# jgeisler0303/DDP-Generator

Hardware: AMD Instinct MI355X
Metric: iLQG iterations/sec, 65k-batch CarParking (n=4,m=2,N=500) (higher is better)
Workload: dtype f64

## Files before the change

### ddp-generator_amd/csrc/ilqg_host.c

```c
#include <math.h>
#include <stddef.h>
#include <stdio.h>
#include <stdlib.h>
#include <string.h>
#include <sys/time.h>

#include "mex.h"
#include "iLQG.h"
#include "back_pass.h"
#include "line_search.h"
#include "boxQP.h"
#include "matMult.h"
#include "printMat.h"

#include "ilqg_batch.h"
#include "ilqg_shim.h"
#include "ilqg_rules.h"

#define REC_HOST_SIZE_BASE (N_X + sizeofQxx + N_U + sizeofQuu + sizeofQxu + N_X * N_X + N_X * N_U + 2 * N_U)
#if FULL_DDP
#define REC_HOST_SIZE (REC_HOST_SIZE_BASE + N_X * sizeofQxx + N_X * sizeofQuu + N_X * sizeofQxu + 2 * N_U + 2 * N_X * N_U)
#else
#define REC_HOST_SIZE (REC_HOST_SIZE_BASE + 2 * N_U + 2 * N_X * N_U)
#endif
#define FIN_SIZE (N_X + sizeofQxx)

#ifndef DEBUG_ILQG
#define DEBUG_ILQG 1
#endif
#ifndef DEBUG_FORWARDPASS
#define DEBUG_FORWARDPASS 1
#endif
#define SAY_LOOP(level, args) do { if((DEBUG_ILQG) && o->debug_level >= (level)) PRNT args; } while(0)
#define SAY_SEARCH(level, args) do { if((DEBUG_FORWARDPASS) && o->debug_level >= (level)) PRNT args; } while(0)

#define ILQG_MAX_GROUPS 4
#define ILQG_TRACE_MAX 4096
struct ilqg_batch {
    ilqg_dev_t *dev[ILQG_MAX_GROUPS];
    int first[ILQG_MAX_GROUPS], count[ILQG_MAX_GROUPS];
    int groups;
    int device, B, N;
    tOptSet opt;
    double alpha_store[ILQG_MAX_ALPHA];
    int resweep, fuse_derivs, ls_split, ls_keep, bw_split;
    double **p;
    char *p_given;
    int params_pushed;
    int pb_n, pb_W, pb_named[64];
    char ps_on[64];
    int hist_cap;
    int compact;
    int trace_n;
    int trace_it[ILQG_TRACE_MAX], trace_active[ILQG_TRACE_MAX], trace_slots[ILQG_TRACE_MAX];
    int compactions;
    long long stream_counts[4];
    double *scratch;
    size_t scratch_doubles;
    char err[512];
};

static char g_create_err[512];

static void fatal_no_device(const char *what, const char *msg) {
    fprintf(stderr,
            "ilqg: %s needs the HIP backend, which is unavailable: %s\n"
            "ilqg: this library has no CPU fallback for the hot path.\n",
            what, msg ? msg : "");
    abort();
}

static double ilqg_default_alpha[8] = {1.0, 0.3727594, 0.1389495, 0.0517947,
                                       0.0193070, 0.0071969, 0.0026827, 0.0010000};

void standard_parameters(tOptSet *o) {
    o->alpha = ilqg_default_alpha;
    o->n_alpha = 8;
    o->tolFun = 1e-7;
    o->tolConstraint = 1e-7;
    o->tolGrad = 1e-5;
    o->max_iter = 20;
    o->lambdaInit = 1;
    o->dlambdaInit = 1;
    o->lambdaFactor = 1.6;
    o->lambdaMax = 1e10;
    o->lambdaMin = 1e-6;
    o->regType = 1;
    o->zMin = 0.0;
    o->debug_level = 2;
    o->w_pen_init_l = 1.0;
    o->w_pen_init_f = 1.0;
    o->w_pen_max_l = INF;
    o->w_pen_max_f = INF;
    o->w_pen_fact1 = 4.0;
    o->w_pen_fact2 = 1.0;
}

static char err_scalar[] = "parameter must be scalar";
static char err_alpha_range[] = "all alpha must be in the range [1.0..0.0)";
static char err_alpha_mono[] = "all alpha must be monotonically decreasing";
static char err_pos[] = "parameter must be positive";
static char err_gt_one[] = "parameter must be > 1";
static char err_one_two[] = "parameter must be in range [1..2]";
static char err_zero_one[] = "parameter must be in range [0..1)";
static char err_debug[] = "parameter must be in range [0..6]";
static char err_unknown[] = "no such parameter";

enum { CHK_GT0, CHK_GE0, CHK_GE1, CHK_1_2, CHK_0_1, CHK_0_6 };
typedef struct {
    const char *name;
    size_t offset;
    int is_int;
    int check;
} opt_row_t;

#define ROW_D(field, chk) {#field, offsetof(tOptSet, field), 0, chk}
#define ROW_I(field, chk) {#field, offsetof(tOptSet, field), 1, chk}
static const opt_row_t opt_rows[] = {
    ROW_D(tolFun, CHK_GT0),       ROW_D(tolConstraint, CHK_GT0), ROW_D(tolGrad, CHK_GT0),
    ROW_I(max_iter, CHK_GE0),     ROW_D(lambdaInit, CHK_GE0),    ROW_D(dlambdaInit, CHK_GE0),
    ROW_D(lambdaFactor, CHK_GE1), ROW_D(lambdaMax, CHK_GE0),     ROW_D(lambdaMin, CHK_GE0),
    ROW_I(regType, CHK_1_2),      ROW_D(zMin, CHK_0_1),          ROW_I(debug_level, CHK_0_6),
    ROW_D(w_pen_init_l, CHK_GE0), ROW_D(w_pen_init_f, CHK_GE0),  ROW_D(w_pen_max_l, CHK_GE0),
    ROW_D(w_pen_max_f, CHK_GE0),  ROW_D(w_pen_fact1, CHK_GE1),   ROW_D(w_pen_fact2, CHK_GE1),
};

char *setOptParam(tOptSet *o, const char *name, const double *value, const int n) {
    size_t r;
// ... 46 lines not shown
void printTri(const double *A, const int n, const char *nm) {
    int r, c;
    PRNT("%s= [\n", nm);
    for(r = 0; r < n; r++) {
        for(c = 0; c < n; c++) PRNT(c ? ", %g" : "  %g", A[SYMTRI_MAT_IDX(r, c)]);
        PRNT("\n");
    }
    PRNT("]\n");
}

void printMat(const double *A, const int n, const int m, const char *nm) {
    int r, c;
    PRNT("%s= [\n", nm);
    for(r = 0; r < n; r++) {
        for(c = 0; c < m; c++) PRNT(c ? ", %g" : "  %g", A[r + n * c]);
        PRNT("\n");
    }
    PRNT("]\n");
}

void printParams(double **p, int k) {
    int i;
    for(i = 0; i < n_params; i++) {
        if(paramdesc[i]->size == -1)
            PRNT("%s[k]= %g\n", paramdesc[i]->name, p[i][k]);
        else if(paramdesc[i]->size == 1)
            PRNT("%s= %g\n", paramdesc[i]->name, p[i][0]);
        else
            printVec(p[i], paramdesc[i]->size, paramdesc[i]->name);
    }
}

static int fail(ilqg_batch_t *c, const char *what) {
    snprintf(c->err, sizeof(c->err), "%s: %s", what, ilqg_dev_error());
    return 1;
}

static int fail_msg(ilqg_batch_t *c, const char *msg) {
    snprintf(c->err, sizeof(c->err), "%s", msg);
    return 1;
}

void ilqg_problem_dims(int *out) {
    ilqg_dev_dims(out);
    out[6] = n_params;
}

const char *ilqg_problem_param_name(int i) { return (i >= 0 && i < n_params) ? paramdesc[i]->name : NULL; }
int ilqg_problem_param_size(int i) { return (i >= 0 && i < n_params) ? paramdesc[i]->size : 0; }
int ilqg_device_count(void) { return ilqg_dev_count(); }

int ilqg_reference_success(int status, int iterations) {
    switch(status) {
    case ILQG_ST_CONVERGED_GRAD:
    case ILQG_ST_CONVERGED_FUN:
    case ILQG_ST_LAMBDA_MAX: return 1;
    case ILQG_ST_DERIVS_FAILED: return iterations > 0;
    default: return 0;
    }
}

const char *ilqg_batch_error(const ilqg_batch_t *c) { return c ? c->err : g_create_err; }

static int param_len(const ilqg_batch_t *c, int i) { return paramdesc[i]->size == -1 ? c->N + 1 : paramdesc[i]->size; }

static int find_param(const char *name) {
    int i;
    for(i = 0; i < n_params; i++)
        if(strcmp(paramdesc[i]->name, name) == 0) return i;
    return -1;
}

ilqg_batch_t *ilqg_batch_create_groups(int device, int batch, int n_hor, int groups) {
    int i, g, per, dims[8];
    ilqg_batch_t *c = (ilqg_batch_t *)calloc(1, sizeof(*c));
    if(!c) return NULL;
    c->device = device;
    c->B = batch;
    c->N = n_hor;
    c->resweep = (sizeof(multipliersEl_t) > 0 || sizeof(multipliersFin_t) > 0) ? 1 : 0;
    c->fuse_derivs = c->resweep ? 0 : 1;
    c->ls_keep = 1;
    c->bw_split = 0;
    standard_parameters(&c->opt);
    ilqg_dev_dims(dims);
    c->ls_split = dims[7] ? 1 : 4;
    c->ls_keep = 2;
    if(groups <= 0) {
        const char *e = getenv("ILQG_GROUPS");
        groups = e ? atoi(e) : ((batch >= 8192 && !dims[7]) ? 4 : 1);
    }

    if(groups < 1) groups = 1;
    if(groups > ILQG_MAX_GROUPS) groups = ILQG_MAX_GROUPS;
    per = ((batch + groups - 1) / groups + 63) / 64 * 64;
    c->groups = 0;
    for(g = 0; g < groups && (g == 0 || g * per < batch); g++) {
        c->first[g] = g * per;
        c->count[g] = (batch - g * per < per) ? batch - g * per : per;
        if(ilqg_dev_create(&c->dev[g], device, c->count[g], n_hor)) {
            snprintf(g_create_err, sizeof(g_create_err), "ilqg_batch_create: %s", ilqg_dev_error());
            for(i = 0; i < g; i++) ilqg_dev_destroy(c->dev[i]);
            free(c);
            return NULL;
        }
        c->groups = g + 1;
    }
    c->p = (double **)calloc(n_params > 0 ? n_params : 1, sizeof(double *));
    c->p_given = (char *)calloc(n_params > 0 ? n_params : 1, 1);
    for(i = 0; i < n_params; i++) c->p[i] = (double *)calloc(param_len(c, i), sizeof(double));
    return c;
}

ilqg_batch_t *ilqg_batch_create(int device, int batch, int n_hor) {
    return ilqg_batch_create_groups(device, batch, n_hor, 0);
}

int ilqg_batch_groups(const ilqg_batch_t *c) { return c->groups; }

void ilqg_batch_destroy(ilqg_batch_t *c) {
    int i;
    if(!c) return;
    for(i = 0; i < c->groups; i++) ilqg_dev_destroy(c->dev[i]);
    for(i = 0; i < n_params; i++) free(c->p[i]);
    free(c->p);
    free(c->p_given);
    free(c->scratch);
    free(c);
}

#define EACH_GROUP(g) for(g = 0; g < c->groups; g++)
static int each_write(ilqg_batch_t *c, int field, const double *host, const char *what) {
    int g;
    EACH_GROUP(g) {
        const size_t per = (size_t)ilqg_dev_field_steps(c->dev[g], field) * ilqg_dev_field_width(field);
        if(ilqg_dev_write(c->dev[g], field, host + per * c->first[g])) return fail(c, what);
    }
    return 0;
}
static int each_write_steps(ilqg_batch_t *c, int field, const double *host, int steps, const char *what) {
    int g;
    EACH_GROUP(g) {
        const size_t per = (size_t)steps * ilqg_dev_field_width(field);
        if(ilqg_dev_write_steps(c->dev[g], field, host + per * c->first[g], steps)) return fail(c, what);
    }
    return 0;
}
static int each_read(ilqg_batch_t *c, int field, double *host, const char *what) {
    int g;
    EACH_GROUP(g) {
        const size_t per = (size_t)ilqg_dev_field_steps(c->dev[g], field) * ilqg_dev_field_width(field);
        if(ilqg_dev_read(c->dev[g], field, host + per * c->first[g])) return fail(c, what);
    }
    return 0;
}
static int int_width(int field) { return field == ILQG_I_ALPHA_OK ? ILQG_MAX_ALPHA : 1; }
static int each_read_int(ilqg_batch_t *c, int field, int *host, const char *what) {
    int g;
    EACH_GROUP(g) if(ilqg_dev_read_int(c->dev[g], field, host + (size_t)int_width(field) * c->first[g])) return fail(c, what);
    return 0;
}
static int each_write_int(ilqg_batch_t *c, int field, const int *host, const char *what) {
    int g;
    EACH_GROUP(g) if(ilqg_dev_write_int(c->dev[g], field, host + (size_t)int_width(field) * c->first[g])) return fail(c, what);
    return 0;
}

int ilqg_batch_set_option(ilqg_batch_t *c, const char *name, const double *value, int n) {
    char *e;
    if(strcmp(name, "resweep") == 0) {
        if(n != 1) return fail_msg(c, err_scalar);
        c->resweep = value[0] != 0.0;
        return 0;
    }
    if(strcmp(name, "ls_split") == 0) {
        if(n != 1) return fail_msg(c, err_scalar);
        if(value[0] < 0.0) return fail_msg(c, err_pos);
        c->ls_split = (int)value[0];
        return 0;
    }
    if(strcmp(name, "bw_split") == 0) {
        if(n != 1) return fail_msg(c, err_scalar);
        c->bw_split = value[0] != 0.0;
        return 0;
    }
    if(strcmp(name, "ls_keep") == 0) {
        if(n != 1) return fail_msg(c, err_scalar);
        if(value[0] != 0.0 && value[0] != 1.0 && value[0] != 2.0) return fail_msg(c, "ls_keep must be 0, 1 or 2");
        c->ls_keep = (int)value[0];
        return 0;
    }
    if(strcmp(name, "fuse_derivs") == 0) {
        if(n != 1) return fail_msg(c, err_scalar);
        c->fuse_derivs = value[0] != 0.0;
        return 0;
    }
    if(strcmp(name, "compact") == 0) {
        if(n != 1) return fail_msg(c, err_scalar);
        if(value[0] < 0.0) return fail_msg(c, err_pos);
        c->compact = (int)value[0];
        return 0;
    }
    if(strcmp(name, "alpha") == 0) {
        tOptSet probe = c->opt;
        if(n > ILQG_MAX_ALPHA) return fail_msg(c, "at most 16 alpha values");
        e = setOptParam(&probe, name, value, n);
        if(e) return fail_msg(c, e);
        memcpy(c->alpha_store, value, sizeof(double) * n);
        value = c->alpha_store;
    }
    e = setOptParam(&c->opt, name, value, n);
    if(e) return fail_msg(c, e);
    return 0;
}

int ilqg_batch_set_param(ilqg_batch_t *c, const char *name, const double *value, int n) {
    const int i = find_param(name);
    int j;
    if(i < 0) {
        snprintf(c->err, sizeof(c->err), "Parameter name '%s' is not a parameter of this problem.", name);
        return 1;
    }
    if(param_len(c, i) != n) {
        snprintf(c->err, sizeof(c->err), "Parameter name '%s' must be a vector length %d.", name, param_len(c, i));
        return 1;
    }
    for(j = 0; j < c->pb_n; j++)
        if(c->pb_named[j] == i) {
            snprintf(c->err, sizeof(c->err), "ilqg_batch_set_param: name: parameter '%s' currently has a value per trajectory "
                     "(ilqg_batch_set_params_batch); a shared value would be read by no trajectory.  Clear the per-trajectory set "
                     "first: ilqg_batch_set_params_batch(c, 0, NULL, NULL)", name);
            return 1;
        }
    if(i < 64 && c->ps_on[i]) {
        snprintf(c->err, sizeof(c->err), "ilqg_batch_set_param: name: parameter '%s' currently has a window per trajectory "
                 "(ilqg_batch_set_param_steps_batch); a shared window would be read by no trajectory.  Use "
                 "ilqg_batch_set_param_steps_batch / ilqg_batch_shift_param_batch, or make the name shared again first: "
                 "ilqg_batch_set_param_steps_batch(c, name, values = NULL)", name);
        return 1;
    }
    memcpy(c->p[i], value, sizeof(double) * n);
    c->p_given[i] = 1;
    c->params_pushed = 0;
    return 0;
}

static int push_config(ilqg_batch_t *c) {
    ilqg_dev_opts_t d;
    int i;
    const tOptSet *o = &c->opt;
    memset(&d, 0, sizeof(d));
    if(o->n_alpha < 1 || o->n_alpha > ILQG_MAX_ALPHA) return fail_msg(c, "n_alpha must be in 1..16");
    d.n_alpha = o->n_alpha;
    for(i = 0; i < o->n_alpha; i++) d.alpha[i] = o->alpha[i];
    d.tolFun = o->tolFun; d.tolGrad = o->tolGrad; d.tolConstraint = o->tolConstraint;
    d.lambdaInit = o->lambdaInit; d.dlambdaInit = o->dlambdaInit; d.lambdaFactor = o->lambdaFactor;
    d.lambdaMax = o->lambdaMax; d.lambdaMin = o->lambdaMin;
    d.zMin = o->zMin; d.regType = o->regType; d.max_iter = o->max_iter;
    d.w_pen_init_l = o->w_pen_init_l; d.w_pen_init_f = o->w_pen_init_f;
    d.w_pen_max_l = o->w_pen_max_l; d.w_pen_max_f = o->w_pen_max_f;
    d.w_pen_fact1 = o->w_pen_fact1; d.w_pen_fact2 = o->w_pen_fact2;
    d.resweep = c->resweep;
    d.fuse_derivs = c->fuse_derivs;
    d.ls_split = c->ls_split;
    d.ls_keep = c->ls_keep;
    d.bw_split = c->bw_split;
    { int g; EACH_GROUP(g) if(ilqg_dev_set_opts(c->dev[g], &d)) return fail(c, "options"); }
    if(!c->params_pushed) {
        int sizes[64];
        for(i = 0; i < n_params; i++)
            if(!c->p_given[i]) {
                snprintf(c->err, sizeof(c->err), "Parameter name '%s' was not set.", paramdesc[i]->name);
                return 1;
            }
        if(n_params > 64) return fail_msg(c, "more than 64 problem parameters");
        for(i = 0; i < n_params; i++) sizes[i] = paramdesc[i]->size;
        { int g; EACH_GROUP(g) if(ilqg_dev_set_params(c->dev[g], n_params, sizes, (const double *const *)c->p)) return fail(c, "parameters"); }
        c->params_pushed = 1;
    }
    return 0;
}

int ilqg_batch_set_x0(ilqg_batch_t *c, const double *x0) { return each_write_steps(c, ILQG_F_X, x0, 1, "set_x0"); }
int ilqg_batch_set_u(ilqg_batch_t *c, const double *u) { return each_write(c, ILQG_F_U, u, "set_u"); }
int ilqg_batch_set_x(ilqg_batch_t *c, const double *x) { return each_write(c, ILQG_F_X, x, "set_x"); }

static int restart(ilqg_batch_t *c) {
    int g;
    EACH_GROUP(g) {
        if(ilqg_dev_rollout_init(c->dev[g])) return fail(c, "initial roll-out");
        if(ilqg_dev_reset(c->dev[g])) return fail(c, "reset");
    }
    return 0;
}

static int clear_history(ilqg_batch_t *c, const char *who) {
    int g;
    if(c->hist_cap > 0) EACH_GROUP(g) if(ilqg_dev_set_history(c->dev[g], c->hist_cap)) return fail(c, who);
    return 0;
}

int ilqg_batch_init(ilqg_batch_t *c) { return push_config(c) || clear_history(c, "ilqg_batch_init") || restart(c); }

typedef struct { const void *ptr; const char *name; } named_ptr_t;
static int device_ptrs(ilqg_batch_t *c, const char *who, const named_ptr_t *ptrs, int n) {
    int i;
    for(i = 0; i < n; i++)
        if(ptrs[i].ptr && ilqg_dev_check_device_ptr(c->dev[0], ptrs[i].ptr, ptrs[i].name)) return fail(c, who);
    return 0;
}
static int stream_in(ilqg_batch_t *c, void *stream, const char *what) {
    int g;
    EACH_GROUP(g) if(ilqg_dev_stream_in(c->dev[g], stream)) return fail(c, what);
    return 0;
}

static int shift_groups(ilqg_batch_t *c, int round, int on_device, int steps, const double *x0_new, const double *u_tail, void *stream) {
    int g;
    EACH_GROUP(g) if(round >= 0 ? ilqg_dev_loop_shift(c->dev[g], round) : ilqg_dev_shift(c->dev[g], steps, x0_new == NULL)) return fail(c, "shift");
    EACH_GROUP(g) {
        const double *const x0_g = x0_new ? x0_new + (size_t)c->first[g] * N_X : NULL;
        const double *const tail_g = (u_tail && steps > 0) ? u_tail + (size_t)c->first[g] * steps * N_U : NULL;
        if(x0_g && (on_device ? ilqg_dev_put_x0_device(c->dev[g], x0_g) : ilqg_dev_write_steps(c->dev[g], ILQG_F_X, x0_g, 1)))
            return fail(c, "shift: x0_new");
        if(tail_g && (on_device ? ilqg_dev_put_u_tail_device : ilqg_dev_write_u_tail)(c->dev[g], tail_g, steps)) return fail(c, "shift: u_tail");
        if(on_device && ilqg_dev_stream_out(c->dev[g], stream)) return fail(c, "shift: stream");
    }
    return restart(c);
}
static int shift(ilqg_batch_t *c, const char *who, int on_device, int steps, const double *x0_new, const double *u_tail, void *stream) {
    const named_ptr_t ptrs[] = {{x0_new, "x0_new"}, {u_tail, "u_tail"}};
    if(steps < 0 || steps >= c->N) {
        snprintf(c->err, sizeof(c->err), "%s: steps = %d, must be in 0 .. n_hor - 1 = %d", who, steps, c->N - 1);
        return 1;
    }
    if(on_device && device_ptrs(c, who, ptrs, 2)) return 1;
    if(push_config(c)) return 1;
    if(on_device && stream_in(c, stream, "shift: stream")) return 1;
    return shift_groups(c, -1, on_device, steps, x0_new, u_tail, stream);
}

int ilqg_batch_shift(ilqg_batch_t *c, int steps, const double *x0_new, const double *u_tail) {
    return shift(c, "ilqg_batch_shift", 0, steps, x0_new, u_tail, NULL);
}

int ilqg_batch_shift_device(ilqg_batch_t *c, int steps, const double *x0_new, const double *u_tail, void *stream) {
    return shift(c, "ilqg_batch_shift_device", 1, steps, x0_new, u_tail, stream);
}

// ... 633 lines not shown
    }
    if(steps < 0 || steps > c->N) {
        snprintf(c->err, sizeof(c->err), "ilqg_batch_shift_param: steps = %d, must be in 0 .. n_hor = %d", steps, c->N);
        return 1;
    }
    if(i < 64 && c->ps_on[i]) {
        snprintf(c->err, sizeof(c->err), "ilqg_batch_shift_param: name: parameter '%s' currently has a window per trajectory "
                 "(ilqg_batch_set_param_steps_batch); moving the shared window would move what no trajectory reads.  Use "
                 "ilqg_batch_shift_param_batch, or make the name shared again first: ilqg_batch_set_param_steps_batch(c, name, "
                 "values = NULL)", name);
        return 1;
    }
    if(steps == 0) return 0;
    n = c->N + 1;
    if(c->params_pushed) EACH_GROUP(g) if(ilqg_dev_shift_param(c->dev[g], i, steps, tail)) return fail(c, "shift_param");
    for(k = 0; k < n; k++) c->p[i][k] = k + steps < n ? c->p[i][k + steps] : (tail ? tail[k + steps - n] : c->p[i][n - 1]);
    return 0;
}

static int iterate_groups(ilqg_batch_t *c, int n) {
    int it, g;
    for(it = 0; it < n; it++) EACH_GROUP(g) if(ilqg_dev_iterate(c->dev[g], 1)) return fail(c, "iterate");
    return 0;
}

int ilqg_batch_iterate(ilqg_batch_t *c, int n) {
    if(push_config(c)) return 1;
    return iterate_groups(c, n);
}

int ilqg_batch_active(ilqg_batch_t *c, int *n) {
    int g, a;
    *n = 0;
    EACH_GROUP(g) {
        if(ilqg_dev_count_active(c->dev[g], &a)) return fail(c, "active count");
        *n += a;
    }
    return 0;
}

static double now_s(void) {
    struct timeval tv;
    gettimeofday(&tv, NULL);
    return (double)tv.tv_sec + 1e-6 * (double)tv.tv_usec;
}
static int group_of(const ilqg_batch_t *c, int b) {
    int g;
    for(g = c->groups - 1; g > 0; g--)
        if(b >= c->first[g]) break;
    return g;
}
static int move_between(ilqg_batch_t *dst, ilqg_batch_t *src, int n, const int *dst_idx, const int *src_idx) {
    int gd, gs, j, rc = 0;
    int *to = (int *)malloc(sizeof(int) * (n > 0 ? n : 1)), *from = (int *)malloc(sizeof(int) * (n > 0 ? n : 1));
    for(gd = 0; gd < dst->groups && !rc; gd++)
        for(gs = 0; gs < src->groups && !rc; gs++) {
            int m = 0;
            for(j = 0; j < n; j++)
                if(group_of(dst, dst_idx[j]) == gd && group_of(src, src_idx[j]) == gs) {
                    to[m] = dst_idx[j] - dst->first[gd];
                    from[m] = src_idx[j] - src->first[gs];
                    m++;
                }
            if(m && ilqg_dev_move(dst->dev[gd], src->dev[gs], m, to, from, !src->fuse_derivs)) rc = fail(dst, "moving trajectories");
        }
    free(to);
    free(from);
    return rc;
}
static ilqg_batch_t *working_copy(ilqg_batch_t *c, int n) {
    int i;
    int dims[8], groups;
    ilqg_batch_t *w;
    ilqg_dev_dims(dims);
    (void)dims;
    groups = 0;
    if(getenv("ILQG_COMPACT_GROUPS")) groups = atoi(getenv("ILQG_COMPACT_GROUPS"));
    w = ilqg_batch_create_groups(c->device, n, c->N, groups);
    if(!w) return NULL;
    c->stream_counts[3] += 1;
    w->opt = c->opt;
    memcpy(w->alpha_store, c->opt.alpha, sizeof(double) * c->opt.n_alpha);
    w->opt.alpha = w->alpha_store;
    w->resweep = c->resweep; w->fuse_derivs = c->fuse_derivs; w->ls_split = c->ls_split; w->ls_keep = c->ls_keep; w->bw_split = c->bw_split;
    for(i = 0; i < n_params; i++) {
        memcpy(w->p[i], c->p[i], sizeof(double) * param_len(c, i));
        w->p_given[i] = c->p_given[i];
    }
    if(push_config(w)) {
        snprintf(c->err, sizeof(c->err), "%s", w->err);
        ilqg_batch_destroy(w);
        return NULL;
    }
    return w;
}

int ilqg_batch_solve(ilqg_batch_t *c) {
    int it, active = 1, rc = 0, j;
    ilqg_batch_t *cur = c;
    int *map = NULL, *status = NULL, *ident = NULL;
    const int dbg = getenv("ILQG_SOLVE_DEBUG") != NULL;
    double t_dbg = 0.0, t_poll = 0.0;
    if(push_config(c)) return 1;
    c->err[0] = 0;
    c->trace_n = 0;
    t_poll = dbg ? now_s() : 0.0;
    c->compactions = 0;
    for(it = 0; it < c->opt.max_iter && active; ) {
        int n = c->opt.max_iter - it < 4 ? c->opt.max_iter - it : 4;
        if(iterate_groups(cur, n)) { rc = 1; break; }
        it += n;
        if(ilqg_batch_active(cur, &active)) { rc = 1; break; }
        if(dbg && it % 40 == 0) {
            fprintf(stderr, "ilqg solve: iteration %d, %d live of %d slots, %.2f ms per iteration\n", it, active, cur->B, 1e3 * (now_s() - t_poll) / n);
        }
        t_poll = dbg ? now_s() : 0.0;
        if(c->trace_n < ILQG_TRACE_MAX) {
            c->trace_it[c->trace_n] = it;
            c->trace_active[c->trace_n] = active;
            c->trace_slots[c->trace_n] = cur->B;
            c->trace_n++;
        }
        if(c->compact > 0 && active > 0 && it < c->opt.max_iter && 2 * active <= cur->B && active >= c->compact) {
            ilqg_batch_t *w;
            int *nmap, m = 0;
            status = (int *)realloc(status, sizeof(int) * cur->B);
            if(each_read_int(cur, ILQG_I_STATUS, status, "status")) { rc = 1; break; }
            if(cur != c) {
                ident = (int *)realloc(ident, sizeof(int) * cur->B);
                for(j = 0; j < cur->B; j++) ident[j] = j;
                if(move_between(c, cur, cur->B, map, ident)) { rc = 1; break; }
            }
            nmap = (int *)malloc(sizeof(int) * active);
            for(j = 0; j < cur->B && m < active; j++)
                if(status[j] == ILQG_ST_ACTIVE) nmap[m++] = (cur == c) ? j : map[j];
            t_dbg = dbg ? now_s() : 0.0;
            w = working_copy(c, m);
            if(!w) { free(nmap); rc = 1; break; }
            if(dbg) fprintf(stderr, "ilqg solve: iteration %d, %d live of %d slots: new context %.1f ms", it, m, cur->B, 1e3 * (now_s() - t_dbg));
            t_dbg = dbg ? now_s() : 0.0;
            ident = (int *)realloc(ident, sizeof(int) * (m > cur->B ? m : cur->B));
            for(j = 0; j < m; j++) ident[j] = j;
            if(move_between(w, c, m, ident, nmap)) { snprintf(c->err, sizeof(c->err), "%s", w->err); ilqg_batch_destroy(w); free(nmap); rc = 1; break; }
            if(dbg) fprintf(stderr, ", gather %.1f ms", 1e3 * (now_s() - t_dbg));
            t_dbg = dbg ? now_s() : 0.0;
            if(cur != c) ilqg_batch_destroy(cur);
            if(dbg) fprintf(stderr, ", release %.1f ms\n", 1e3 * (now_s() - t_dbg));
            free(map);
            cur = w;
            map = nmap;
            c->compactions++;
        }
    }
    if(cur != c) {
        if(!rc) {
            ident = (int *)realloc(ident, sizeof(int) * cur->B);
            for(j = 0; j < cur->B; j++) ident[j] = j;
            if(move_between(c, cur, cur->B, map, ident)) rc = 1;
        } else if(!c->err[0]) {
            snprintf(c->err, sizeof(c->err), "%s", cur->err);
        }
        ilqg_batch_destroy(cur);
    }
    free(map);
    free(status);
    free(ident);
    return rc;
// ... 1384 lines not shown
```

### ddp-generator_amd/csrc/ilqg_shim.h

```cpp
#ifndef ILQG_SHIM_H
#define ILQG_SHIM_H

#ifdef __cplusplus
extern "C" {
#endif

#define ILQG_MAX_ALPHA 16

typedef struct ilqg_dev ilqg_dev_t;

typedef struct {
    int n_alpha;
    double alpha[ILQG_MAX_ALPHA];
    double tolFun, tolGrad, tolConstraint;
    double lambdaInit, dlambdaInit, lambdaFactor, lambdaMax, lambdaMin;
    double zMin;
    int regType;
    int max_iter;
    double w_pen_init_l, w_pen_init_f, w_pen_max_l, w_pen_max_f, w_pen_fact1, w_pen_fact2;
    int resweep;
    int ls_split;
    int ls_keep;
    int bw_split;
    int fuse_derivs;
} ilqg_dev_opts_t;

enum {
    ILQG_ST_ACTIVE = 0,
    ILQG_ST_CONVERGED_GRAD = 1,
    ILQG_ST_CONVERGED_FUN = 2,
    ILQG_ST_MAX_ITER = 3,
    ILQG_ST_NO_DESCENT = 4,
    ILQG_ST_LAMBDA_MAX = 5,
    ILQG_ST_DERIVS_FAILED = 6,
    ILQG_ST_INIT_FAILED = 7
};

enum {
    ILQG_F_X = 0,
    ILQG_F_U,
    ILQG_F_LG,
    ILQG_F_KG,
    ILQG_F_DER,
    ILQG_F_FIN,
    ILQG_F_MUL,
    ILQG_F_MULF,
    ILQG_F_COST,
    ILQG_F_NEW_COST,
    ILQG_F_DCOST,
    ILQG_F_EXPECTED,
    ILQG_F_LAMBDA,
    ILQG_F_DLAMBDA,
    ILQG_F_GNORM,
    ILQG_F_DV0,
    ILQG_F_DV1,
    ILQG_F_WPEN_L,
    ILQG_F_WPEN_F,
    ILQG_F_WPEN_L_DER,
    ILQG_F_WPEN_F_DER,
    ILQG_F_ALPHA_COST,
    ILQG_F_COUNT
};

enum {
    ILQG_I_STATUS = 0,
    ILQG_I_ITER,
    ILQG_I_NEED_DERIVS,
    ILQG_I_ALPHA_IDX,
    ILQG_I_ACCEPTED,
    ILQG_I_BP_CALLS,
    ILQG_I_BP_RC,
    ILQG_I_RESWEEP,
    ILQG_I_LOC,
    ILQG_I_ALPHA_OK,
    ILQG_I_COUNT
};

enum {
    ILQG_K_DERIVS = 0,
    ILQG_K_BACKWARD,
    ILQG_K_ROLLOUT_SEARCH,
    ILQG_K_SELECT,
    ILQG_K_ROLLOUT_WINNER,
    ILQG_K_UPDATE,
    ILQG_K_ROLLOUT_COST,
    ILQG_K_ROLLOUT_INIT,
    ILQG_K_TRANSPOSE,
    ILQG_K_BACKWARD_FUSED,
    ILQG_K_ROLLOUT_SEARCH2,
    ILQG_K_MULTIPLIERS,
    ILQG_K_SEARCH,
    ILQG_K_SEARCH2,
    ILQG_K_ADOPT,
    ILQG_K_SHIFT,
    ILQG_K_LOG,
    ILQG_K_HEAD,
    ILQG_K_SHIFT_PARAM,
    ILQG_K_POLICY,
    ILQG_K_POLICY_PARAMS,
    ILQG_K_PLANT,
    ILQG_K_SHIFT_PARAM_ROWS,
    ILQG_K_SHIFT_WINDOWS,
    ILQG_K_HISTORY,
    ILQG_K_COUNT
};
enum {
    ILQG_K_BEST_OF = ILQG_K_COUNT,
// ... 146 lines not shown
```

### ddp-generator_amd/csrc/ilqg_shim_impl.inc

```

#if ILQG_WAVE_MAP
struct SharedWork {
    trajEl_t *buf;
    size_t bytes;
    hipEvent_t free_ev;
    int refs;
    bool whole, half[2], factored, pv_set;
    int N, B, part, half_cap;
    ParamValues pv;
};
static SharedWork g_work[64];
#else
struct SharedWork;
#endif

constexpr int QUEUE_CELL = 32;

namespace {

struct DeviceMem {
    static hipError_t take(void **p, size_t bytes) { return hipMalloc(p, bytes); }
    static hipError_t give(void *p) { return hipFree(p); }
};
struct PinnedMem {
    static hipError_t take(void **p, size_t bytes) { return hipHostMalloc(p, bytes, hipHostMallocDefault); }
    static hipError_t give(void *p) { return hipHostFree(p); }
};
template <class T, class Mem = DeviceMem>
class Buffer {
    T *p_ = nullptr;
    size_t bytes_ = 0;

  public:
    Buffer() = default;
    Buffer(const Buffer &) = delete;
    Buffer &operator=(const Buffer &) = delete;
    Buffer(Buffer &&o) noexcept : p_(o.p_), bytes_(o.bytes_) { o.p_ = nullptr, o.bytes_ = 0; }
    Buffer &operator=(Buffer &&o) noexcept {
        if(this != &o) {
            (void)release();
            p_ = o.p_, bytes_ = o.bytes_;
            o.p_ = nullptr, o.bytes_ = 0;
        }
        return *this;
    }
    ~Buffer() {
        if(p_) (void)Mem::give(p_);
    }
    T *get() const { return p_; }
    size_t bytes() const { return bytes_; }
    int release() {
        T *old = p_;
        p_ = nullptr, bytes_ = 0;
        if(old) HIP_TRY(Mem::give(old));
        return 0;
    }
    int renew(size_t bytes) {
        if(release()) return 1;
        const hipError_t allocation = Mem::take((void **)&p_, bytes);
        if(allocation != hipSuccess) p_ = nullptr;
        HIP_TRY(allocation);
        bytes_ = bytes;
        return 0;
    }
    int reserve(size_t bytes, hipStream_t drain = nullptr) {
        if(bytes <= bytes_) return 0;
        if(drain) HIP_TRY(hipStreamSynchronize(drain));
        return renew(bytes);
    }
    int try_reserve(size_t bytes, hipStream_t drain) {
        if(bytes <= bytes_) return 0;
        HIP_TRY(hipStreamSynchronize(drain));
        if(release()) return 1;
        if(getenv("ILQG_TEST_NO_PLANES") || Mem::take((void **)&p_, bytes) != hipSuccess) {
            (void)hipGetLastError();
            p_ = nullptr;
            return 2;
        }
        bytes_ = bytes;
        return 0;
    }
};
template <class T>
static int repoint(T *&view, const Buffer<T> &owner, int rc) {
    view = owner.get();
    return rc;
}

struct DevBuffers {
    Buffer<double> f[ILQG_F_COUNT], nom;
    Buffer<int> i[ILQG_I_COUNT], derivs_failed, pending_list, n_pending;
    Buffer<trajEl_t> work;
    Buffer<double *> param_table;
    std::vector<Buffer<double>> param_bufs;
    Buffer<int> counter;
    Buffer<int> queues;
    Buffer<double> cand, cand1;
    Buffer<double> xpl, upl;
    Buffer<unsigned> spec_ints;
    Buffer<double> spec_doubles;
    Buffer<double> log_x, log_u, log_c;
    Buffer<double> plant_xp, plant_cost, plant_values, plant_dist;
    Buffer<int> plant_failed;
    Buffer<double> pb_values;
    static constexpr int SR = N_STEP_PARAMS > 0 ? N_STEP_PARAMS : 1;
    Buffer<double> sr_rows[SR];
    Buffer<double> win_future[SR];
    Buffer<double> hist_d;
    Buffer<int> hist_i;
    Buffer<double> hist_next_d;
    Buffer<int> hist_next_i;
    Buffer<unsigned long long> harvest;
    Buffer<char, PinnedMem> harvest_host;
    Buffer<double> staging;
    Buffer<char, PinnedMem> pinned;
};

template <class Fn>
struct WaveKernel {
    Fn fn;
    int block;
    size_t lds;
    int per_wg;
    int cap;
    size_t lds_limit;
    bool scratch;
    dim3 grid(size_t n, int cus) const {
        const size_t wgs = (n + per_wg - 1) / per_wg, most = (size_t)cap * cus;
        return dim3((unsigned)(cap && most < wgs ? most : wgs));
    }
};
struct WaveKernels {
    WaveKernel<void (*)(DevPtrs, ilqg_dev_opts_t, ParamValues, int, int, int, int, int)> derivs[2];
    WaveKernel<void (*)(DevPtrs, ilqg_dev_opts_t, int, int, int)> sweep[6];
};

}

struct ilqg_dev : DevBuffers {
    int device, B, Bp, N;
    hipStream_t stream;
    DevPtrs P;
    ilqg_dev_opts_t O;
    ParamValues pv;
    bool io_deferred;
    size_t io_off;
    struct PendingRead { void *dst; const void *src; size_t bytes; int transpose_w; };
    std::vector<PendingRead> pending;
    bool keep_first;
    size_t roll_pad;
    bool roll_dma;
    int loc_set;
    bool defer_commit, commit_pending, pending_zero;
    int commit_s1, commit_set;
    bool winner_done;
    int cus;
    bool work_consts;
    bool half_consts[2];
    hipStream_t stream2;
    hipEvent_t fork, join;
    hipStream_t roll;
    hipEvent_t roll_in, roll_out;
    struct SharedWork *shared;
    bool per_step_params;
    struct Loop {
        int rounds, steps;
        bool plant, windows;
        bool named;
        PolicyParamMap map;
        bool given[SR];
    } loop;
    bool pb_on;
    PolicyParamMap pb_map;
    bool sr_on[SR];
    bool rows_on;
    PolicyParamMap rows_map;
    int hist_next_cap;
    History hist;
    hipEvent_t ext_in, ext_out;
    struct EnvSwitches { bool no_quad, quad_stored, two_pieces, deriv_parts, no_dma, no_rollout_parts, quad_spec, second_stream; size_t roll_lds; } env;
    WaveKernels wave_kernels;
    bool timing;
    struct Span { int kernel; hipEvent_t a, b; };
    std::vector<Span> spans;
    std::vector<hipEvent_t> event_pool;
    double t_ms[ILQG_K_TOTAL];
    int t_n[ILQG_K_TOTAL];
    hipEvent_t epoch;
    double t_busy[ILQG_K_TOTAL];
};

namespace {

static ilqg_dev *g_spec_last;
struct FieldInfo { int steps_plus; int wd, wh; };

FieldInfo field_info(int f) {
    switch(f) {
        case ILQG_F_X: return {1, NX, NX};
        case ILQG_F_U: return {0, NU, NU};
        case ILQG_F_LG: return {0, NU, NU};
        case ILQG_F_KG: return {0, NXU, NXU};
        case ILQG_F_DER: return {0, WAVE_MAP ? REC_HOST : REC, REC_HOST};
        case ILQG_F_FIN: return {-1, FIN, FIN};
        case ILQG_F_MUL: return {0, MEW, MEW};
        case ILQG_F_MULF: return {-1, MFW, MFW};
        case ILQG_F_ALPHA_COST: return {-1, ILQG_MAX_ALPHA, ILQG_MAX_ALPHA};
        default: return {-1, 1, 1};
    }
}

int nom_column(int field) {
    switch(field) {
        case ILQG_F_X: return NOM_X;
        case ILQG_F_U: return NOM_U;
        case ILQG_F_LG: return NOM_L;
        case ILQG_F_KG: return NOM_K;
        default: return -1;
    }
}
bool has_tiled_copy(int field) { return !WAVE_MAP && (field == ILQG_F_X || field == ILQG_F_U); }
bool has_tiled_scratch(int field) { return !WAVE_MAP && (field == ILQG_F_LG || field == ILQG_F_KG); }
int field_steps(const ilqg_dev *d, int f) {
    const FieldInfo fi = field_info(f);
    return fi.steps_plus < 0 ? 1 : d->N + fi.steps_plus;
}

int int_field_width(int f) { return f == ILQG_I_ALPHA_OK ? ILQG_MAX_ALPHA : 1; }

int io_flush(ilqg_dev *d) {
    HIP_TRY(hipStreamSynchronize(d->stream));
    for(const auto &r : d->pending) {
        if(r.transpose_w) {
            const int *src = (const int *)r.src;
            int *dst = (int *)r.dst;
            for(int b = 0; b < d->B; b++)
                for(int j = 0; j < r.transpose_w; j++) dst[(size_t)b * r.transpose_w + j] = src[(size_t)j * d->Bp + b];
        } else {
            memcpy(r.dst, r.src, r.bytes);
        }
    }
    d->pending.clear();
    d->io_off = 0;
    return 0;
}

int stage(ilqg_dev *d, size_t bytes, void **dev, void **pin) {
    if(!d->io_deferred) {
        if(d->staging.reserve(bytes)) return 1;
        *dev = d->staging.get();
        *pin = nullptr;
        return 0;
    }
    bytes = (bytes + 255) & ~(size_t)255;
    if(d->io_off + bytes > d->staging.bytes() || d->io_off + bytes > d->pinned.bytes()) {
        if(io_flush(d)) return 1;
        const size_t want = (bytes > (1u << 20) ? bytes : (1u << 20)) + 2 * d->pinned.bytes();
        if(d->staging.reserve(want) || d->pinned.reserve(want)) return 1;
    }
    *dev = (char *)d->staging.get() + d->io_off;
    *pin = d->pinned.get() + d->io_off;
    d->io_off += bytes;
    return 0;
}
int stage_in(ilqg_dev *d, void *dev, void *pin, const void *host, size_t bytes) {
    if(pin) {
        memcpy(pin, host, bytes);
        host = pin;
    }
    HIP_TRY(hipMemcpyAsync(dev, host, bytes, hipMemcpyHostToDevice, d->stream));
    return 0;
}
int stage_out(ilqg_dev *d, const void *dev, void *pin, void *host, size_t bytes) {
    HIP_TRY(hipMemcpyAsync(pin ? pin : host, dev, bytes, hipMemcpyDeviceToHost, d->stream));
    if(pin) d->pending.push_back({host, pin, bytes, 0});
    else HIP_TRY(hipStreamSynchronize(d->stream));
    return 0;
}
// ... 298 lines not shown
                    }
                    bytes = bytes / 2 + sizeof(trajEl_t);
                }
                W.bytes = bytes;
                HIP_TRY(hipMemsetAsync(W.buf, 0, W.bytes, d->stream));
                HIP_TRY(hipStreamSynchronize(d->stream));
                HIP_TRY(hipEventCreateWithFlags(&W.free_ev, hipEventDisableTiming));
            }
            W.refs++;
            d->shared = &W;
            if((W.bytes - sizeof(trajEl_t)) / per_traj < 1) {
                g_err = "ilqg_dev_create: the device's derivative work buffer (made for a shorter horizon) does not hold one trajectory";
                return 1;
            }
#endif
            continue;
        }
        if(nom_column(f) >= 0 && !has_tiled_copy(f) && !has_tiled_scratch(f)) continue;
        const FieldInfo fi = field_info(f);
        const size_t bytes = (size_t)field_steps(d, f) * fi.wd * d->Bp * sizeof(double);
        if(repoint(d->P.f[f], d->f[f], d->f[f].reserve(bytes))) return 1;
        HIP_TRY(hipMemsetAsync(d->P.f[f], 0, bytes, d->stream));
    }
    {
        const size_t bytes = (size_t)d->Bp * (d->N + 1) * RN * sizeof(double);
        if(repoint(d->P.nom, d->nom, d->nom.reserve(bytes))) return 1;
        HIP_TRY(hipMemsetAsync(d->P.nom, 0, bytes, d->stream));
    }
    for(int f = 0; f < ILQG_I_COUNT; f++) {
        const size_t bytes = (size_t)int_field_width(f) * d->Bp * sizeof(int);
        if(repoint(d->P.i[f], d->i[f], d->i[f].reserve(bytes))) return 1;
        HIP_TRY(hipMemsetAsync(d->P.i[f], 0, bytes, d->stream));
    }
    if(repoint(d->P.derivs_failed, d->derivs_failed, d->derivs_failed.reserve(d->Bp * sizeof(int)))) return 1;
    HIP_TRY(hipMemsetAsync(d->P.derivs_failed, 0, d->Bp * sizeof(int), d->stream));
    if(d->counter.reserve(sizeof(int))) return 1;
    if(d->queues.reserve(2 * QUEUE_CELL * sizeof(int))) return 1;
    {
        int cus = 0;
        HIP_TRY(hipDeviceGetAttribute(&cus, hipDeviceAttributeMultiprocessorCount, device));
        d->cus = cus > 0 ? cus : 256;
    }
    if(repoint(d->P.pending, d->pending_list, d->pending_list.reserve(d->Bp * sizeof(int)))) return 1;
    if(repoint(d->P.n_pending, d->n_pending, d->n_pending.reserve(sizeof(int)))) return 1;
    HIP_TRY(hipMemsetAsync(d->P.n_pending, 0, sizeof(int), d->stream));
    d->P.n_pending_next = d->P.n_pending;
    HIP_TRY(hipStreamSynchronize(d->stream));
    return 0;
}

void ilqg_dev_destroy(ilqg_dev_t *d) {
    if(!d) return;
    hipSetDevice(d->device);
    if(d->stream) hipStreamSynchronize(d->stream);
    if(d->stream2) hipStreamSynchronize(d->stream2);
    for(auto &s : d->spans) {
        hipEventDestroy(s.a);
        hipEventDestroy(s.b);
    }
    for(hipEvent_t e : d->event_pool) hipEventDestroy(e);
    static_cast<DevBuffers &>(*d) = DevBuffers();
#if ILQG_WAVE_MAP
    if(d->shared && --d->shared->refs == 0) {
        hipFree(d->shared->buf);
        hipEventDestroy(d->shared->free_ev);
        memset(d->shared, 0, sizeof(SharedWork));
    }
#endif
    if(g_spec_last == d) g_spec_last = nullptr;
    if(d->stream) hipStreamDestroy(d->stream);
    if(d->stream2) hipStreamDestroy(d->stream2);
    if(d->fork) hipEventDestroy(d->fork);
    if(d->join) hipEventDestroy(d->join);
    if(d->roll) hipStreamSynchronize(d->roll);
    if(d->roll_in) hipEventDestroy(d->roll_in);
    if(d->roll_out) hipEventDestroy(d->roll_out);
    if(d->epoch) hipEventDestroy(d->epoch);
    if(d->ext_in) hipEventDestroy(d->ext_in);
    if(d->ext_out) hipEventDestroy(d->ext_out);
    delete d;
}

int ilqg_dev_set_params(ilqg_dev_t *d, int n_params, const int *sizes, const double *const *values) {
    HIP_TRY(hipSetDevice(d->device));
    HIP_TRY(hipStreamSynchronize(d->stream));
    d->param_bufs.clear();
    if(repoint(d->P.p, d->param_table, d->param_table.release())) return 1;
    std::vector<double *> ptrs(n_params > 0 ? n_params : 1, nullptr);
    {
        constexpr int want[ILQG_NP > 0 ? ILQG_NP : 1] = ILQG_PSIZES;
        constexpr int offs[ILQG_NP > 0 ? ILQG_NP : 1] = ILQG_POFFSETS;
        if(n_params != ILQG_NP) {
            g_err = "ilqg_dev_set_params: parameter count differs from the problem this library was built for";
            return 1;
        }
        for(int i = 0; i < n_params; i++) {
            if(sizes[i] != want[i]) {
                g_err = "ilqg_dev_set_params: parameter size differs from the problem's paramdesc[]";
                return 1;
            }
            for(int j = 0; j < sizes[i]; j++) d->pv.v[offs[i] + j] = values[i][j];
        }
        d->per_step_params = false;
        for(int i = 0; i < n_params; i++) d->per_step_params |= (sizes[i] == -1);
    }
    for(int i = 0; i < n_params; i++) {
        const int sz = sizes[i] == -1 ? d->N + 1 : sizes[i];
        Buffer<double> buf;
        if(buf.reserve(sz * sizeof(double))) return 1;
        HIP_TRY(hipMemcpy(buf.get(), values[i], sz * sizeof(double), hipMemcpyHostToDevice));
        ptrs[i] = buf.get();
        d->param_bufs.push_back(std::move(buf));
    }
    if(repoint(d->P.p, d->param_table, d->param_table.reserve(ptrs.size() * sizeof(double *)))) return 1;
    HIP_TRY(hipMemcpy(d->P.p, ptrs.data(), ptrs.size() * sizeof(double *), hipMemcpyHostToDevice));
    d->work_consts = d->half_consts[0] = d->half_consts[1] = false;
    return 0;
}

static const PolicyParamMap *policy_param_map(int n_named, const int *named, const double *values, PolicyParamMap &map);
static void rows_refresh(ilqg_dev_t *d) {
    PolicyParamMap m;
    if(d->pb_on) {
        m = d->pb_map;
    } else {
        for(int j = 0; j < ILQG_PTOTAL; j++) m.src[j] = -1;
        m.W = 0;
    }
    const bool steps = step_rows_into(m, d);
    d->rows_map = m;
    d->rows_on = d->pb_on || steps;
}
static int table_buffer(ilqg_dev_t *d, size_t bytes) {
    if(bytes <= d->pb_values.bytes()) return 0;
    d->pb_on = false;
    rows_refresh(d);
    return d->pb_values.reserve(bytes, d->stream);
}
int ilqg_dev_set_params_batch(ilqg_dev_t *d, int n_named, const int *named, const double *values, int on_device) {
    HIP_TRY(hipSetDevice(d->device));
    if(WAVE_MAP) {
        g_err = "set_params_batch: this library maps one wavefront to a trajectory (wave mapping); its kernels do not carry "
                "parameters per lane, per-trajectory parameters need a lane-mapped library";
        return 1;
    }
    if(n_named < 0) {
        g_err = "set_params_batch: n_names must not be negative";
        return 1;
    }
    if(n_named == 0) {
        d->pb_on = false;
        rows_refresh(d);
        return 0;
    }
    PolicyParamMap map;
    if(!policy_param_map(n_named, named, values, map)) return 1;
    const size_t bytes = (size_t)d->B * (size_t)map.W * sizeof(double);
    if(table_buffer(d, bytes)) return 1;
    HIP_TRY(hipMemcpyAsync(d->pb_values.get(), values, bytes, on_device ? hipMemcpyDeviceToDevice : hipMemcpyHostToDevice, d->stream));
    if(!on_device) HIP_TRY(hipStreamSynchronize(d->stream));
    d->pb_map = map;
    d->pb_on = true;
    rows_refresh(d);
    return 0;
}

static int step_slot(int index) {
    constexpr int sizes[ILQG_NP > 0 ? ILQG_NP : 1] = ILQG_PSIZES;
    if(index < 0 || index >= ILQG_NP || sizes[index] != -1) return -1;
    int s = 0;
    for(int i = 0; i < index; i++) s += sizes[i] == -1 ? 1 : 0;
    return s;
}
static int step_rows_buffer(ilqg_dev_t *d, int s) {
    const size_t n = (size_t)d->N + 1, bytes = (size_t)d->Bp * n * sizeof(double);
    if(bytes > d->sr_rows[s].bytes()) {
        d->sr_on[s] = false;
        rows_refresh(d);
        if(d->sr_rows[s].reserve(bytes, d->stream)) return 1;
    }
    if(!d->sr_on[s] && d->Bp > d->B)
        HIP_TRY(hipMemsetAsync(d->sr_rows[s].get() + (size_t)d->B * n, 0, (size_t)(d->Bp - d->B) * n * sizeof(double), d->stream));
    return 0;
}
int ilqg_dev_set_param_steps_batch(ilqg_dev_t *d, int index, const double *values, int on_device) {
    HIP_TRY(hipSetDevice(d->device));
    if(WAVE_MAP) {
        g_err = "set_param_steps_batch: this library maps one wavefront to a trajectory (wave mapping); its kernels do not carry "
                "parameters per lane, per-trajectory parameters need a lane-mapped library";
        return 1;
    }
    const int s = step_slot(index);
    if(s < 0) {
        g_err = "set_param_steps_batch: not a parameter with one value per time step";
        return 1;
    }
    if(!values) {
        d->sr_on[s] = false;
        rows_refresh(d);
        return 0;
    }
    if(step_rows_buffer(d, s)) return 1;
    const size_t bytes = (size_t)d->B * ((size_t)d->N + 1) * sizeof(double);
    HIP_TRY(hipMemcpyAsync(d->sr_rows[s].get(), values, bytes, on_device ? hipMemcpyDeviceToDevice : hipMemcpyHostToDevice, d->stream));
    if(!on_device) HIP_TRY(hipStreamSynchronize(d->stream));
    d->sr_on[s] = true;
    rows_refresh(d);
    return 0;
}

int ilqg_dev_get_param_steps_batch(ilqg_dev_t *d, int index, double *rows) {
    HIP_TRY(hipSetDevice(d->device));
    const int s = step_slot(index);
    if(s < 0 || !d->sr_on[s]) {
        g_err = "get_param_steps_batch: the parameter has no rows per trajectory in this context";
        return 1;
    }
    HIP_TRY(hipMemcpyAsync(rows, d->sr_rows[s].get(), (size_t)d->B * ((size_t)d->N + 1) * sizeof(double), hipMemcpyDeviceToHost, d->stream));
    HIP_TRY(hipStreamSynchronize(d->stream));
    return 0;
}

int ilqg_dev_get_params_batch(ilqg_dev_t *d, double *rows) {
    HIP_TRY(hipSetDevice(d->device));
    if(!d->pb_on) {
        g_err = "get_params_batch: the context has no per-trajectory parameters";
        return 1;
    }
    HIP_TRY(hipMemcpyAsync(rows, d->pb_values.get(), (size_t)d->B * (size_t)d->pb_map.W * sizeof(double), hipMemcpyDeviceToHost, d->stream));
    HIP_TRY(hipStreamSynchronize(d->stream));
    return 0;
}

int ilqg_dev_set_opts(ilqg_dev_t *d, const ilqg_dev_opts_t *o) {
#if !ILQG_EXPERIMENTS
    if(o->bw_split) {
        g_err = "option bw_split: the two-wavefront backward pass (a measured negative result) is compiled into the -DILQG_EXPERIMENTS libraries only (lib*_exp.so)";
        return 1;
    }
#endif
    if(o->n_alpha < 1 || o->n_alpha > ILQG_MAX_ALPHA) {
        g_err = "ilqg_dev_set_opts: n_alpha must be in 1..16";
        return 1;
    }
    d->O = *o;
    return 0;
}

int ilqg_dev_field_width(int field) { return field_info(field).wh; }
int ilqg_dev_field_steps(ilqg_dev_t *d, int field) { return field_steps(d, field); }
void *ilqg_dev_field_ptr(ilqg_dev_t *d, int field) { return d->P.f[field]; }
void *ilqg_dev_stream(ilqg_dev_t *d) { return (void *)d->stream; }

int ilqg_dev_copy_scalar_to(ilqg_dev_t *d, int field, void *dst_device) {
    HIP_TRY(hipSetDevice(d->device));
    if(field < ILQG_F_COST || field >= ILQG_F_ALPHA_COST) {
        g_err = "ilqg_dev_copy_scalar_to: not a per-trajectory scalar field";
        return 1;
    }
    HIP_TRY(hipMemcpyAsync(dst_device, d->P.f[field], (size_t)d->B * sizeof(double), hipMemcpyDeviceToDevice, d->stream));
    return 0;
}

int ilqg_dev_write(ilqg_dev_t *d, int field, const double *host) {
    return ilqg_dev_write_steps(d, field, host, field_steps(d, field));
}

static bool is_traj_major(int field) { return WAVE_MAP && field == ILQG_F_FIN; }

static int nom_io(ilqg_dev *d, int field, double *host_rw, const double *host_ro, int steps) {
    const FieldInfo fi = field_info(field);
    const size_t n = (size_t)d->B * steps * fi.wh;
    void *dev, *pin;
    if(stage(d, n * sizeof(double), &dev, &pin)) return 1;
    if(host_ro && stage_in(d, dev, pin, host_ro, n * sizeof(double))) return 1;
    {
        Timed t(d, ILQG_K_TRANSPOSE);
        hipLaunchKernelGGL(k_nom_io, grid1(n, 256), dim3(256), 0, d->stream, d->P.nom, (double *)dev, d->B, d->N, steps,
                           fi.wh, nom_column(field), host_ro ? 1 : 0);
    }
    HIP_TRY(hipGetLastError());
    if(host_rw) return stage_out(d, dev, pin, host_rw, n * sizeof(double));
    return io_done(d);
}

#if ILQG_WAVE_MAP
#define REC_FIELDS(OP)                                                                            \
    OP(cx, NX) OP(cxx, SXX) OP(cu, NU) OP(cuu, SUU) OP(cxu, NXU) OP(fx, NX * NX) OP(fu, NXU)     \
    OP(lower, NU) OP(upper, NU) REC_FIELDS_FULL(OP)                                               \
    OP(lower_sign, NU) OP(upper_sign, NU) OP(lower_hx, NXU) OP(upper_hx, NXU)
#if FULL_DDP
#define REC_FIELDS_FULL(OP) OP(fxx, NX * SXX) OP(fuu, NX * SUU) OP(fxu, NX * NXU)
#else
#define REC_FIELDS_FULL(OP)
#endif

static int own_work(ilqg_dev *d) {
    if(d->P.work) return 0;
    size_t free_b = 0, total_b = 0;
    HIP_TRY(hipMemGetInfo(&free_b, &total_b));
    const size_t per_traj = (size_t)d->N * sizeof(trajEl_t);
    if((double)d->B * (double)per_traj > 0.5 * (double)free_b) {
        g_err = "derivative records of the whole batch do not fit the device (wave mapping): stage-by-stage calls and "
                "record transfers need a smaller batch; ilqg_dev_iterate / ilqg_dev_backward(mode 2) work in chunks";
        return 1;
    }
    if(repoint(d->P.work, d->work, d->work.reserve((size_t)d->B * per_traj))) return 1;
    HIP_TRY(hipMemsetAsync(d->P.work, 0, (size_t)d->B * per_traj, d->stream));
    d->work_consts = false;
    return 0;
}

static int der_io(ilqg_dev *d, double *host_rw, const double *host_ro) {
    if(own_work(d)) return 1;
    const size_t n = (size_t)d->B * d->N;
    std::vector<trajEl_t> tmp(n);
    HIP_TRY(hipMemcpy(tmp.data(), d->P.work, n * sizeof(trajEl_t), hipMemcpyDeviceToHost));
    for(size_t e = 0; e < n; e++) {
        trajEl_t &t = tmp[e];
        if(host_ro) {
            const double *r = host_ro + e * REC_HOST;
#define OP(field, cnt) memcpy(t.field, r, sizeof(double) * (cnt)); r += (cnt);
            REC_FIELDS(OP)
#undef OP
        } else {
            double *r = host_rw + e * REC_HOST;
#define OP(field, cnt) memcpy(r, t.field, sizeof(double) * (cnt)); r += (cnt);
            REC_FIELDS(OP)
#undef OP
        }
    }
    if(host_ro) HIP_TRY(hipMemcpy(d->P.work, tmp.data(), n * sizeof(trajEl_t), hipMemcpyHostToDevice));
    return 0;
}
#endif

static int all_home(ilqg_dev_t *d);

int ilqg_dev_write_steps(ilqg_dev_t *d, int field, const double *host, int steps) {
    HIP_TRY(hipSetDevice(d->device));
    if(has_tiled_copy(field) && all_home(d)) return 1;
    const FieldInfo fi = field_info(field);
    if(steps < 1 || steps > field_steps(d, field)) {
        g_err = "ilqg_dev_write_steps: bad step count";
        return 1;
    }
#if ILQG_WAVE_MAP
    if(field == ILQG_F_DER) {
        if(io_flush(d)) return 1;
        return der_io(d, nullptr, host);
    }
#endif
    if(nom_column(field) >= 0) {
        if(nom_io(d, field, nullptr, host, steps)) return 1;
        if(!has_tiled_copy(field)) return 0;
    }
    if(is_traj_major(field)) {
        const size_t row = (size_t)steps * fi.wd * sizeof(double);
        const size_t dpitch = (size_t)field_steps(d, field) * fi.wd * sizeof(double);
        const void *src = host;
        if(d->io_deferred) {
            void *dev, *pin;
            if(stage(d, row * d->B, &dev, &pin)) return 1;
            memcpy(pin, host, row * d->B);
            src = pin;
        }
        HIP_TRY(hipMemcpy2DAsync(d->P.f[field], dpitch, src, row, row, d->B, hipMemcpyHostToDevice, d->stream));
        return io_done(d);
    }
    const size_t n = (size_t)d->B * steps * fi.wh;
    void *dev, *pin;
    if(stage(d, n * sizeof(double), &dev, &pin)) return 1;
    if(stage_in(d, dev, pin, host, n * sizeof(double))) return 1;
    {
        Timed t(d, ILQG_K_TRANSPOSE);
        const size_t total = (size_t)d->B * steps * fi.wd;
        hipLaunchKernelGGL(k_to_dev, grid1(total, 256), dim3(256), 0, d->stream, (const double *)dev, d->P.f[field], d->B, d->Bp,
                           steps, fi.wh, fi.wd);
    }
    HIP_TRY(hipGetLastError());
    return io_done(d);
}

int ilqg_dev_read(ilqg_dev_t *d, int field, double *host) {
    HIP_TRY(hipSetDevice(d->device));
    if(has_tiled_copy(field) && all_home(d)) return 1;
    const FieldInfo fi = field_info(field);
    const int steps = field_steps(d, field);
    const size_t n = (size_t)d->B * steps * fi.wh;
#if ILQG_WAVE_MAP
    if(field == ILQG_F_DER) {
        if(io_flush(d)) return 1;
        return der_io(d, host, nullptr);
    }
#endif
    if(nom_column(field) >= 0 && !has_tiled_copy(field)) return nom_io(d, field, host, nullptr, steps);
    if(is_traj_major(field)) {
        void *dev = nullptr, *pin = nullptr;
        if(d->io_deferred && stage(d, n * sizeof(double), &dev, &pin)) return 1;
        return stage_out(d, d->P.f[field], pin, host, n * sizeof(double));
    }
    void *dev, *pin;
    if(stage(d, n * sizeof(double), &dev, &pin)) return 1;
    {
        Timed t(d, ILQG_K_TRANSPOSE);
        hipLaunchKernelGGL(k_from_dev, grid1(n, 256), dim3(256), 0, d->stream, d->P.f[field], (double *)dev, d->B, d->Bp,
                           steps, fi.wh, fi.wd);
    }
    HIP_TRY(hipGetLastError());
    return stage_out(d, dev, pin, host, n * sizeof(double));
}

int ilqg_dev_write_int(ilqg_dev_t *d, int field, const int *host) {
    HIP_TRY(hipSetDevice(d->device));
    const int w = int_field_width(field);
    const size_t bytes = (size_t)w * d->Bp * sizeof(int);
    std::vector<int> tmp;
    int *src;
    if(d->io_deferred) {
        void *dev, *pin;
        if(stage(d, bytes, &dev, &pin)) return 1;
        src = (int *)pin;
    } else {
        tmp.resize((size_t)w * d->Bp);
        src = tmp.data();
    }
    memset(src, 0, bytes);
    for(int b = 0; b < d->B; b++)
        for(int j = 0; j < w; j++) src[(size_t)j * d->Bp + b] = host[(size_t)b * w + j];
    HIP_TRY(hipMemcpyAsync(d->P.i[field], src, bytes, hipMemcpyHostToDevice, d->stream));
    return io_done(d);
}

int ilqg_dev_read_int(ilqg_dev_t *d, int field, int *host) {
    HIP_TRY(hipSetDevice(d->device));
    const int w = int_field_width(field);
    const size_t bytes = (size_t)w * d->Bp * sizeof(int);
    if(d->io_deferred) {
        void *dev, *pin;
        if(stage(d, bytes, &dev, &pin)) return 1;
        HIP_TRY(hipMemcpyAsync(pin, d->P.i[field], bytes, hipMemcpyDeviceToHost, d->stream));
        d->pending.push_back({host, pin, bytes, w});
        return 0;
    }
    std::vector<int> tmp((size_t)w * d->Bp, 0);
    HIP_TRY(hipMemcpyAsync(tmp.data(), d->P.i[field], tmp.size() * sizeof(int), hipMemcpyDeviceToHost, d->stream));
    HIP_TRY(hipStreamSynchronize(d->stream));
    for(int b = 0; b < d->B; b++)
        for(int j = 0; j < w; j++) host[(size_t)b * w + j] = tmp[(size_t)j * d->Bp + b];
    return 0;
}

int ilqg_dev_io_begin(ilqg_dev_t *d) {
    d->io_deferred = true;
    d->io_off = 0;
    return 0;
}

int ilqg_dev_io_end(ilqg_dev_t *d) {
    HIP_TRY(hipSetDevice(d->device));
    d->io_deferred = false;
    return io_flush(d);
}

#define NEED_PARAMS(d)                                                   \
    if(!(d)->P.p) {                                                      \
        g_err = "problem parameters not set (ilqg_dev_set_params)";      \
        return 1;                                                        \
    }

static int all_home(ilqg_dev_t *d) {
#if !ILQG_WAVE_MAP
    if(d->loc_set < 0) return 0;
    hipLaunchKernelGGL(k_all_home, dim3(8 * d->cus), dim3(256), 0, d->stream, d->P);
    HIP_TRY(hipGetLastError());
    HIP_TRY(hipMemsetAsync(d->P.i[ILQG_I_LOC], 0, d->Bp * sizeof(int), d->stream));
    d->loc_set = -1;
#endif
    return 0;
}

int ilqg_dev_reset(ilqg_dev_t *d) {
    HIP_TRY(hipSetDevice(d->device));
    hipLaunchKernelGGL(k_reset, grid1(d->Bp, 256), dim3(256), 0, d->stream, d->P, d->O);
    if(HAS_MUL) {
        NEED_PARAMS(d);
        Timed t(d, ILQG_K_MULTIPLIERS);
        LAUNCH_TWIN(d, k_multipliers, dim3(d->Bp / WAVE), dim3(WAVE), 0, d->stream, d->P, d->O, d->pv, 1);
    }
    HIP_TRY(hipGetLastError());
    return 0;
}

static hipStream_t roll_stream(ilqg_dev_t *d) { return d->roll ? d->roll : d->stream; }
static int roll_enter(ilqg_dev_t *d) {
    if(!d->roll) return 0;
    HIP_TRY(hipEventRecord(d->roll_in, d->stream));
    HIP_TRY(hipStreamWaitEvent(d->roll, d->roll_in, 0));
    return 0;
}
static int roll_leave(ilqg_dev_t *d) {
    if(!d->roll) return 0;
    HIP_TRY(hipEventRecord(d->roll_out, d->roll));
    HIP_TRY(hipStreamWaitEvent(d->stream, d->roll_out, 0));
    return 0;
}

static void launch_rollout(ilqg_dev_t *d, int mode, int kernel_id, int a0, int n_alpha, hipStream_t stream = nullptr) {
    if(!stream) stream = d->stream;
    Timed t(d, kernel_id, stream);
    const dim3 grid((d->Bp + ROLL_BLOCK - 1) / ROLL_BLOCK, n_alpha), block(ROLL_BLOCK);
    if(mode == ROLL_INIT)
        with_rows(d, [&](auto... tr) { hipLaunchKernelGGL((k_rollout<RK_INIT, decltype(tr)...>), grid, block, 0, stream, d->P, d->O, d->pv, mode, a0, tr...); });
    else if(mode == ROLL_COST)
        with_rows(d, [&](auto... tr) { hipLaunchKernelGGL((k_rollout<RK_COST, decltype(tr)...>), grid, block, 0, stream, d->P, d->O, d->pv, mode, a0, tr...); });
#if ILQG_WAVE_MAP && defined(ILQG_ROLLOUT_PARTS)
    else if(!HAS_MUL && !d->env.no_rollout_parts) {
        DevPtrs Q = d->P;
        if(!d->keep_first) Q.cand1 = nullptr;
        if(d->roll_dma) {
            hipLaunchKernelGGL(k_rollout_parts<true>, dim3(d->Bp / WAVE, n_alpha), dim3(WAVE * RW), (size_t)WAVE * RNP * sizeof(double) + d->roll_pad,
                               stream, Q, d->O, d->pv, mode, a0);
        } else {
            const size_t lds = (n_alpha > 1) ? d->env.roll_lds : 0;
            hipLaunchKernelGGL(k_rollout_parts<false>, dim3(d->Bp / WAVE, n_alpha), dim3(WAVE * RW), lds, stream, Q, d->O, d->pv, mode, a0);
        }
    }
#endif
    else
        with_rows(d, [&](auto... tr) { hipLaunchKernelGGL((k_rollout<RK_GENERAL, decltype(tr)...>), grid, block, 0, stream, d->P, d->O, d->pv, mode, a0, tr...); });
}

int ilqg_dev_rollout_init(ilqg_dev_t *d) {
    NEED_PARAMS(d);
    HIP_TRY(hipSetDevice(d->device));
    if(all_home(d)) return 1;
    if(roll_enter(d)) return 1;
    HIP_TRY(hipMemsetAsync(d->P.i[ILQG_I_STATUS], 0, d->Bp * sizeof(int), roll_stream(d)));
    launch_rollout(d, ROLL_INIT, ILQG_K_ROLLOUT_INIT, 0, 1, roll_stream(d));
    HIP_TRY(hipGetLastError());
    return roll_leave(d);
}

int ilqg_dev_shift(ilqg_dev_t *d, int steps, int use_plan_x0) {
    HIP_TRY(hipSetDevice(d->device));
    if(steps < 0 || steps >= d->N) {
        g_err = "ilqg_dev_shift: steps must be in 0 .. n_hor - 1";
        return 1;
    }
    {
        Timed t(d, ILQG_K_SHIFT);
#if ILQG_WAVE_MAP
        hipLaunchKernelGGL(k_shift_wave, dim3(d->B), dim3(SHIFT_BLOCK), 0, d->stream, d->P, steps, use_plan_x0);
#else
        hipLaunchKernelGGL(k_shift_lane, dim3((unsigned)((size_t)(NX > NU ? NX : NU) * d->Bp / WAVE)), dim3(WAVE * SHIFT_WAVES), 0, d->stream, d->P, steps, use_plan_x0);
#endif
    }
    HIP_TRY(hipGetLastError());
#if !ILQG_WAVE_MAP
    if(d->loc_set >= 0) HIP_TRY(hipMemsetAsync(d->P.i[ILQG_I_LOC], 0, d->Bp * sizeof(int), d->stream));
    d->loc_set = -1;
#endif
    return 0;
}

int ilqg_dev_write_u_tail(ilqg_dev_t *d, const double *host, int steps) {
    HIP_TRY(hipSetDevice(d->device));
    if(steps < 1 || steps > d->N) {
        g_err = "ilqg_dev_write_u_tail: bad step count";
        return 1;
    }
    if(all_home(d)) return 1;
    const size_t n = (size_t)d->B * steps * NU;
    void *dev, *pin;
    if(stage(d, n * sizeof(double), &dev, &pin)) return 1;
    if(stage_in(d, dev, pin, host, n * sizeof(double))) return 1;
    {
        Timed t(d, ILQG_K_TRANSPOSE);
        hipLaunchKernelGGL(k_put_u_steps, grid1(n, 256), dim3(256), 0, d->stream, d->P, (const double *)dev, d->N - steps, steps);
    }
    HIP_TRY(hipGetLastError());
    return io_done(d);
}

static int segments_ok(ilqg_dev_t *d, int K, int first) {
    if(K < 1 || K > WAVE || (K & (K - 1)) != 0) {
        g_err = "K must be one of 1, 2, 4, 8, 16, 32, 64";
        return 0;
    }
    if(d->B % K != 0 || first < 0 || first % K != 0) {
        g_err = "K must divide the group's size and its first trajectory";
        return 0;
    }
    return 1;
}
static size_t slice(size_t &total, size_t bytes) {
    const size_t at = total;
    total += (bytes + 255) & ~(size_t)255;
    return at;
}

static int launch_best_of(ilqg_dev_t *d, int K, int first, const double *score, int *winner, double *best, int *n_eligible) {
    {
        Timed t(d, ILQG_K_BEST_OF);
        hipLaunchKernelGGL(k_best_of, dim3(d->Bp / WAVE), dim3(WAVE), 0, d->stream, d->P, K, first, score, winner, best, n_eligible);
    }
    HIP_TRY(hipGetLastError());
    return 0;
}

int ilqg_dev_best_of(ilqg_dev_t *d, int K, int first, const double *score, int *winner, double *best, int *n_eligible, int on_device) {
    HIP_TRY(hipSetDevice(d->device));
    if(!segments_ok(d, K, first)) return 1;
    if(!winner) {
        g_err = "best_of: winner is NULL";
        return 1;
    }
    if(on_device) return launch_best_of(d, K, first, score, winner, best, n_eligible);
    const size_t G = (size_t)(d->B / K);
    size_t total = 0;
    const size_t o_score = slice(total, score ? d->B * sizeof(double) : 0), o_win = slice(total, G * sizeof(int));
    const size_t o_best = slice(total, best ? G * sizeof(double) : 0), o_n = slice(total, n_eligible ? G * sizeof(int) : 0);
    void *dev, *pin;
    if(stage(d, total, &dev, &pin)) return 1;
    char *const dv = (char *)dev, *const pv = (char *)pin;
    if(score && stage_in(d, dv + o_score, pin ? pv + o_score : nullptr, score, d->B * sizeof(double))) return 1;
    if(launch_best_of(d, K, first, score ? (const double *)(dv + o_score) : nullptr, (int *)(dv + o_win), best ? (double *)(dv + o_best) : nullptr,
                      n_eligible ? (int *)(dv + o_n) : nullptr))
        return 1;
    void *const host[3] = {winner, best, n_eligible};
    const size_t off[3] = {o_win, o_best, o_n}, bytes[3] = {G * sizeof(int), G * sizeof(double), G * sizeof(int)};
    for(int i = 0; i < 3; i++) {
        if(!host[i]) continue;
        void *to = pin ? (void *)(pv + off[i]) : host[i];
        HIP_TRY(hipMemcpyAsync(to, dv + off[i], bytes[i], hipMemcpyDeviceToHost, d->stream));
        if(pin) d->pending.push_back({host[i], to, bytes[i], 0});
    }
    if(!pin) HIP_TRY(hipStreamSynchronize(d->stream));
    return 0;
}

int ilqg_dev_shift_winners(ilqg_dev_t *d, int K, int first, const int *winner, int steps, const double *x0_new, const double *u_tail, const double *du,
                           int on_device) {
    HIP_TRY(hipSetDevice(d->device));
    if(!segments_ok(d, K, first)) return 1;
    if(steps < 0 || steps >= d->N) {
        g_err = "ilqg_dev_shift_winners: steps must be in 0 .. n_hor - 1";
        return 1;
    }
    if(!winner) {
        g_err = "ilqg_dev_shift_winners: winner is NULL";
        return 1;
    }
    if(steps == 0) u_tail = nullptr;
    if(!on_device) {
        const size_t G = (size_t)(d->B / K);
        size_t total = 0;
        const size_t b_win = G * sizeof(int), b_x0 = x0_new ? G * NX * sizeof(double) : 0, b_tail = u_tail ? G * steps * NU * sizeof(double) : 0;
        const size_t b_du = du ? (size_t)d->B * d->N * NU * sizeof(double) : 0;
        const size_t o_win = slice(total, b_win), o_x0 = slice(total, b_x0), o_tail = slice(total, b_tail), o_du = slice(total, b_du);
        void *dev, *pin;
        if(stage(d, total, &dev, &pin)) return 1;
        char *const dv = (char *)dev, *const pv = (char *)pin;
        if(stage_in(d, dv + o_win, pin ? pv + o_win : nullptr, winner, b_win)) return 1;
        if(x0_new && stage_in(d, dv + o_x0, pin ? pv + o_x0 : nullptr, x0_new, b_x0)) return 1;
        if(u_tail && stage_in(d, dv + o_tail, pin ? pv + o_tail : nullptr, u_tail, b_tail)) return 1;
        if(du && stage_in(d, dv + o_du, pin ? pv + o_du : nullptr, du, b_du)) return 1;
        winner = (const int *)(dv + o_win);
        if(x0_new) x0_new = (const double *)(dv + o_x0);
        if(u_tail) u_tail = (const double *)(dv + o_tail);
        if(du) du = (const double *)(dv + o_du);
    }
    {
        Timed t(d, ILQG_K_SHIFT_WINNERS);
#if ILQG_WAVE_MAP
        hipLaunchKernelGGL(k_shift_winners_wave, dim3(d->B / K), dim3(SHIFT_BLOCK), 0, d->stream, d->P, K, first, winner, steps, x0_new, u_tail, du);
#else
        hipLaunchKernelGGL(k_shift_winners_lane, dim3((unsigned)((size_t)(NX > NU ? NX : NU) * d->Bp / WAVE)), dim3(WAVE * SHIFT_WAVES), 0, d->stream, d->P, K,
                           first, winner, steps, x0_new, u_tail, du);
#endif
    }
    HIP_TRY(hipGetLastError());
#if !ILQG_WAVE_MAP
    if(d->loc_set >= 0) HIP_TRY(hipMemsetAsync(d->P.i[ILQG_I_LOC], 0, d->Bp * sizeof(int), d->stream));
    d->loc_set = -1;
#endif
    return on_device ? 0 : io_done(d);
}

static int launch_head(ilqg_dev_t *d, int steps, double *x, double *u, double *l, double *L, double *cost) {
    const int tiles = (x ? (steps * NX + 7) / 8 : 0) + ((u ? 1 : 0) + (l ? 1 : 0)) * ((steps * NU + 7) / 8) + (L ? (steps * NXU + 7) / 8 : 0);
    const int gy = tiles > 0 ? (tiles + HEAD_WAVES - 1) / HEAD_WAVES : 1;
    {
        Timed t(d, ILQG_K_HEAD);
        hipLaunchKernelGGL(k_head, dim3((unsigned)((d->B + 7) / 8), (unsigned)gy), dim3(WAVE * HEAD_WAVES), 0, d->stream, d->P, steps, x, u, l, L, cost);
    }
    HIP_TRY(hipGetLastError());
    return 0;
}
static int head_steps_ok(ilqg_dev_t *d, int steps) {
    if(steps >= 1 && steps <= d->N) return 1;
    g_err = "head: steps must be in 1 .. n_hor";
    return 0;
}

int ilqg_dev_head_device(ilqg_dev_t *d, int steps, double *x, double *u, double *l, double *L, double *cost) {
    HIP_TRY(hipSetDevice(d->device));
    if(!head_steps_ok(d, steps)) return 1;
    if(!x && !u && !l && !L && !cost) return 0;
    return launch_head(d, steps, x, u, l, L, cost);
}

int ilqg_dev_head(ilqg_dev_t *d, int steps, double *x, double *u, double *l, double *L, double *cost) {
    HIP_TRY(hipSetDevice(d->device));
    if(!head_steps_ok(d, steps)) return 1;
    double *const host[5] = {x, u, l, L, cost};
    const size_t per[5] = {(size_t)steps * NX, (size_t)steps * NU, (size_t)steps * NU, (size_t)steps * NXU, 1};
    size_t off[5], total = 0;
    for(int i = 0; i < 5; i++) {
        off[i] = total;
        if(host[i]) total += ((size_t)d->B * per[i] + 31) & ~(size_t)31;
    }
    if(total == 0) return 0;
    void *dev, *pin;
    if(stage(d, total * sizeof(double), &dev, &pin)) return 1;
    double *dv[5];
// ... 53 lines not shown
    }
    return &map;
}
static int launch_policy(ilqg_dev_t *d, int R, const double *x0, const PolicyParamMap *map, const double *values, int shared, const double *dist,
                         int dist_shared, double alpha, int feedback, double *cost, int *ok, double *x_end, double *x, double *u) {
    if(roll_enter(d)) return 1;
    const dim3 grid = grid1((size_t)d->B * (size_t)R, ROLL_BLOCK);
    {
        Timed t(d, map ? ILQG_K_POLICY_PARAMS : ILQG_K_POLICY, roll_stream(d));
        with_rows(d, [&](auto... tr) {
            with_own_rows(map != nullptr, [&](auto... own) {
                hipLaunchKernelGGL((k_policy<sizeof...(own) != 0, decltype(tr)..., decltype(own)...>), grid, dim3(ROLL_BLOCK), 0, roll_stream(d), d->P, d->O,
                                   d->pv, R, x0, alpha, feedback ? 1 : 0, cost, ok, x_end, x, u, dist, dist_shared ? 1 : 0, tr..., own...);
            }, values, shared ? 1 : 0, map ? *map : PolicyParamMap{});
        });
    }
    HIP_TRY(hipGetLastError());
    return roll_leave(d);
}

static int policy_rollout_staged(ilqg_dev_t *d, int R, const double *x0, const PolicyParamMap *map, const double *values, int shared,
                                 const double *dist, int dist_shared, double alpha, int feedback, double *cost, int *ok, double *x_end, double *x,
                                 double *u) {
    const size_t n = (size_t)d->B * (size_t)R;
    void *const host[5] = {cost, ok, x_end, x, u};
    const size_t bytes[5] = {n * sizeof(double), n * sizeof(int), n * NX * sizeof(double), n * (size_t)(d->N + 1) * NX * sizeof(double),
                             n * (size_t)d->N * NU * sizeof(double)};
    const size_t in_bytes = n * NX * sizeof(double);
    const size_t val_bytes = map ? (shared ? (size_t)R : n) * (size_t)map->W * sizeof(double) : 0;
    const size_t val_off = (in_bytes + 255) & ~(size_t)255;
    const size_t dist_bytes = dist ? (dist_shared ? (size_t)R : n) * (size_t)d->N * NX * sizeof(double) : 0;
    const size_t dist_off = val_off + ((val_bytes + 255) & ~(size_t)255);
    size_t off[5], total = dist_off + ((dist_bytes + 255) & ~(size_t)255);
    for(int i = 0; i < 5; i++) {
        off[i] = total;
        if(host[i]) total += (bytes[i] + 255) & ~(size_t)255;
    }
    void *dev, *pin;
    if(stage(d, total, &dev, &pin)) return 1;
    if(stage_in(d, dev, pin, x0, in_bytes)) return 1;
    if(map && stage_in(d, (char *)dev + val_off, pin ? (char *)pin + val_off : nullptr, values, val_bytes)) return 1;
    if(dist && stage_in(d, (char *)dev + dist_off, pin ? (char *)pin + dist_off : nullptr, dist, dist_bytes)) return 1;
    void *dv[5];
    for(int i = 0; i < 5; i++) dv[i] = host[i] ? (void *)((char *)dev + off[i]) : nullptr;
    if(launch_policy(d, R, (const double *)dev, map, (const double *)((char *)dev + val_off), shared,
                     dist ? (const double *)((char *)dev + dist_off) : nullptr, dist_shared, alpha, feedback, (double *)dv[0], (int *)dv[1],
                     (double *)dv[2], (double *)dv[3], (double *)dv[4]))
        return 1;
    for(int i = 0; i < 5; i++) {
        if(!host[i]) continue;
        void *to = pin ? (void *)((char *)pin + off[i]) : host[i];
        HIP_TRY(hipMemcpyAsync(to, dv[i], bytes[i], hipMemcpyDeviceToHost, d->stream));
        if(pin) d->pending.push_back({host[i], to, bytes[i], 0});
    }
    if(!pin) HIP_TRY(hipStreamSynchronize(d->stream));
    return 0;
}

static int policy_rollout(ilqg_dev_t *d, bool on_host, int R, const double *x0, int n_named, const int *named, const double *values, int shared,
                          const double *dist, int dist_shared, double alpha, int feedback, double *cost, int *ok, double *x_end, double *x,
                          double *u) {
    HIP_TRY(hipSetDevice(d->device));
    NEED_PARAMS(d);
    PolicyParamMap table;
    const PolicyParamMap *map = nullptr;
    if(!policy_args_ok(d, R, x0) || (n_named != 0 && !(map = policy_param_map(n_named, named, values, table)))) return 1;
    if(!cost && !ok && !x_end && !x && !u) return 0;
    return on_host ? policy_rollout_staged(d, R, x0, map, values, shared, dist, dist_shared, alpha, feedback, cost, ok, x_end, x, u)
                   : launch_policy(d, R, x0, map, values, shared, dist, dist_shared, alpha, feedback, cost, ok, x_end, x, u);
}

int ilqg_dev_policy_rollout(ilqg_dev_t *d, int R, const double *x0, int n_named, const int *named, const double *values, int shared,
                            const double *dist, int dist_shared, double alpha, int feedback, double *cost, int *ok, double *x_end, double *x, double *u) {
    return policy_rollout(d, false, R, x0, n_named, named, values, shared, dist, dist_shared, alpha, feedback, cost, ok, x_end, x, u);
}

int ilqg_dev_policy_rollout_host(ilqg_dev_t *d, int R, const double *x0, int n_named, const int *named, const double *values, int shared,
                                 const double *dist, int dist_shared, double alpha, int feedback, double *cost, int *ok, double *x_end, double *x,
                                 double *u) {
    return policy_rollout(d, true, R, x0, n_named, named, values, shared, dist, dist_shared, alpha, feedback, cost, ok, x_end, x, u);
}

int ilqg_dev_put_x0_device(ilqg_dev_t *d, const double *x0) {
    HIP_TRY(hipSetDevice(d->device));
    if(all_home(d)) return 1;
    const size_t n = (size_t)d->B * NX;
    {
        Timed t(d, ILQG_K_TRANSPOSE);
        hipLaunchKernelGGL(k_nom_io, grid1(n, 256), dim3(256), 0, d->stream, d->P.nom, const_cast<double *>(x0), d->B, d->N, 1, NX, NOM_X, 1);
        if(!WAVE_MAP) hipLaunchKernelGGL(k_to_dev, grid1(n, 256), dim3(256), 0, d->stream, x0, d->P.f[ILQG_F_X], d->B, d->Bp, 1, NX, NX);
    }
    HIP_TRY(hipGetLastError());
    return 0;
}

int ilqg_dev_put_u_tail_device(ilqg_dev_t *d, const double *tail, int steps) {
    HIP_TRY(hipSetDevice(d->device));
    if(steps < 1 || steps > d->N) {
        g_err = "ilqg_dev_put_u_tail_device: bad step count";
        return 1;
    }
    if(all_home(d)) return 1;
    {
        Timed t(d, ILQG_K_TRANSPOSE);
        hipLaunchKernelGGL(k_put_u_steps, grid1((size_t)d->B * steps * NU, 256), dim3(256), 0, d->stream, d->P, tail, d->N - steps, steps);
    }
    HIP_TRY(hipGetLastError());
    return 0;
}

int ilqg_dev_stream_in(ilqg_dev_t *d, void *stream) {
    HIP_TRY(hipSetDevice(d->device));
    HIP_TRY(hipEventRecord(d->ext_in, (hipStream_t)stream));
    HIP_TRY(hipStreamWaitEvent(d->stream, d->ext_in, 0));
    return 0;
}
int ilqg_dev_stream_out(ilqg_dev_t *d, void *stream) {
    HIP_TRY(hipSetDevice(d->device));
    HIP_TRY(hipEventRecord(d->ext_out, d->stream));
    HIP_TRY(hipStreamWaitEvent((hipStream_t)stream, d->ext_out, 0));
    return 0;
}

int ilqg_dev_check_device_ptr(ilqg_dev_t *d, const void *ptr, const char *what) {
    HIP_TRY(hipSetDevice(d->device));
    hipPointerAttribute_t a;
    memset(&a, 0, sizeof(a));
    const hipError_t e = hipPointerGetAttributes(&a, ptr);
    if(e != hipSuccess) (void)hipGetLastError();
    if(e != hipSuccess || a.type != hipMemoryTypeDevice || a.device != d->device) {
        g_err = std::string(what) + " must point to device memory on the context's device";
        return 1;
    }
    return 0;
}

int ilqg_dev_shift_param(ilqg_dev_t *d, int index, int steps, const double *tail) {
    HIP_TRY(hipSetDevice(d->device));
    NEED_PARAMS(d);
    constexpr int want[ILQG_NP > 0 ? ILQG_NP : 1] = ILQG_PSIZES;
    if(index < 0 || index >= ILQG_NP || index >= (int)d->param_bufs.size() || want[index] != -1) {
        g_err = "ilqg_dev_shift_param: not a parameter with one value per time step";
        return 1;
    }
    if(steps < 0 || steps > d->N) {
        g_err = "ilqg_dev_shift_param: steps must be in 0 .. n_hor";
        return 1;
    }
    if(steps == 0) return 0;
    const double *tail_dev = nullptr;
    if(tail) {
        void *dev, *pin;
        if(stage(d, (size_t)steps * sizeof(double), &dev, &pin)) return 1;
        if(stage_in(d, dev, pin, tail, (size_t)steps * sizeof(double))) return 1;
        tail_dev = (const double *)dev;
    }
    {
        Timed t(d, ILQG_K_SHIFT_PARAM);
        hipLaunchKernelGGL(k_shift_param, dim3(1), dim3(PARAM_BLOCK), 0, d->stream, d->param_bufs[index].get(), d->N + 1, steps, tail_dev);
    }
    HIP_TRY(hipGetLastError());
    d->work_consts = d->half_consts[0] = d->half_consts[1] = false;
    return tail ? io_done(d) : 0;
}

int ilqg_dev_shift_param_batch(ilqg_dev_t *d, int index, int steps, const double *tail, int on_device) {
    HIP_TRY(hipSetDevice(d->device));
    const int s = step_slot(index);
    if(s < 0 || !d->sr_on[s]) {
        g_err = "ilqg_dev_shift_param_batch: the parameter has no rows per trajectory in this context";
        return 1;
    }
    if(steps < 0 || steps > d->N) {
        g_err = "ilqg_dev_shift_param_batch: steps must be in 0 .. n_hor";
        return 1;
    }
    if(steps == 0) return 0;
    const double *tail_dev = tail;
    if(tail && !on_device) {
        void *dev, *pin;
        const size_t bytes = (size_t)d->B * (size_t)steps * sizeof(double);
        if(stage(d, bytes, &dev, &pin)) return 1;
        if(stage_in(d, dev, pin, tail, bytes)) return 1;
        tail_dev = (const double *)dev;
    }
    {
        Timed t(d, ILQG_K_SHIFT_PARAM_ROWS);
        hipLaunchKernelGGL(k_shift_param_rows, dim3(d->B), dim3(PARAM_BLOCK), 0, d->stream, d->sr_rows[s].get(), d->N + 1, steps, tail_dev);
    }
    HIP_TRY(hipGetLastError());
    return (tail && !on_device) ? io_done(d) : 0;
}

static int slot_index(int s) {
    constexpr int sizes[ILQG_NP > 0 ? ILQG_NP : 1] = ILQG_PSIZES;
    for(int i = 0; i < ILQG_NP; i++)
        if(sizes[i] == -1 && s-- == 0) return i;
    return -1;
}
}
template <int n_slots, class Each>
static int each_future(ilqg_dev_t *d, const double *const *future, Each &&each) {
    if constexpr(n_slots > 0) {
        const size_t per = (size_t)d->loop.rounds * (size_t)d->loop.steps;
        for(int s = 0; s < n_slots; s++) {
            const double *f = future ? future[slot_index(s)] : nullptr;
            if(f && each(s, f, (d->sr_on[s] ? (size_t)d->B : (size_t)1) * per * sizeof(double))) return 1;
        }
    }
    return 0;
}
template <int n_slots>
static int windows_move(ilqg_dev_t *d, int round) {
    if constexpr(n_slots > 0) {
        NEED_PARAMS(d);
        WindowSet<n_slots> S;
        int most = 1;
        for(int s = 0; s < n_slots; s++) {
            const bool rows = d->sr_on[s];
            S.w[s].base = rows ? d->sr_rows[s].get() : d->param_bufs[slot_index(s)].get();
            S.w[s].rows = rows ? d->B : 1;
            S.w[s].future = d->loop.given[s] ? d->win_future[s].get() : nullptr;
            S.w[s].stride = rows ? (size_t)d->loop.rounds * (size_t)d->loop.steps : 0;
            if(S.w[s].rows > most) most = S.w[s].rows;
        }
        {
            Timed t(d, ILQG_K_SHIFT_WINDOWS);
            hipLaunchKernelGGL(k_shift_windows<n_slots>, dim3(most, n_slots), dim3(PARAM_BLOCK), 0, d->stream, S, d->N + 1, d->loop.steps,
                               round * d->loop.steps);
        }
        HIP_TRY(hipGetLastError());
        d->work_consts = d->half_consts[0] = d->half_consts[1] = false;
    }
    return 0;
}
static int loop_close(ilqg_dev_t *d) {
    d->loop.rounds = 0;
    return d->log_x.release() | d->log_u.release() | d->log_c.release() | plant_release(d);
}
static int loop_round_ok(const ilqg_dev_t *d, int round, const char *who) {
    if(round >= 0 && round < d->loop.rounds) return 1;
    g_err = std::string(who) + ": no such round of an open loop (ilqg_dev_loop_begin)";
    return 0;
}
extern "C" {
int ilqg_dev_loop_begin(ilqg_dev_t *d, const ilqg_dev_loop_t *loop) {
    HIP_TRY(hipSetDevice(d->device));
    const ilqg_dev_loop_t &L = *loop;
    const bool windows = L.windows && N_STEP_PARAMS > 0, named = L.plant && L.n_named > 0;
    if(L.rounds < 1 || L.steps < 1 || L.steps >= d->N) {
        g_err = "ilqg_dev_loop_begin: need rounds >= 1 and 1 <= steps < n_hor";
        return 1;
    }
    if(L.plant || windows) NEED_PARAMS(d);
    PolicyParamMap map;
    if(L.plant && L.n_named < 0) {
        g_err = "ilqg_dev_loop_begin: n_names must not be negative";
        return 1;
    }
    if(named && !policy_param_map(L.n_named, L.named, L.values, map)) return 1;
    HIP_TRY(hipStreamSynchronize(d->stream));
    if(L.plant && d->roll) HIP_TRY(hipStreamSynchronize(d->roll));
    d->loop.rounds = L.rounds, d->loop.steps = L.steps, d->loop.plant = L.plant != 0, d->loop.windows = L.windows != 0;
    for(bool &given : d->loop.given) given = false;
    const size_t B = (size_t)d->B, rounds = (size_t)L.rounds, per = B * rounds * (size_t)L.steps;
    if(d->log_x.renew(per * NX * sizeof(double)) || d->log_u.renew(per * NU * sizeof(double)) || d->log_c.renew(B * rounds * sizeof(double)) ||
       (L.plant && (plant_release(d) || d->plant_xp.renew(B * NX * sizeof(double)) || d->plant_failed.renew(B * sizeof(int)) ||
                    d->plant_cost.renew(B * rounds * sizeof(double)) || (named && d->plant_values.renew(B * (size_t)map.W * sizeof(double))) ||
                    (L.disturbance && d->plant_dist.renew(per * NX * sizeof(double))))) ||
       (windows && each_future<N_STEP_PARAMS>(d, L.future, [&](int s, const double *, size_t bytes) {
            d->loop.given[s] = true;
            return d->win_future[s].reserve(bytes);
        }))) {
        (void)loop_close(d);
        return 1;
    }
    bool sent = L.plant != 0;
    if(L.plant) {
        HIP_TRY(hipMemsetAsync(d->plant_failed.get(), 0, B * sizeof(int), d->stream));
        HIP_TRY(hipMemsetAsync(d->log_x.get(), 0, per * NX * sizeof(double), d->stream));
        HIP_TRY(hipMemsetAsync(d->log_u.get(), 0, per * NU * sizeof(double), d->stream));
        HIP_TRY(hipMemsetAsync(d->plant_cost.get(), 0, B * rounds * sizeof(double), d->stream));
        if(named) {
            d->loop.map = map;
            d->loop.named = true;
            HIP_TRY(hipMemcpyAsync(d->plant_values.get(), L.values, B * (size_t)map.W * sizeof(double), hipMemcpyHostToDevice, d->stream));
        }
        if(L.disturbance) HIP_TRY(hipMemcpyAsync(d->plant_dist.get(), L.disturbance, per * NX * sizeof(double), hipMemcpyHostToDevice, d->stream));
        if(L.x_plant) HIP_TRY(hipMemcpyAsync(d->plant_xp.get(), L.x_plant, B * NX * sizeof(double), hipMemcpyHostToDevice, d->stream));
        else if(launch_head(d, 1, d->plant_xp.get(), nullptr, nullptr, nullptr, nullptr)) return 1;
    }
    if(windows && each_future<N_STEP_PARAMS>(d, L.future, [&](int s, const double *f, size_t bytes) {
           HIP_TRY(hipMemcpyAsync(d->win_future[s].get(), f, bytes, hipMemcpyHostToDevice, d->stream));
           sent = true;
           return 0;
       }))
        return 1;
    if(sent) HIP_TRY(hipStreamSynchronize(d->stream));
    return 0;
}

int ilqg_dev_loop_apply(ilqg_dev_t *d, int round, int feedback) {
    HIP_TRY(hipSetDevice(d->device));
    if(!loop_round_ok(d, round, "ilqg_dev_loop_apply")) return 1;
    const int steps = d->loop.steps, rounds = d->loop.rounds;
    if(!d->loop.plant) {
        {
            Timed t(d, ILQG_K_LOG);
            hipLaunchKernelGGL(k_log_steps, grid1((size_t)d->B * steps * (NX + NU), 256), dim3(256), 0, d->stream, d->P, d->log_x.get(), d->log_u.get(),
                               d->log_c.get(), round, rounds, steps);
        }
        HIP_TRY(hipGetLastError());
        return 0;
    }
    NEED_PARAMS(d);
    if(roll_enter(d)) return 1;
    {
        Timed t(d, ILQG_K_PLANT, roll_stream(d));
        with_rows(d, [&](auto... tr) {
            with_own_rows(d->loop.named, [&](auto... own) {
                hipLaunchKernelGGL((k_plant<sizeof...(own) != 0, decltype(tr)..., decltype(own)...>), grid1((size_t)d->B, ROLL_BLOCK), dim3(ROLL_BLOCK), 0,
                                   roll_stream(d), d->P, d->O, d->pv, steps, feedback ? 1 : 0, d->plant_xp.get(), d->plant_failed.get(),
                                   (const double *)d->plant_dist.get(), round * steps, rounds * steps, round, rounds, d->log_x.get(), d->log_u.get(),
                                   d->plant_cost.get(), d->log_c.get(), tr..., own...);
            }, (const double *)d->plant_values.get(), d->loop.map);
        });
    }
    HIP_TRY(hipGetLastError());
    return roll_leave(d);
}

int ilqg_dev_loop_shift(ilqg_dev_t *d, int round) {
    HIP_TRY(hipSetDevice(d->device));
    if(!loop_round_ok(d, round, "ilqg_dev_loop_shift")) return 1;
    if(d->loop.windows && windows_move<N_STEP_PARAMS>(d, round)) return 1;
    if(ilqg_dev_shift(d, d->loop.steps, !d->loop.plant)) return 1;
    return d->loop.plant ? ilqg_dev_put_x0_device(d, d->plant_xp.get()) : 0;
}

int ilqg_dev_loop_read(ilqg_dev_t *d, double *x_plant, double *x, double *u, double *cost_applied, double *plan_cost, int *ok) {
    HIP_TRY(hipSetDevice(d->device));
    if(d->loop.rounds < 1 || ((x_plant || cost_applied || ok) && !d->loop.plant)) {
        g_err = "ilqg_dev_loop_read: no loop, or none with plants (ilqg_dev_loop_begin)";
        return 1;
    }
    const size_t B = (size_t)d->B, rounds = (size_t)d->loop.rounds, per = B * rounds * (size_t)d->loop.steps;
    if(x_plant) HIP_TRY(hipMemcpyAsync(x_plant, d->plant_xp.get(), B * NX * sizeof(double), hipMemcpyDeviceToHost, d->stream));
    if(cost_applied) HIP_TRY(hipMemcpyAsync(cost_applied, d->plant_cost.get(), B * rounds * sizeof(double), hipMemcpyDeviceToHost, d->stream));
    if(ok) HIP_TRY(hipMemcpyAsync(ok, d->plant_failed.get(), B * sizeof(int), hipMemcpyDeviceToHost, d->stream));
    if(x) HIP_TRY(hipMemcpyAsync(x, d->log_x.get(), per * NX * sizeof(double), hipMemcpyDeviceToHost, d->stream));
    if(u) HIP_TRY(hipMemcpyAsync(u, d->log_u.get(), per * NU * sizeof(double), hipMemcpyDeviceToHost, d->stream));
    if(plan_cost) HIP_TRY(hipMemcpyAsync(plan_cost, d->log_c.get(), B * rounds * sizeof(double), hipMemcpyDeviceToHost, d->stream));
    HIP_TRY(hipStreamSynchronize(d->stream));
    if(ok)
        for(size_t b = 0; b < B; b++) ok[b] = ok[b] ? 0 : 1;
    return 0;
}

#if ILQG_WAVE_MAP

static int spec_sweeps_at_most(const ilqg_dev_opts_t &O) {
    double lam = 0.0, dlam = 0.0;
    int sweeps = 1;
    while(sweeps <= 4096) {
        lambda_up(O.lambdaFactor, O.lambdaMin, &lam, &dlam);
        if(lam > O.lambdaMax || !(lam == lam)) break;
        sweeps++;
    }
    return sweeps;
}

struct WorkPlan {
    SharedWork *shared;
    bool fact, quad;
    char *work;
    size_t stride;
    int chunk;
    bool split;
    int half_cap, part, pieces;
    bool *whole, *half;
};

static int work_plan(ilqg_dev_t *d, int do_derivs, int do_backward, WorkPlan &w) {
    w.shared = do_derivs && do_backward ? d->shared : nullptr;
    w.fact = FACTORED && d->O.fuse_derivs && w.shared;
    w.stride = w.fact ? FACT_STRIDE : (w.shared ? STORED_STRIDE : sizeof(trajEl_t));
    if(w.shared) {
        w.work = reinterpret_cast<char *>(w.shared->buf);
        const size_t fit = (w.shared->bytes - sizeof(trajEl_t)) / ((size_t)d->N * w.stride);
        w.chunk = (int)(fit > (size_t)d->B ? (size_t)d->B : fit);
        if(w.chunk < 1) {
            g_err = "the device's derivative work buffer does not hold one trajectory of this horizon";
            return 1;
        }
    } else {
        if(own_work(d)) return 1;
        w.work = reinterpret_cast<char *>(d->P.work);
        w.chunk = d->B;
    }
    w.quad = QUAD_STEP && d->O.regType == 1 && (w.fact || !FULL || d->env.quad_stored) && !d->env.no_quad;
    w.split = w.shared && w.chunk >= 2 && (d->B > w.chunk || (d->B >= 16 * d->cus && (!w.quad || d->env.two_pieces)));
    w.half_cap = w.split ? w.chunk / 2 : w.chunk;
    w.pieces = (d->B + w.half_cap - 1) / w.half_cap;
    w.part = w.chunk;
    if(w.split) {
        w.part = ((d->B + w.pieces - 1) / w.pieces + 7) / 8 * 8;
        if(w.part > w.half_cap) w.part = w.half_cap;
    }
    w.whole = &d->work_consts, w.half = d->half_consts;
    if(w.shared) {
        SharedWork *W = w.shared;
        const bool same = W->pv_set && W->N == d->N && W->B == d->B && W->part == w.part && W->half_cap == w.half_cap &&
                          W->factored == w.fact && !d->per_step_params && memcmp(&W->pv, &d->pv, sizeof(ParamValues)) == 0;
        if(!same) {
            W->whole = W->half[0] = W->half[1] = false;
// ... 23 lines not shown
           Timed t(d, ILQG_K_DERIVS, q);
           hipLaunchKernelGGL(k.fn, k.grid((size_t)cnt * (d->N + 1), d->cus), dim3(k.block), k.lds, q, P, d->O, d->pv, c0, cnt, have_consts ? 0 : 1,
                              limit_gradients, 0);
       }))
        return 1;
    if(cnt == w.part) {
        if(w.split) w.half[h] = true;
        else *w.whole = w.half[0] = w.half[1] = true;
    }
    return 0;
}

static int spec_rows(ilqg_dev_t *d, int cnt, hipStream_t st) {
    const int rows = (int)sweep_kernel(d, false, true, true).grid((size_t)cnt, d->cus).x * 4 * QUAD_WAVES;
    const int ri = d->spec_ints.try_reserve(((size_t)(3 + SPEC_ATTEMPTS) * d->B + rows) * sizeof(unsigned), st);
    const int rd = ri ? ri : d->spec_doubles.try_reserve((size_t)rows * (SPEC_SLOTS + (size_t)d->N * SPEC_GW) * sizeof(double), st);
    return rd == 0 ? rows : (rd == 2 ? 0 : -1);
}
static void spec_point(ilqg_dev_t *d, DevPtrs &P, int rows, hipStream_t q) {
    unsigned *w = d->spec_ints.get();
    const size_t nb = (size_t)d->B;
    P.spec_word = w;
    P.spec_done = w + nb;
    P.spec_out = w + 2 * nb;
    P.spec_best = w + (2 + SPEC_ATTEMPTS) * nb;
    P.spec_row_b = reinterpret_cast<int *>(w + (3 + SPEC_ATTEMPTS) * nb);
    P.spec_res = d->spec_doubles.get();
    P.spec_gains = d->spec_doubles.get() + (size_t)rows * SPEC_SLOTS;
    P.spec_rows = rows;
    g_spec_last = d;
    (void)hipMemsetAsync(w, 0, (2 + SPEC_ATTEMPTS) * nb * sizeof(unsigned), q);
    (void)hipMemsetAsync(P.spec_best, 0xff, (nb + (size_t)rows) * sizeof(unsigned), q);
}

static int launch_sweep(ilqg_dev_t *d, const WorkPlan &w, DevPtrs &P, hipStream_t st, int single_sweep, int c0, int cnt) {
    HIP_TRY(hipMemsetAsync(P.queue, 0, sizeof(int), st));
    bool spec = w.quad && d->env.quad_spec && !single_sweep && !w.split && c0 == 0 && cnt == d->B;
    if(spec && spec_sweeps_at_most(d->O) > SPEC_ATTEMPTS) spec = false;
    const int rows = spec ? spec_rows(d, cnt, st) : 0;
    if(rows < 0) return 1;
    const auto &k = sweep_kernel(d, w.fact, w.quad, rows > 0);
    return on_scratch_stream(d, k.scratch, st, [&](hipStream_t q) {
        Timed t(d, ILQG_K_BACKWARD, q);
        if(rows) spec_point(d, P, rows, q);
        hipLaunchKernelGGL(k.fn, k.grid((size_t)cnt, d->cus), dim3(k.block), k.lds, q, P, d->O, single_sweep, c0, cnt);
    });
}

static int wave_backward(ilqg_dev_t *d, int single_sweep, int do_derivs, int do_backward) {
    WorkPlan w;
    if(work_plan(d, do_derivs, do_backward, w)) return 1;
    if(w.shared) HIP_TRY(hipStreamWaitEvent(d->stream, w.shared->free_ev, 0));
    if(w.split) {
        HIP_TRY(hipEventRecord(d->fork, d->stream));
        HIP_TRY(hipStreamWaitEvent(d->stream2, d->fork, 0));
    }
    int piece = 0;
    for(int c0 = 0; c0 < d->B; c0 += w.part, piece++) {
        const int cnt = (d->B - c0 < w.part) ? d->B - c0 : w.part;
        const int h = w.split ? (piece & 1) : 0;
        hipStream_t st = h ? d->stream2 : d->stream;
        DevPtrs P = d->P;
        P.work = reinterpret_cast<trajEl_t *>(w.work + (size_t)h * w.half_cap * d->N * w.stride);
        P.work_stride = w.stride;
        P.queue = d->queues.get() + h * QUEUE_CELL;
        if(do_derivs && launch_derivs(d, w, P, st, h, c0, cnt)) return 1;
        if(do_backward && launch_sweep(d, w, P, st, single_sweep, c0, cnt)) return 1;
    }
    if(do_derivs) {
        if(w.split) w.half[0] = w.half[1] = true;
        else *w.whole = w.half[0] = w.half[1] = true;
    }
    if(w.split) {
        HIP_TRY(hipEventRecord(d->join, d->stream2));
        HIP_TRY(hipStreamWaitEvent(d->stream, d->join, 0));
    }
    if(w.shared) HIP_TRY(hipEventRecord(w.shared->free_ev, d->stream));
    HIP_TRY(hipGetLastError());
    return 0;
}
#endif

int ilqg_dev_derivs(ilqg_dev_t *d) {
    NEED_PARAMS(d);
    HIP_TRY(hipSetDevice(d->device));
#if ILQG_WAVE_MAP
    return wave_backward(d, 0, 1, 0);
#else
    {
        Timed t(d, ILQG_K_DERIVS);
        const size_t total = (size_t)d->Bp * (d->N + 1);
        LAUNCH_TWIN(d, k_derivs, grid1(total, 256), dim3(256), 0, d->stream, d->P, d->O, d->pv);
    }
    HIP_TRY(hipGetLastError());
    return 0;
#endif
}

int ilqg_dev_backward(ilqg_dev_t *d, int mode) {
    HIP_TRY(hipSetDevice(d->device));
    if(mode < 0 || mode > 2) {
        g_err = "ilqg_dev_backward: mode must be 0, 1 or 2";
        return 1;
    }
    if(mode == 2) NEED_PARAMS(d);

#if ILQG_WAVE_MAP
    return wave_backward(d, mode == 1, mode == 2, 1);
#else
    {
        Timed t(d, mode == 2 ? ILQG_K_BACKWARD_FUSED : ILQG_K_BACKWARD);
        const dim3 grid(d->Bp / WAVE), block(WAVE);
        if(mode == 0)
            with_rows(d, [&](auto... tr) { hipLaunchKernelGGL((k_backward<0, decltype(tr)...>), grid, block, 0, d->stream, d->P, d->O, d->pv, tr...); });
        else if(mode == 1)
            with_rows(d, [&](auto... tr) { hipLaunchKernelGGL((k_backward<1, decltype(tr)...>), grid, block, 0, d->stream, d->P, d->O, d->pv, tr...); });
#if ILQG_HAVE_SPLIT
        else if(d->O.bw_split && !HAS_MUL && !d->rows_on)
            hipLaunchKernelGGL(k_backward_split, grid, dim3(2 * WAVE), 0, d->stream, d->P, d->O, d->pv);
#endif
        else
            with_rows(d, [&](auto... tr) { hipLaunchKernelGGL((k_backward<2, decltype(tr)...>), grid, block, 0, d->stream, d->P, d->O, d->pv, tr...); });
    }
    if(mode != 2) {
        Timed t(d, ILQG_K_TRANSPOSE);
        hipLaunchKernelGGL(k_pack_records, dim3(d->Bp / WAVE, (d->N + 1 + PACK_WAVES - 1) / PACK_WAVES),
                           dim3(WAVE * PACK_WAVES), 0, d->stream, d->P);
    }
    HIP_TRY(hipGetLastError());
    return 0;
#endif
}

static void launch_select(ilqg_dev_t *d, hipStream_t rs, int a0, int a1, int second) {
    Timed t(d, ILQG_K_SELECT, rs);
    hipLaunchKernelGGL(k_select, grid1(d->Bp, 256), dim3(256), 0, rs, d->P, d->O, a0, a1, second);
}
static int reserve_kept(ilqg_dev_t *d, double *&view, Buffer<double> &owner, int n_alpha, hipStream_t rs) {
    return repoint(view, owner, owner.reserve((size_t)d->Bp * n_alpha * (d->N + 1) * CAND_W * sizeof(double), rs));
}

#if !ILQG_WAVE_MAP
}
template <int STAGE>
static void launch_search_stage(ilqg_dev_t *d, hipStream_t rs, int a0, int n, int set) {
    Timed t(d, STAGE ? ILQG_K_SEARCH2 : ILQG_K_SEARCH, rs);
    const int T = WAVE / n;
    const dim3 grid((d->B + T - 1) / T), block(WAVE);
    if(T * (RN / 2) <= WAVE * DMA_LOADS && !d->env.no_dma)
        with_rows(d, [&](auto... tr) { hipLaunchKernelGGL((k_search<STAGE, true, decltype(tr)...>), grid, block, 2 * T * RN * sizeof(double), rs, d->P, d->O, d->pv, a0, n, set, tr...); });
    else
        with_rows(d, [&](auto... tr) { hipLaunchKernelGGL((k_search<STAGE, false, decltype(tr)...>), grid, block, 0, rs, d->P, d->O, d->pv, a0, n, set, tr...); });
}
extern "C" {

static int search_kept_planes(ilqg_dev_t *d, int A, int s1) {
    hipStream_t rs = roll_stream(d);
    const size_t xplane = (size_t)(d->N + 1) * NX * d->Bp, uplane = (size_t)d->N * NU * d->Bp;
    if(d->P.plane_n != s1) {
        if(all_home(d)) return 1;
        d->P.plane_n = s1;
    }
    const int rx = repoint(d->P.xpl, d->xpl, d->xpl.try_reserve(2 * (size_t)s1 * xplane * sizeof(double), rs));
    const int ru = rx ? rx : repoint(d->P.upl, d->upl, d->upl.try_reserve(2 * (size_t)s1 * uplane * sizeof(double), rs));
    if(rx == 1 || ru == 1) return 1;
    if(rx == 2 || ru == 2) {
        if(repoint(d->P.xpl, d->xpl, d->xpl.release())) return 1;
        d->loc_set = -1;
        HIP_TRY(hipMemsetAsync(d->P.i[ILQG_I_LOC], 0, d->Bp * sizeof(int), d->stream));
        return 2;
    }
    const int n2 = A - s1, set = (d->loc_set == 0) ? 1 : 0;
    d->P.xplane = xplane;
    d->P.uplane = uplane;
    if(n2 > 0 && reserve_kept(d, d->P.cand, d->cand, n2, rs)) return 1;
    if(!d->pending_zero) HIP_TRY(hipMemsetAsync(d->P.n_pending, 0, sizeof(int), rs));
    d->pending_zero = false;
    launch_search_stage<0>(d, rs, 0, s1, set);
    if(n2 > 0) {
        launch_search_stage<1>(d, rs, s1, n2, set);
        Timed t(d, ILQG_K_ADOPT, rs);
        hipLaunchKernelGGL(k_adopt_home, dim3(8 * d->cus), dim3(256), 0, rs, d->P, s1);
    } else {
        Timed t(d, ILQG_K_ADOPT, rs);
        hipLaunchKernelGGL(k_rejected_home, dim3(8 * d->cus), dim3(256), 0, rs, d->P);
    }
    if(d->defer_commit) {
        d->commit_pending = true;
        d->commit_s1 = s1;
        d->commit_set = set;
    } else {
        Timed t(d, ILQG_K_ADOPT, rs);
        hipLaunchKernelGGL(k_commit, grid1(d->Bp, 256), dim3(256), 0, rs, d->P, s1, set);
    }
    d->loc_set = set;
    d->winner_done = true;
    HIP_TRY(hipGetLastError());
    return 0;
}
#endif

#if ILQG_WAVE_MAP && defined(ILQG_ROLLOUT_PARTS)
static int search_rollout_parts(ilqg_dev_t *d, int A, int s1) {
    hipStream_t rs = roll_stream(d);
    const int n2 = A - s1;
    if(reserve_kept(d, d->P.cand1, d->cand1, s1, rs)) return 1;
    if(n2 > 0 && reserve_kept(d, d->P.cand, d->cand, n2, rs)) return 1;
    d->keep_first = true;
    launch_rollout(d, ROLL_SEARCH, ILQG_K_ROLLOUT_SEARCH, 0, s1, rs);
    d->keep_first = false;
    launch_select(d, rs, 0, s1, 0);
    if(n2 > 0) {
        launch_rollout(d, ROLL_LIST_KEEP, ILQG_K_ROLLOUT_SEARCH2, s1, n2, rs);
        launch_select(d, rs, s1, A, 1);
        Timed t(d, ILQG_K_ROLLOUT_WINNER, rs);
        hipLaunchKernelGGL(k_adopt, dim3(8 * d->cus), dim3(256), 0, rs, d->P, s1, n2);
    }
    {
        Timed t(d, ILQG_K_ROLLOUT_WINNER, rs);
        hipLaunchKernelGGL(k_adopt_first, dim3(16 * d->cus), dim3(256), 0, rs, d->P, s1);
    }
    d->winner_done = true;
    return 0;
}
#endif

static int search_plain(ilqg_dev_t *d, int A, int s1) {
    hipStream_t rs = roll_stream(d);
    launch_rollout(d, ROLL_SEARCH, ILQG_K_ROLLOUT_SEARCH, 0, s1, rs);
    launch_select(d, rs, 0, s1, 0);
    d->winner_done = false;
    if(s1 < A && !d->O.ls_keep) {
        launch_rollout(d, ROLL_SEARCH_LIST, ILQG_K_ROLLOUT_SEARCH2, s1, A - s1, rs);
        launch_select(d, rs, s1, A, 1);
    } else if(s1 < A) {
        const int n2 = A - s1;
        if(reserve_kept(d, d->P.cand, d->cand, n2, rs)) return 1;
        launch_rollout(d, ROLL_SECOND, ILQG_K_ROLLOUT_SEARCH2, s1, n2 + 1, rs);
        launch_select(d, rs, s1, A, 1);
        Timed t(d, ILQG_K_ROLLOUT_WINNER, rs);
        hipLaunchKernelGGL(k_adopt, dim3(8 * d->cus), dim3(256), 0, rs, d->P, s1, n2);
        d->winner_done = true;
    }
    return 0;
}

int ilqg_dev_search(ilqg_dev_t *d) {
    NEED_PARAMS(d);
    HIP_TRY(hipSetDevice(d->device));
    const int A = d->O.n_alpha;
    const int s1 = (d->O.ls_split > 0 && d->O.ls_split < A) ? d->O.ls_split : A;
#if !ILQG_WAVE_MAP
    if(d->O.ls_keep >= 2 && s1 <= PLANE_A && WAVE / s1 >= 1 && (A == s1 || WAVE / (A - s1) >= 1)) {
        const int rc = search_kept_planes(d, A, s1);
        if(rc != 2) return rc;
    }
    if(all_home(d)) return 1;
#endif
    if(roll_enter(d)) return 1;
    HIP_TRY(hipMemsetAsync(d->P.n_pending, 0, sizeof(int), roll_stream(d)));
    d->pending_zero = false;
    bool parts = false;
#if ILQG_WAVE_MAP && defined(ILQG_ROLLOUT_PARTS)
    parts = d->O.ls_keep >= 2 && !HAS_MUL && !d->env.no_rollout_parts;
    if(parts && search_rollout_parts(d, A, s1)) return 1;
#endif
    if(!parts && search_plain(d, A, s1)) return 1;
    HIP_TRY(hipGetLastError());
    return roll_leave(d);
}

static void launch_history(ilqg_dev_t *d, hipStream_t stream);
static void launch_move_history(ilqg_dev_t *dst, ilqg_dev_t *src, const int *to, const int *from, int count);
static void launch_harvest(ilqg_dev_t *d, const HarvestPlan &plan, const int *from);

int ilqg_dev_winner(ilqg_dev_t *d) {
    NEED_PARAMS(d);
    HIP_TRY(hipSetDevice(d->device));
    if(d->winner_done) {
        d->winner_done = false;
        return 0;
    }
    if(roll_enter(d)) return 1;
    launch_rollout(d, ROLL_WINNER, ILQG_K_ROLLOUT_WINNER, 0, 1, roll_stream(d));
    HIP_TRY(hipGetLastError());
    return roll_leave(d);
}

int ilqg_dev_update(ilqg_dev_t *d) {
    NEED_PARAMS(d);
    HIP_TRY(hipSetDevice(d->device));
    hipStream_t rs = roll_stream(d);
    if(roll_enter(d)) return 1;
    if(d->hist.cap > 0) {
        Timed t(d, ILQG_K_HISTORY, rs);
        launch_history(d, rs);
    }
    {
        Timed t(d, ILQG_K_UPDATE, rs);
        const int reset = (!WAVE_MAP && d->defer_commit) ? 1 : 0;
        hipLaunchKernelGGL(k_update, grid1(d->Bp, 256), dim3(256), 0, rs, d->P, d->O, d->commit_pending ? d->commit_s1 : -1, d->commit_set, reset);
        d->commit_pending = false;
        d->pending_zero = reset != 0;
    }
    if(HAS_MUL) {
        Timed t(d, ILQG_K_MULTIPLIERS, rs);
        LAUNCH_TWIN(d, k_multipliers, dim3(d->Bp / WAVE), dim3(WAVE), 0, rs, d->P, d->O, d->pv, 0);
    }
    if(d->O.resweep || HAS_MUL) launch_rollout(d, ROLL_COST, ILQG_K_ROLLOUT_COST, 0, 1, rs);
    HIP_TRY(hipGetLastError());
    return roll_leave(d);
}

int ilqg_dev_iterate(ilqg_dev_t *d, int n) {
    struct Defer {
        ilqg_dev_t *d;
        explicit Defer(ilqg_dev_t *d_) : d(d_) { d->defer_commit = true; }
        ~Defer() { d->defer_commit = false; }
    } defer(d);
    for(int it = 0; it < n; it++) {
        if(d->O.fuse_derivs || WAVE_MAP) {
            if(ilqg_dev_backward(d, 2)) return 1;
        } else {
            if(ilqg_dev_derivs(d)) return 1;
            if(ilqg_dev_backward(d, 0)) return 1;
        }
        if(ilqg_dev_search(d)) return 1;
        if(ilqg_dev_winner(d)) return 1;
        if(ilqg_dev_update(d)) return 1;
    }
    return 0;
}

int ilqg_dev_move(ilqg_dev_t *dst, ilqg_dev_t *src, int count, const int *to, const int *from, int with_records) {
    if(count < 1) return 0;
    if(dst->device != src->device || dst->N != src->N) {
        g_err = "ilqg_dev_move: the two contexts differ in device or horizon";
        return 1;
    }
    HIP_TRY(hipSetDevice(dst->device));
    for(int j = 0; j < count; j++)
        if(to[j] < 0 || to[j] >= dst->B || from[j] < 0 || from[j] >= src->B) {
            g_err = "ilqg_dev_move: trajectory index out of range";
            return 1;
        }
    HIP_TRY(hipStreamSynchronize(src->stream));
    if(io_flush(dst)) return 1;
    if(dst->staging.reserve(2 * (size_t)count * sizeof(int))) return 1;
    int *idx = reinterpret_cast<int *>(dst->staging.get());
    HIP_TRY(hipMemcpyAsync(idx, to, (size_t)count * sizeof(int), hipMemcpyHostToDevice, dst->stream));
    HIP_TRY(hipMemcpyAsync(idx + count, from, (size_t)count * sizeof(int), hipMemcpyHostToDevice, dst->stream));
    hipLaunchKernelGGL(k_move_traj, grid1((size_t)count * (src->N + 1), 256), dim3(256), 0, dst->stream, dst->P, src->P, idx, idx + count, count,
                       (with_records && !WAVE_MAP) ? 1 : 0);
    HIP_TRY(hipGetLastError());
    if(src->pb_on) {
        const size_t W = (size_t)src->pb_map.W, bytes = (size_t)dst->B * W * sizeof(double);
        bool same = dst->pb_on && dst->pb_map.W == src->pb_map.W;
        for(int j = 0; same && j < ILQG_PTOTAL; j++) same = dst->pb_map.src[j] == src->pb_map.src[j];
        if(!same) {
            if(table_buffer(dst, bytes)) return 1;
            HIP_TRY(hipMemsetAsync(dst->pb_values.get(), 0, bytes, dst->stream));
            dst->pb_map = src->pb_map;
            dst->pb_on = true;
        }
        rows_refresh(dst);
        hipLaunchKernelGGL(k_move_rows, grid1((size_t)count * W, 256), dim3(256), 0, dst->stream, dst->pb_values.get(), (const double *)src->pb_values.get(), idx,
                           idx + count, count, (int)W);
        HIP_TRY(hipGetLastError());
    }
    for(int s = 0; s < N_STEP_PARAMS; s++) {
        if(!src->sr_on[s]) continue;
        const size_t W = (size_t)src->N + 1;
        if(!dst->sr_on[s]) {
            if(step_rows_buffer(dst, s)) return 1;
            HIP_TRY(hipMemsetAsync(dst->sr_rows[s].get(), 0, (size_t)dst->B * W * sizeof(double), dst->stream));
            dst->sr_on[s] = true;
            rows_refresh(dst);
        }
        hipLaunchKernelGGL(k_move_rows, grid1((size_t)count * W, 256), dim3(256), 0, dst->stream, dst->sr_rows[s].get(), (const double *)src->sr_rows[s].get(), idx,
                           idx + count, count, (int)W);
        HIP_TRY(hipGetLastError());
    }
    if(src->hist.cap > 0) {
        if(dst->hist.cap == 0 && ilqg_dev_set_history(dst, src->hist.cap)) return 1;
        launch_move_history(dst, src, idx, idx + count, count);
        HIP_TRY(hipGetLastError());
    }
    HIP_TRY(hipStreamSynchronize(dst->stream));
    return 0;
}

int ilqg_dev_harvest(ilqg_dev_t *d, int count, const int *from, const ilqg_dev_harvest_t *what, int *words, int *offsets) {
    if(count < 1) return 0;
    HIP_TRY(hipSetDevice(d->device));
    if(!from || !what || !words || !offsets) {
        g_err = "ilqg_dev_harvest: from, what, words or offsets is NULL";
        return 1;
    }
    for(int j = 0; j < count; j++)
        if(from[j] < 0 || from[j] >= d->B) {
            g_err = "ilqg_dev_harvest: trajectory index out of range";
            return 1;
        }
    if(what->n_hist < 0 || what->n_hist > HARVEST_FIELDS || (what->n_hist > 0 && (!what->hist_int || !what->hist_field))) {
        g_err = "ilqg_dev_harvest: n_hist = " + std::to_string(what->n_hist) + ", must be 0 .. " + std::to_string(HARVEST_FIELDS) + " fields, each with its kind and index";
        return 1;
    }
    if(what->n_hist > 0 && d->hist.cap == 0) {
        g_err = "ilqg_dev_harvest: the context has no history (ilqg_dev_set_history with cap > 0 switches one on)";
        return 1;
    }
    HarvestPlan plan = {};
    plan.count = count, plan.n_hist = what->n_hist;
    int w = 2;
    plan.ox = what->x ? w : -1;
    w += what->x ? (d->N + 1) * NX : 0;
    plan.ou = what->u ? w : -1;
    w += what->u ? d->N * NU : 0;
    offsets[0] = plan.ox, offsets[1] = plan.ou;
    for(int i = 0; i < what->n_hist; i++) {
        const int f = what->hist_field[i], is_int = what->hist_int[i];
        if(is_int ? (f != ILQG_HI_N && (f < 0 || f >= ILQG_HI_COUNT)) : (f < 0 || f >= HIST_DOUBLES)) {
            g_err = "ilqg_dev_harvest: no such history field (w_pen_l / w_pen_f are recorded in libraries of problems with multipliers only)";
// ... 194 lines not shown
    HIP_TRY(hipSetDevice(d->device));
    if(drain_spans(d)) return 1;
    if(enable)
        while(d->event_pool.size() < 1024) {
            hipEvent_t e = nullptr;
            HIP_TRY(hipEventCreate(&e));
            d->event_pool.push_back(e);
        }
    d->timing = enable != 0;
    memset(d->t_ms, 0, sizeof(d->t_ms));
    memset(d->t_n, 0, sizeof(d->t_n));
    memset(d->t_busy, 0, sizeof(d->t_busy));
    if(enable) {
        if(!d->epoch) HIP_TRY(hipEventCreate(&d->epoch));
        HIP_TRY(hipEventRecord(d->epoch, d->stream));
    }
    return 0;
}

int ilqg_dev_get_busy(ilqg_dev_t *d, int kernel, double *busy_ms) {
    if(kernel < 0 || kernel >= ILQG_K_TOTAL) {
        g_err = "ilqg_dev_get_busy: bad kernel id";
        return 1;
    }
    if(drain_spans(d)) return 1;
    *busy_ms = d->t_busy[kernel];
    return 0;
}

int ilqg_dev_get_timing(ilqg_dev_t *d, int kernel, int *launches, double *total_ms) {
    if(kernel < 0 || kernel >= ILQG_K_TOTAL) {
        g_err = "ilqg_dev_get_timing: bad kernel id";
        return 1;
    }
    if(drain_spans(d)) return 1;
    *launches = d->t_n[kernel];
    *total_ms = d->t_ms[kernel];
    return 0;
}

int ilqg_dev_dense(int device, int op, int shape, const double *in0, int n_in0, const double *in1, int n_in1,
                   const double *in2, int n_in2, double *out, int n_out, int *flag) {
    HIP_TRY(hipSetDevice(device));
    Buffer<double> d0, d1, d2, dout;
    Buffer<int> dflag;
    if(d0.reserve((n_in0 > 0 ? n_in0 : 1) * 8) || d1.reserve((n_in1 > 0 ? n_in1 : 1) * 8) || d2.reserve((n_in2 > 0 ? n_in2 : 1) * 8) ||
       dout.reserve((n_out > 0 ? n_out : 1) * 8) || dflag.reserve(4))
        return 1;
    if(n_in0 > 0) HIP_TRY(hipMemcpy(d0.get(), in0, n_in0 * 8, hipMemcpyHostToDevice));
    if(n_in1 > 0) HIP_TRY(hipMemcpy(d1.get(), in1, n_in1 * 8, hipMemcpyHostToDevice));
    if(n_in2 > 0) HIP_TRY(hipMemcpy(d2.get(), in2, n_in2 * 8, hipMemcpyHostToDevice));
    HIP_TRY(hipMemcpy(dout.get(), out, n_out * 8, hipMemcpyHostToDevice));
    hipLaunchKernelGGL(k_dense_test, dim3(1), dim3(64), 0, 0, op, shape, 0, 0, d0.get(), d1.get(), d2.get(), dout.get(), dflag.get());
    HIP_TRY(hipGetLastError());
    HIP_TRY(hipDeviceSynchronize());
    HIP_TRY(hipMemcpy(out, dout.get(), n_out * 8, hipMemcpyDeviceToHost));
    HIP_TRY(hipMemcpy(flag, dflag.get(), 4, hipMemcpyDeviceToHost));
    return 0;
}

int ilqg_dev_sincos_batch(int device, int n, const double *x, double *s, double *c) {
    HIP_TRY(hipSetDevice(device));
    Buffer<double> dx, ds, dc;
    if(dx.reserve(n * 8) || ds.reserve(n * 8) || dc.reserve(n * 8)) return 1;
    HIP_TRY(hipMemcpy(dx.get(), x, n * 8, hipMemcpyHostToDevice));
    hipLaunchKernelGGL(k_sincos_test, grid1(n, 256), dim3(256), 0, 0, n, dx.get(), ds.get(), dc.get());
    HIP_TRY(hipGetLastError());
    HIP_TRY(hipDeviceSynchronize());
    HIP_TRY(hipMemcpy(s, ds.get(), n * 8, hipMemcpyDeviceToHost));
    HIP_TRY(hipMemcpy(c, dc.get(), n * 8, hipMemcpyDeviceToHost));
    return 0;
}

static void launch_history(ilqg_dev_t *d, hipStream_t stream) {
    hipLaunchKernelGGL(k_history<>, grid1(d->Bp, 256), dim3(256), 0, stream, d->P, d->hist);
}
static void launch_move_history(ilqg_dev_t *dst, ilqg_dev_t *src, const int *to, const int *from, int count) {
    hipLaunchKernelGGL(k_move_history<>, grid1((size_t)count * dst->hist.cap, 256), dim3(256), 0, dst->stream, dst->hist, src->hist, to, from, count);
}
static void launch_harvest(ilqg_dev_t *d, const HarvestPlan &plan, const int *from) {
    hipLaunchKernelGGL(k_harvest<>, dim3((unsigned)((plan.count + HARVEST_WAVES - 1) / HARVEST_WAVES), (unsigned)((plan.W + WAVE - 1) / WAVE)),
                       dim3(WAVE * HARVEST_WAVES), 0, d->stream, d->P, d->hist, plan, from, d->harvest.get());
}

static int boxqp_batch(int rows, int device, int n, int count, const double *H, const double *g, const double *lower,
                       const double *upper, double *x, int *clamp, int *n_free, double *invH, int *rc, const int *active = nullptr) {
    if(n != 2 && n != 8 && n != NU) {
        g_err = "ilqg_dev_boxqp_batch: n must be 2, 8 or N_U";
        return 1;
    }
    if(rows == 3) {
#if ILQG_WAVE_MAP
        if(n != 2 && n != NU) {
            g_err = "ilqg_dev_boxqp_quad_batch: n must be 2 or N_U";
            return 1;
        }
#else
        g_err = "ilqg_dev_boxqp_quad_batch: the quad form is compiled into the libraries of the wave mapping only (N_X > 8, lib*_wave.so)";
        return 1;
#endif
    }
    HIP_TRY(hipSetDevice(device));
    const size_t T = n * (n + 1) / 2;
    Buffer<double> oH, oinv, og, olo, oup, ox;
    Buffer<int> ocl, onf, orc, oact;
    if(oH.reserve(count * T * 8) || oinv.reserve(count * T * 8) || og.reserve(count * n * 8) || olo.reserve(count * n * 8) ||
       oup.reserve(count * n * 8) || ox.reserve(count * n * 8) || ocl.reserve(count * n * 4) || onf.reserve(count * 4) || orc.reserve(count * 4))
        return 1;
    double *const dH = oH.get(), *const dinv = oinv.get(), *const dg = og.get(), *const dlo = olo.get(), *const dup = oup.get(), *const dx = ox.get();
    int *const dcl = ocl.get(), *const dnf = onf.get(), *const drc = orc.get();
    HIP_TRY(hipMemcpy(dH, H, count * T * 8, hipMemcpyHostToDevice));
    HIP_TRY(hipMemcpy(dg, g, count * n * 8, hipMemcpyHostToDevice));
    HIP_TRY(hipMemcpy(dlo, lower, count * n * 8, hipMemcpyHostToDevice));
    HIP_TRY(hipMemcpy(dup, upper, count * n * 8, hipMemcpyHostToDevice));
    HIP_TRY(hipMemcpy(dx, x, count * n * 8, hipMemcpyHostToDevice));
    const dim3 grid = rows == 1 ? dim3(count) : (rows == 3 ? grid1(count, 4) : grid1(count, 64)), block(64);
#if ILQG_WAVE_MAP
    if(rows == 3) {
        if(oact.reserve(count * 4)) return 1;
        int *const dact = oact.get();
        const std::vector<int> every(count, 1);
        HIP_TRY(hipMemcpy(dact, active ? active : every.data(), count * 4, hipMemcpyHostToDevice));
        if(n == NU)
            hipLaunchKernelGGL(k_boxqp_quad_test<NU>, grid, block, 0, 0, count, dact, dH, dg, dlo, dup, dx, dcl, dnf, dinv, drc);
        else
            hipLaunchKernelGGL(k_boxqp_quad_test<2>, grid, block, 0, 0, count, dact, dH, dg, dlo, dup, dx, dcl, dnf, dinv, drc);
    } else
#endif
#if ILQG_EXPERIMENTS
    if(rows == 2 && n == 2)
        hipLaunchKernelGGL((k_boxqp_test<2, true>), grid, block, 0, 0, count, dH, dg, dlo, dup, dx, dcl, dnf, dinv, drc);
    else if(rows == 2 && n == NU)
        hipLaunchKernelGGL((k_boxqp_test<NU, true>), grid, block, 0, 0, count, dH, dg, dlo, dup, dx, dcl, dnf, dinv, drc);
    else if(rows == 2) {
        g_err = "ilqg_dev_boxqp_table_batch: n must be 2 or N_U";
        return 1;
    } else
#else
    if(rows == 2) {
        g_err = "ilqg_dev_boxqp_table_batch: the pattern-table form is compiled into the -DILQG_EXPERIMENTS libraries only (lib*_exp.so)";
        return 1;
    } else
#endif
    if(rows && n == 2)
        hipLaunchKernelGGL(k_boxqp_rows_test<2>, grid, block, 0, 0, count, dH, dg, dlo, dup, dx, dcl, dnf, dinv, drc);
    else if(rows && n == 8)
        hipLaunchKernelGGL(k_boxqp_rows_test<8>, grid, block, 0, 0, count, dH, dg, dlo, dup, dx, dcl, dnf, dinv, drc);
    else if(rows)
        hipLaunchKernelGGL(k_boxqp_rows_test<NU>, grid, block, 0, 0, count, dH, dg, dlo, dup, dx, dcl, dnf, dinv, drc);
    else if(n == 2)
        hipLaunchKernelGGL(k_boxqp_test<2>, grid, block, 0, 0, count, dH, dg, dlo, dup, dx, dcl, dnf, dinv, drc);
    else if(n == 8)
        hipLaunchKernelGGL(k_boxqp_test<8>, grid, block, 0, 0, count, dH, dg, dlo, dup, dx, dcl, dnf, dinv, drc);
    else
        hipLaunchKernelGGL(k_boxqp_test<NU>, grid, block, 0, 0, count, dH, dg, dlo, dup, dx, dcl, dnf, dinv, drc);
    HIP_TRY(hipGetLastError());
    HIP_TRY(hipDeviceSynchronize());
    HIP_TRY(hipMemcpy(x, dx, count * n * 8, hipMemcpyDeviceToHost));
    HIP_TRY(hipMemcpy(invH, dinv, count * T * 8, hipMemcpyDeviceToHost));
    HIP_TRY(hipMemcpy(clamp, dcl, count * n * 4, hipMemcpyDeviceToHost));
    HIP_TRY(hipMemcpy(n_free, dnf, count * 4, hipMemcpyDeviceToHost));
    HIP_TRY(hipMemcpy(rc, drc, count * 4, hipMemcpyDeviceToHost));
    return 0;
}

int ilqg_dev_boxqp_batch(int device, int n, int count, const double *H, const double *g, const double *lower,
// ... 121 lines not shown
```

### ddp-generator_amd/csrc/k_lane_backward.inc

```
template <class F>
__device__ __forceinline__ int derivs_step(trajEl_t &t, multipliersEl_t *m, Callbacks &C, ilqg_hooks &H, int k, int N,
                                           F &&overlapped) {
    double x[NX], u[NU];
#pragma unroll
    for(int i = 0; i < NX; i++) x[i] = t.x[i];
#pragma unroll
    for(int i = 0; i < NU; i++) u[i] = t.u[i];
    const double nf0 = H.nonfinite;
    H.huge = 0.0;
    int ok = 1;
    auto body = [&]() {
        ok = calcXVariableAux(&t, m, k, &C.o);
        ok &= calcXUVariableAux(&t, m, k, &C.o);
        ok &= calcLAuxDeriv(&t, m, k, &C.o);
        ok &= bp_derivsL(&t, k, C.o.p);
        limitsU(&t, k, C.o.p, N);
    };
    body();
    overlapped();
    if(H.huge != 0.0) {
#pragma unroll
        for(int i = 0; i < NX; i++) t.x[i] = x[i];
#pragma unroll
        for(int i = 0; i < NU; i++) t.u[i] = u[i];
// ... 90 lines not shown
        load_mul_fin(P, b, mf);
        init_final(&fin, &C.o);
        const double *xs = cur_x(P, P.N, b);
#pragma unroll
        for(int i = 0; i < NX; i++) fin.x[i] = xs[i * XSI];

        ok = derivs_final(fin, HAS_MUL ? &mf : nullptr, C, H, P.N);
        double *out = P.f[ILQG_F_FIN] + ix(P, FIN, 1, 0, 0, b);
        PUT(0, fin.cx, NX)
        PUT(NX, fin.cxx, SXX)
#undef PUT
    }
    if(!ok || H.nonfinite != 0.0) P.derivs_failed[b] = 1;
}
__global__ __launch_bounds__(256) void k_derivs(DevPtrs P, ilqg_dev_opts_t O, ParamValues A) { derivs_lane(P, O, A); }
template <class... Rows>
__global__ __launch_bounds__(256) void k_derivs_rows(DevPtrs P, ilqg_dev_opts_t O, ParamValues A, Rows... rows) {
    derivs_lane(P, O, A, rows...);
}

__device__ __forceinline__ void load_record(double *dst, double *udst, const double *src, const double *us) {
#pragma unroll
    for(int i = 0; i < REC; i++) dst[i] = src[i * SI];
#pragma unroll
    for(int i = 0; i < NU; i++) udst[i] = us[i * XSI];
}

template <int CS = 1>
__device__ __forceinline__ void store_gains(const double *l, const double *K, double *lo, double *ko) {
#pragma unroll
    for(int i = 0; i < NU; i++) lo[i * CS] = l[i];
#pragma unroll
    for(int i = 0; i < NXU; i++) ko[i * CS] = K[i];
}

__device__ __forceinline__ int backward_sweep(const DevPtrs &P, int b, double lambda, int regType, double &dV0,
                                              double &dV1, double &g_norm) {
    const int N = P.N;
    double Vx[NX], Vxx[SXX], l[NU], K[NXU];
    const double *fin = P.f[ILQG_F_FIN] + ix(P, FIN, 1, 0, 0, b);
#pragma unroll
    for(int i = 0; i < NX; i++) Vx[i] = fin[i * SI];
#pragma unroll
    for(int i = 0; i < SXX; i++) Vxx[i] = fin[(NX + i) * SI];
#pragma unroll
    for(int i = 0; i < NU; i++) l[i] = 0.0;
    dV0 = 0.0;
    dV1 = 0.0;
    double gsum = 0.0;

    const double *rp = P.f[ILQG_F_DER] + ix(P, REC, N, N - 1, 0, b);
    const double *up = cur_u(P, N - 1, b);
    double *lo = WAVE_MAP ? nomp(P, N - 1, b) + NOM_L : P.f[ILQG_F_LG] + ix(P, NU, N, N - 1, 0, b);
    double *ko = WAVE_MAP ? nomp(P, N - 1, b) + NOM_K : P.f[ILQG_F_KG] + ix(P, NXU, N, N - 1, 0, b);
    const size_t rs = step_stride(P, REC), us = cur_ustride(P);
    const size_t ls = WAVE_MAP ? (size_t)RN : step_stride(P, NU), ks = WAVE_MAP ? (size_t)RN : step_stride(P, NXU);

    double cur[REC], ucur[NU];
    load_record(cur, ucur, rp, up);
    int failed = 0;
    drain_memory_ops();
    for(int k = N - 1; k >= 0; k--) {
        double nxt[REC], unxt[NU];
        if(k > 0) load_record(nxt, unxt, rp - rs, up - us);
        const int rc = back_step<NX, NU, FULL, HX>(cur, ucur, Vx, Vxx, l, K, lambda, regType, dV0, dV1, gsum);
        store_gains<XSI>(l, K, lo, ko);
        if(BOXQP_FAILED(rc)) {
            failed = 1;
            break;
        }
        rp -= rs;
        up -= us;
        lo -= ls;
        ko -= ks;
#pragma unroll
        for(int i = 0; i < REC; i++) cur[i] = nxt[i];
#pragma unroll
        for(int i = 0; i < NU; i++) ucur[i] = unxt[i];
    }
    if(!failed) g_norm = gsum / ((double)(N - 1));
    return failed;
}

__device__ __forceinline__ int backward_sweep_fused(const DevPtrs &P, Callbacks &C, ilqg_hooks &H, int b, double lambda, int regType,
                                                    double &dV0, double &dV1, double &g_norm) {
    const int N = P.N;
    H.nonfinite = 0.0;
    const double *xp = cur_x(P, N, b);
    const double *up = cur_u(P, N - 1, b);
    double *rec_k = nomp(P, N - 1, b);
    const size_t xs = cur_xstride(P), us = cur_ustride(P);

    double Vx[NX], Vxx[SXX], l[NU], K[NXU];
    {
        trajFin_t fin;
        init_final(&fin, &C.o);
#pragma unroll
        for(int i = 0; i < NX; i++) fin.x[i] = xp[i * XSI];
        if(!WAVE_MAP) {
            double *recN = nomp(P, N, b);
#pragma unroll
            for(int i = 0; i < NX; i++) recN[NOM_X + i] = fin.x[i];
        }
        multipliersFin_t mf;
        load_mul_fin(P, b, mf);
        const int ok = derivs_final(fin, HAS_MUL ? &mf : nullptr, C, H, N);
        if(!ok || H.nonfinite != 0.0) return 2;
#pragma unroll
        for(int i = 0; i < NX; i++) Vx[i] = fin.cx[i];
#pragma unroll
        for(int i = 0; i < SXX; i++) Vxx[i] = fin.cxx[i];
    }
    xp -= xs;
#pragma unroll
    for(int i = 0; i < NU; i++) l[i] = 0.0;
    dV0 = 0.0;
    dV1 = 0.0;
    double gsum = 0.0;

    trajEl_t t;
    init_running(&t, &C.o1);
    double xk[NX], uk[NU];
    double cur[REC];
#define GETF(off, arr, cnt) _Pragma("unroll") for(int i = 0; i < (cnt); i++) rec[(off) + i] = (arr)[i];
    auto record_of = [&](const double *xv, const double *uv, int k, double *rec, auto &&overlapped) {
#pragma unroll
        for(int i = 0; i < NX; i++) t.x[i] = xv[i];
#pragma unroll
        for(int i = 0; i < NU; i++) t.u[i] = uv[i];
        multipliersEl_t m;
        load_mul(P, k, b, m);
        const int ok = derivs_step(t, HAS_MUL ? &m : nullptr, C, H, k, N, overlapped);
        REC_COPY(GETF, t)
        return ok;
    };
    {
#pragma unroll
        for(int i = 0; i < NX; i++) xk[i] = xp[i * XSI];
#pragma unroll
        for(int i = 0; i < NU; i++) uk[i] = up[i * XSI];
        const int ok = record_of(xk, uk, N - 1, cur, [] {});
        if(!ok || H.nonfinite != 0.0) return 2;
    }
    double xn[NX], un[NU];
#pragma unroll
    for(int i = 0; i < NX; i++) xn[i] = (xp - xs)[i * XSI];
#pragma unroll
    for(int i = 0; i < NU; i++) un[i] = (up - us)[i * XSI];
    int result = 0;
#ifdef ILQG_PROFILE_SECTIONS
    Prof prof;
    prof.start();
    Prof *pf = &prof;
#else
    Prof *pf = nullptr;
#endif
    drain_memory_ops();
    for(int k = N - 1; k >= 0; k--) {
        if(pf) pf->probe(7);
        double xnn[NX], unn[NU];
        const int back = (k > 1) ? 2 : k;
#pragma unroll
        for(int i = 0; i < NX; i++) xnn[i] = (xp - back * xs)[i * XSI];
#pragma unroll
        for(int i = 0; i < NU; i++) unn[i] = (up - back * us)[i * XSI];
        if(pf) pf->probe(0);
        const int rc = back_step<NX, NU, FULL, HX, RecZeros>(cur, uk, Vx, Vxx, l, K, lambda, regType, dV0, dV1, gsum, pf);
        double nxt[REC];
        const int ok = record_of(xn, un, (k > 0) ? k - 1 : 0, nxt, [&] {
#pragma unroll
            for(int i = 0; i < NX; i++) pin(Vx[i]);
#pragma unroll
            for(int i = 0; i < SXX; i++) pin(Vxx[i]);
            pin(dV0);
            pin(dV1);
            pin(gsum);
        });
        if(!ok || H.nonfinite != 0.0) {
            result = 2;
            break;
        }
        if(pf) pf->probe(6);
        store_gains(l, K, rec_k + NOM_L, rec_k + NOM_K);
        if(!WAVE_MAP) {
#pragma unroll
            for(int i = 0; i < NX; i++) rec_k[NOM_X + i] = xk[i];
#pragma unroll
            for(int i = 0; i < NU; i++) rec_k[NOM_U + i] = uk[i];
        }
        if(BOXQP_FAILED(rc)) {
            result = 1;
            break;
        }
#pragma unroll
        for(int i = 0; i < REC; i++) cur[i] = nxt[i];
        xp -= xs;
        up -= us;
        rec_k -= RN;
#pragma unroll
        for(int i = 0; i < NX; i++) xk[i] = xn[i];
#pragma unroll
        for(int i = 0; i < NU; i++) uk[i] = un[i];
#pragma unroll
        for(int i = 0; i < NX; i++) xn[i] = xnn[i];
#pragma unroll
        for(int i = 0; i < NU; i++) un[i] = unn[i];
    }
#undef GETF
    if(!result) g_norm = gsum / ((double)(N - 1));
#ifdef ILQG_PROFILE_SECTIONS
    if((threadIdx.x & 63) == 0)
        for(int i = 0; i < 8; i++) atomicAdd(&ilqg_prof_cycles[i], (unsigned long long)prof.acc[i]);
#endif
    return result;
}

template <int mode, class... Rows>
__global__ __launch_bounds__(WAVE, 1)
void k_backward(DevPtrs P, ilqg_dev_opts_t O, ParamValues A, Rows... rows) {
    constexpr bool PER_TRAJECTORY = RowPack<OWN_NONE, Rows...>::has_trajectory_rows;
    const Place place(1);
    const int b = blockIdx.x * WAVE + threadIdx.x;
    if(b >= P.B) return;
    if(P.i[ILQG_I_STATUS][b] != ILQG_ST_ACTIVE) return;
    const int single_sweep = (mode == 1);
    P.i[ILQG_I_NEED_DERIVS][b] = 0;
    if(P.derivs_failed[b]) {
        P.i[ILQG_I_STATUS][b] = ILQG_ST_DERIVS_FAILED;
        return;
    }
    ILQG_CALLBACKS_IN(C, H, VECTOR_PARAMS && !PER_TRAJECTORY && mode == 2);
    apply_rows<OWN_NONE>(C_values, C_table, P, b, 0, 0, rows...);
    load_penalty_weights_der(C, P, b);
    double lambda = P.f[ILQG_F_LAMBDA][b], dlambda = P.f[ILQG_F_DLAMBDA][b];
    double dV0 = 0.0, dV1 = 0.0, g_norm = P.f[ILQG_F_GNORM][b];
    int calls = 0, rc;
    for(;;) {
        if(mode == 2)
            rc = backward_sweep_fused(P, C, H, b, lambda, O.regType, dV0, dV1, g_norm);
        else
            rc = backward_sweep(P, b, lambda, O.regType, dV0, dV1, g_norm);
        calls++;
        if(single_sweep || rc != 1) break;
        lambda_up(O.lambdaFactor, O.lambdaMin, &lambda, &dlambda);
        if(lambda > O.lambdaMax) break;
    }
    const int status = back_status(rc, g_norm, lambda, dlambda, single_sweep, O);
    store_result(P, b, {status, lambda, dlambda, dV0, dV1, g_norm, calls, rc});
}

#if defined(ILQG_TIME_VARYING) && !ILQG_STATE_DEPENDENT_LIMITS && ILQG_EXPERIMENTS
#define ILQG_HAVE_SPLIT 1
#define ILQG_COUNT_ENTRY(member, index) +1
constexpr int SPLIT_VARY = 0 ILQG_TIME_VARYING(ILQG_COUNT_ENTRY) ILQG_TIME_VARYING_FULL(ILQG_COUNT_ENTRY);
constexpr int SPLIT_SLOT = SPLIT_VARY + NX + NU + 1;

__global__ __launch_bounds__(2 * WAVE) void k_backward_split(DevPtrs P, ilqg_dev_opts_t O, ParamValues A) {
    __shared__ double ring[2][SPLIT_SLOT][WAVE];
    __shared__ int ctl[3];
    const int role = threadIdx.x >> 6, lane = threadIdx.x & 63;
    const int b = blockIdx.x * WAVE + lane;
    const int N = P.N;
    const bool mine = b < P.B && P.i[ILQG_I_STATUS][b] == ILQG_ST_ACTIVE;
    if(__builtin_amdgcn_ballot_w64(mine) == 0ull) return;
    ILQG_CALLBACKS(C, H);
    const size_t xs = cur_xstride(P), us = cur_ustride(P);

    if(role == 1) {
        trajEl_t t;
        init_running(&t, &C.o1);
        for(;;) {
            H.nonfinite = 0.0;
            const double *xp = cur_x(P, N - 1, b), *up = cur_u(P, N - 1, b);
            double xn[NX], un[NU];
#pragma unroll
            for(int i = 0; i < NX; i++) xn[i] = xp[i * XSI];
#pragma unroll
            for(int i = 0; i < NU; i++) un[i] = up[i * XSI];
            for(int k = N - 1; k >= 0; k--) {
                double xnn[NX], unn[NU];
                const int back = (k > 0) ? 1 : 0;
#pragma unroll
                for(int i = 0; i < NX; i++) xnn[i] = (xp - back * xs)[i * XSI];
#pragma unroll
                for(int i = 0; i < NU; i++) unn[i] = (up - back * us)[i * XSI];
#pragma unroll
                for(int i = 0; i < NX; i++) t.x[i] = xn[i];
#pragma unroll
                for(int i = 0; i < NU; i++) t.u[i] = un[i];
                const int ok = derivs_step(t, nullptr, C, H, k, N, [] {});
                double(*slot)[WAVE] = ring[k & 1];
                int j = 0;
#define ILQG_PUT_ENTRY(member, index) slot[j++][lane] = t.member[index];
                ILQG_TIME_VARYING(ILQG_PUT_ENTRY) ILQG_TIME_VARYING_FULL(ILQG_PUT_ENTRY)
#undef ILQG_PUT_ENTRY
#pragma unroll
                for(int i = 0; i < NX; i++) slot[SPLIT_VARY + i][lane] = xn[i];
#pragma unroll
                for(int i = 0; i < NU; i++) slot[SPLIT_VARY + NX + i][lane] = un[i];
                slot[SPLIT_VARY + NX + NU][lane] = (!ok || H.nonfinite != 0.0) ? 1.0 : 0.0;
                __syncthreads();
                if(k < N - 1 && !ctl[(k + 1) & 1]) break;
                xp -= back * xs;
                up -= back * us;
#pragma unroll
                for(int i = 0; i < NX; i++) xn[i] = xnn[i];
#pragma unroll
                for(int i = 0; i < NU; i++) un[i] = unn[i];
            }
            __syncthreads();
            if(!ctl[2]) break;
        }
        return;
    }

    load_penalty_weights_der(C, P, b);
    if(mine) P.i[ILQG_I_NEED_DERIVS][b] = 0;
    const bool dead = mine && P.derivs_failed[b];
    bool sweeping = mine && !dead;
    double lambda = mine ? P.f[ILQG_F_LAMBDA][b] : 1.0, dlambda = mine ? P.f[ILQG_F_DLAMBDA][b] : 1.0;
    double dV0 = 0.0, dV1 = 0.0, g_norm = mine ? P.f[ILQG_F_GNORM][b] : 0.0;
    int calls = 0, rc = 0;
    const bool took_part = sweeping;
    trajEl_t t;
    init_running(&t, &C.o1);
    for(;;) {
        bool in_sweep = sweeping;
        int result = 0;
        double Vx[NX], Vxx[SXX], l[NU], K[NXU], gsum = 0.0;
        H.nonfinite = 0.0;
        if(in_sweep) {
            const double *xp = cur_x(P, N, b);
// ... 152 lines not shown
```

### ddp-generator_amd/csrc/k_lane_search.inc

```
constexpr int DMA_LOADS = 3;
template <int stage, bool DMA, class... Rows>
__global__ __launch_bounds__(WAVE, 1)
void k_search(DevPtrs P, ilqg_dev_opts_t O, ParamValues A, int a0, int n, int set, Rows... rows) {
    constexpr bool PER_TRAJECTORY = RowPack<OWN_NONE, Rows...>::has_trajectory_rows;
    extern __shared__ __attribute__((aligned(16))) double s_rec[];
    const Place place(2 + stage);
    const int lane = threadIdx.x;
    const int T = WAVE / n;
    int a = lane / T;
    const int t = lane - a * T;
    const bool used = a < n;
    if(!used) a = n - 1;
    const int count = stage ? *P.n_pending : P.B;
    if((int)blockIdx.x * T >= count) return;
    const int e = blockIdx.x * T + t;
    const int ee = e < count ? e : count - 1;
    const int b = stage ? P.pending[ee] : ee;
    const bool live = used && e < count && P.i[ILQG_I_STATUS][b] == ILQG_ST_ACTIVE;
    if(__builtin_amdgcn_ballot_w64(live) == 0ull) return;
    const int N = P.N;
    const int ai = a0 + a;
    const double alpha = O.alpha[ai];
    const bool feedback = (alpha != 0.0);

    ILQG_CALLBACKS_IN(C, H, VECTOR_PARAMS && !PER_TRAJECTORY && DMA);
    apply_rows<OWN_NONE>(C_values, C_table, P, b, 0, 0, rows...);
    load_penalty_weights(C, P, b);
    trajEl_t ct;
    multipliersEl_t mk;
    multipliersEl_t *const mp = HAS_MUL ? &mk : nullptr;
    init_running(&ct, &C.o1);

    NomPtrs q;
    q.x = nomp(P, 0, b) + NOM_X;
    q.u = nomp(P, 0, b) + NOM_U;
    q.l = nomp(P, 0, b) + NOM_L;
    q.K = nomp(P, 0, b) + NOM_K;
    constexpr int PIECES = RN / 2;
    const double *dsrc[DMA_LOADS];
    bool dact[DMA_LOADS];
    if(DMA) {
#pragma unroll
        for(int m = 0; m < DMA_LOADS; m++) {
            const int qq = m * WAVE + lane;
            const int j = qq / T, r = qq - j * T;
            dact[m] = qq < T * PIECES;
            const int br = __shfl(b, r < T ? r : 0);
            dsrc[m] = nomp(P, 0, br) + 2 * (j < PIECES ? j : 0);
        }
    }
    auto dma_issue = [&](int buf) {
#pragma unroll
        for(int m = 0; m < DMA_LOADS; m++) {
            if(dact[m])
                __builtin_amdgcn_global_load_lds((const __attribute__((address_space(1))) void *)dsrc[m],
                                                 (__attribute__((address_space(3))) void *)(s_rec + (size_t)buf * T * RN + m * WAVE * 2),
                                                 16, 0, 0);
            dsrc[m] += RN;
        }
    };
    auto dma_read = [&](NomStep &c, int buf) {
        double rec[RN];
        const double *base = s_rec + (size_t)buf * T * RN + 2 * t;
#pragma unroll
        for(int j = 0; j < PIECES; j++) {
            rec[2 * j] = base[(size_t)j * T * 2];
            rec[2 * j + 1] = base[(size_t)j * T * 2 + 1];
        }
#pragma unroll
        for(int i = 0; i < NX; i++) c.x[i] = rec[NOM_X + i];
#pragma unroll
        for(int i = 0; i < NU; i++) c.u[i] = rec[NOM_U + i];
#pragma unroll
        for(int i = 0; i < NU; i++) c.l[i] = rec[NOM_L + i];
#pragma unroll
        for(int i = 0; i < NXU; i++) c.K[i] = rec[NOM_K + i];
    };
    double *kx, *ku;
    const size_t kxs = stage ? (size_t)CAND_W * P.Bp : cur_xstride(P), kus = stage ? kxs : cur_ustride(P);
    const size_t kcs = stage ? (size_t)P.Bp : (size_t)XSI;
    if(stage) {
        kx = P.cand + (size_t)a * (N + 1) * CAND_W * P.Bp + ee;
        ku = kx + (size_t)NX * P.Bp;
    } else {
        const int plane = set * P.plane_n + a;
        kx = P.xpl + (size_t)plane * P.xplane + ix(P, NX, N + 1, 0, 0, b);
        ku = P.upl + (size_t)plane * P.uplane + ix(P, NU, N, 0, 0, b);
    }

    double xc[NX];
#pragma unroll
    for(int i = 0; i < NX; i++) xc[i] = q.x[i];
    double csum = 0.0;
    int okc = 1;
    NomStep cur;
    if(DMA) {
        dma_issue(0);
        asm volatile("s_waitcnt vmcnt(0)" ::: "memory");
        dma_issue(1);
    } else {
        load_nominal<true, 1>(cur, q);
    }
    drain_memory_ops();
    for(int k = 0; k < N; k++) {
        NomPtrs qn;
        qn.x = q.x + RN;
        qn.u = q.u + RN;
        qn.l = q.l + RN;
        qn.K = q.K + RN;
        if(DMA) dma_read(cur, k & 1);
        double xin[NX], uin[NU];
#pragma unroll
        for(int i = 0; i < NX; i++) xin[i] = xc[i];
        {
            double uf[NU];
#pragma unroll
            for(int j = 0; j < NU; j++) uf[j] = cur.u[j] + cur.l[j] * alpha;
#pragma unroll
            for(int i = 0; i < NX; i++) {
                const double dx = xin[i] - cur.x[i];
#pragma unroll
                for(int j = 0; j < NU; j++) uf[j] += cur.K[j + i * NU] * dx;
            }
#pragma unroll
            for(int j = 0; j < NU; j++) uin[j] = feedback ? uf[j] : cur.u[j];
        }
        if(!DMA) load_nominal<true, 1>(cur, qn);
        if(HAS_MUL) load_mul(P, k, b, mk);
        double xnext[NX];
        auto step = ILQG_FORWARD_STEP(false, ct, mp, k, N, C, xin, uin, xnext);
        const int r = run_step(H, okc, step);
        okc &= r;
        csum += ct.c;
        if(DMA) {
            asm volatile("s_waitcnt vmcnt(0)" ::: "memory");
        }
        if(live) {
#pragma unroll
            for(int i = 0; i < NX; i++) kx[i * kcs] = ct.x[i];
#pragma unroll
            for(int i = 0; i < NU; i++) ku[i * kcs] = ct.u[i];
        }
        if(DMA && k + 2 <= N) dma_issue(k & 1);
        kx += kxs;
        ku += kus;
#pragma unroll
        for(int i = 0; i < NX; i++) xc[i] = xnext[i];
        q = qn;
    }
    {
        trajFin_t cf;
        multipliersFin_t mf;
        if(HAS_MUL) load_mul_fin(P, b, mf);
        init_final(&cf, &C.o);
        auto fin = [&]() {
#pragma unroll
            for(int i = 0; i < NX; i++) cf.x[i] = xc[i];
            int r = calcFVariableAux(&cf, HAS_MUL ? &mf : nullptr, &C.o);
            r &= ddpF(&cf, &C.o);
            return r;
        };
        const int r = run_step(H, okc, fin);
        okc &= r;
        csum += cf.c;
        if(live) {
#pragma unroll
            for(int i = 0; i < NX; i++) kx[i * kcs] = cf.x[i];
        }
    }
    const int ok = (okc && H.nonfinite == 0.0) ? 1 : 0;
    if(live) {
        P.f[ILQG_F_ALPHA_COST][tile_ix(ILQG_MAX_ALPHA, ai, b)] = csum;
        P.i[ILQG_I_ALPHA_OK][(size_t)ai * P.Bp + b] = ok;
    }

    const double cost = P.f[ILQG_F_COST][b], dV0 = P.f[ILQG_F_DV0][b], dV1 = P.f[ILQG_F_DV1][b];
    const double my_dcost = cost - csum;
    const double my_expected = expected_reduction(alpha, dV0, dV1);
    const double my_z = reduction_ratio(my_dcost, my_expected);
    const int my_pass = (ok && my_z > O.zMin) ? 1 : 0;
    double cnew = (a0 > 0) ? P.f[ILQG_F_NEW_COST][b] : 0.0;
    double dcost = P.f[ILQG_F_DCOST][b], expected = P.f[ILQG_F_EXPECTED][b];
    int win = -1;
    for(int i = 0; i < n; i++) {
        const int src = i * T + t;
        const int ok_i = __shfl(ok, src);
        const int pass_i = __shfl(my_pass, src);
        const double cnew_i = __shfl(csum, src);
        const double dcost_i = __shfl(my_dcost, src);
        const double expected_i = __shfl(my_expected, src);
        if(win < 0) {
            cnew = cnew_i;
            if(ok_i) {
                dcost = dcost_i;
                expected = expected_i;
                if(pass_i) win = i;
            }
        }
    }
    const bool leader = live && lane < T;
    if(leader) {
        P.i[ILQG_I_ALPHA_IDX][b] = (win >= 0 ? a0 + win : a0 + n) + 1;
        P.i[ILQG_I_ACCEPTED][b] = win >= 0 ? 1 : 0;
        P.f[ILQG_F_NEW_COST][b] = cnew;
        P.f[ILQG_F_DCOST][b] = dcost;
        P.f[ILQG_F_EXPECTED][b] = expected;
    }
    const bool more = leader && win < 0 && stage == 0 && a0 + n < O.n_alpha;
    const unsigned long long m = __builtin_amdgcn_ballot_w64(more);
    if(m != 0ull) {
        int base = 0;
        const int first = __builtin_ctzll(m);
        if(lane == first) base = atomicAdd(P.n_pending_next, __builtin_popcountll(m));
        base = __shfl(base, first);
        if(more) P.pending[base + __builtin_popcountll(m & ((1ull << lane) - 1ull))] = b;
    }
}

__global__ void k_adopt_home(DevPtrs P, int s1) {
    const size_t stride = (size_t)gridDim.x * blockDim.x;
    const int np = *P.n_pending, N1 = P.N + 1;
    const size_t total2 = (size_t)N1 * np;
    for(size_t w = (size_t)blockIdx.x * blockDim.x + threadIdx.x; w < total2; w += stride) {
        const int e = (int)(w % np), k = (int)(w / np);
        const int b = P.pending[e];
        if(P.i[ILQG_I_STATUS][b] != ILQG_ST_ACTIVE) continue;
        double *xo = home_x(P, k, b);
        if(P.i[ILQG_I_ACCEPTED][b]) {
            const int a = P.i[ILQG_I_ALPHA_IDX][b] - 1 - s1;
            const double *src = P.cand + ((size_t)a * N1 + k) * CAND_W * P.Bp + e;
#pragma unroll
            for(int i = 0; i < NX; i++) xo[i * XSI] = src[(size_t)i * P.Bp];
            if(k < P.N) {
                double *uo = home_u(P, k, b);
#pragma unroll
                for(int i = 0; i < NU; i++) uo[i * XSI] = src[(size_t)(NX + i) * P.Bp];
            }
        } else if(P.i[ILQG_I_LOC][b]) {
            const double *xs = cur_x(P, k, b);
#pragma unroll
            for(int i = 0; i < NX; i++) xo[i * XSI] = xs[i * XSI];
            if(k < P.N) {
                const double *us = cur_u(P, k, b);
                double *uo = home_u(P, k, b);
#pragma unroll
                for(int i = 0; i < NU; i++) uo[i * XSI] = us[i * XSI];
            }
        }
    }
}

__global__ void k_rejected_home(DevPtrs P) {
    const size_t total = (size_t)(P.N + 1) * P.Bp, stride = (size_t)gridDim.x * blockDim.x;
    for(size_t w = (size_t)blockIdx.x * blockDim.x + threadIdx.x; w < total; w += stride) {
        const int b = (int)(w % P.Bp), k = (int)(w / P.Bp);
        if(b >= P.B || P.i[ILQG_I_STATUS][b] != ILQG_ST_ACTIVE || P.i[ILQG_I_ACCEPTED][b] || !P.i[ILQG_I_LOC][b]) continue;
        const double *xs = cur_x(P, k, b);
        double *xo = home_x(P, k, b);
#pragma unroll
        for(int i = 0; i < NX; i++) xo[i * XSI] = xs[i * XSI];
        if(k < P.N) {
            const double *us = cur_u(P, k, b);
            double *uo = home_u(P, k, b);
#pragma unroll
            for(int i = 0; i < NU; i++) uo[i * XSI] = us[i * XSI];
        }
    }
}

__global__ void k_commit(DevPtrs P, int s1, int set) {
    const int b = blockIdx.x * blockDim.x + threadIdx.x;
    if(b >= P.B || P.i[ILQG_I_STATUS][b] != ILQG_ST_ACTIVE) return;
    const int a = P.i[ILQG_I_ALPHA_IDX][b] - 1;
    if(P.i[ILQG_I_ACCEPTED][b])
        P.i[ILQG_I_LOC][b] = (a < s1) ? 1 + set * P.plane_n + a : 0;
    else
        P.i[ILQG_I_LOC][b] = 0;
}

__global__ void k_all_home(DevPtrs P) {
    const size_t total = (size_t)(P.N + 1) * P.Bp, stride = (size_t)gridDim.x * blockDim.x;
    for(size_t w = (size_t)blockIdx.x * blockDim.x + threadIdx.x; w < total; w += stride) {
        const int b = (int)(w % P.Bp), k = (int)(w / P.Bp);
        if(b >= P.B || !P.i[ILQG_I_LOC][b]) continue;
        const double *xs = cur_x(P, k, b);
        double *xo = home_x(P, k, b);
#pragma unroll
        for(int i = 0; i < NX; i++) xo[i * XSI] = xs[i * XSI];
        if(k < P.N) {
            const double *us = cur_u(P, k, b);
            double *uo = home_u(P, k, b);
#pragma unroll
            for(int i = 0; i < NU; i++) uo[i * XSI] = us[i * XSI];
        }
    }
}
```

Baseline: 193.2.

## Compute derivatives ahead during line search and reuse them in backward pass

Adds a 'derivs_ahead' mode that stores a compact per-step record of the time-varying derivatives. The search kernels write this record for the accepted trajectory, along with a post-adopt kernel for second-stage winners, so the next backward pass reads precomputed derivatives instead of recomputing them in the fused backward kernel. Staleness tracking invalidates the record on any state or parameter write. The aim is to take derivative evaluation off the serial backward sweep, at the cost of extra memory, extra writes during the search, and a fair amount of invalidation logic.

```diff
diff --git a/ddp-generator_amd/csrc/ilqg_host.c b/ddp-generator_amd/csrc/ilqg_host.c
--- a/ddp-generator_amd/csrc/ilqg_host.c
+++ b/ddp-generator_amd/csrc/ilqg_host.c
@@ -43,7 +43,7 @@
     int device, B, N;
     tOptSet opt;
     double alpha_store[ILQG_MAX_ALPHA];
-    int resweep, fuse_derivs, ls_split, ls_keep, bw_split;
+    int resweep, fuse_derivs, ls_split, ls_keep, bw_split, derivs_ahead;
     double **p;
     char *p_given;
     int params_pushed;
@@ -256,6 +256,7 @@
     c->fuse_derivs = c->resweep ? 0 : 1;
     c->ls_keep = 1;
     c->bw_split = 0;
+    c->derivs_ahead = 1;
     standard_parameters(&c->opt);
     ilqg_dev_dims(dims);
     c->ls_split = dims[7] ? 1 : 4;
@@ -356,6 +357,11 @@
     if(strcmp(name, "bw_split") == 0) {
         if(n != 1) return fail_msg(c, err_scalar);
         c->bw_split = value[0] != 0.0;
+        return 0;
+    }
+    if(strcmp(name, "derivs_ahead") == 0) {
+        if(n != 1) return fail_msg(c, err_scalar);
+        c->derivs_ahead = value[0] != 0.0;
         return 0;
     }
     if(strcmp(name, "ls_keep") == 0) {
@@ -439,6 +445,7 @@
     d.ls_split = c->ls_split;
     d.ls_keep = c->ls_keep;
     d.bw_split = c->bw_split;
+    d.derivs_ahead = c->derivs_ahead;
     { int g; EACH_GROUP(g) if(ilqg_dev_set_opts(c->dev[g], &d)) return fail(c, "options"); }
     if(!c->params_pushed) {
         int sizes[64];
@@ -1238,7 +1245,7 @@
     w->opt = c->opt;
     memcpy(w->alpha_store, c->opt.alpha, sizeof(double) * c->opt.n_alpha);
     w->opt.alpha = w->alpha_store;
-    w->resweep = c->resweep; w->fuse_derivs = c->fuse_derivs; w->ls_split = c->ls_split; w->ls_keep = c->ls_keep; w->bw_split = c->bw_split;
+    w->resweep = c->resweep; w->fuse_derivs = c->fuse_derivs; w->ls_split = c->ls_split; w->ls_keep = c->ls_keep; w->bw_split = c->bw_split; w->derivs_ahead = c->derivs_ahead;
     for(i = 0; i < n_params; i++) {
         memcpy(w->p[i], c->p[i], sizeof(double) * param_len(c, i));
         w->p_given[i] = c->p_given[i];
diff --git a/ddp-generator_amd/csrc/ilqg_shim.h b/ddp-generator_amd/csrc/ilqg_shim.h
--- a/ddp-generator_amd/csrc/ilqg_shim.h
+++ b/ddp-generator_amd/csrc/ilqg_shim.h
@@ -23,6 +23,7 @@
     int ls_keep;
     int bw_split;
     int fuse_derivs;
+    int derivs_ahead;
 } ilqg_dev_opts_t;
 
 enum {
diff --git a/ddp-generator_amd/csrc/ilqg_shim_impl.inc b/ddp-generator_amd/csrc/ilqg_shim_impl.inc
--- a/ddp-generator_amd/csrc/ilqg_shim_impl.inc
+++ b/ddp-generator_amd/csrc/ilqg_shim_impl.inc
@@ -97,6 +97,7 @@
     Buffer<int> queues;
     Buffer<double> cand, cand1;
     Buffer<double> xpl, upl;
+    Buffer<double> ahead_rec;
     Buffer<unsigned> spec_ints;
     Buffer<double> spec_doubles;
     Buffer<double> log_x, log_u, log_c;
@@ -153,6 +154,7 @@
     int loc_set;
     bool defer_commit, commit_pending, pending_zero;
     int commit_s1, commit_set;
+    bool ahead_valid, ahead_run, ahead_off;
     bool winner_done;
     int cus;
     bool work_consts;
@@ -194,6 +196,8 @@
 
 static ilqg_dev *g_spec_last;
 struct FieldInfo { int steps_plus; int wd, wh; };
+
+inline void ahead_stale(ilqg_dev *d) { d->ahead_valid = false; }
 
 FieldInfo field_info(int f) {
     switch(f) {
@@ -658,6 +662,7 @@
 }
 
 int ilqg_dev_set_params(ilqg_dev_t *d, int n_params, const int *sizes, const double *const *values) {
+    ahead_stale(d);
     HIP_TRY(hipSetDevice(d->device));
     HIP_TRY(hipStreamSynchronize(d->stream));
     d->param_bufs.clear();
@@ -714,6 +719,7 @@
     return d->pb_values.reserve(bytes, d->stream);
 }
 int ilqg_dev_set_params_batch(ilqg_dev_t *d, int n_named, const int *named, const double *values, int on_device) {
+    ahead_stale(d);
     HIP_TRY(hipSetDevice(d->device));
     if(WAVE_MAP) {
         g_err = "set_params_batch: this library maps one wavefront to a trajectory (wave mapping); its kernels do not carry "
@@ -760,6 +766,7 @@
     return 0;
 }
 int ilqg_dev_set_param_steps_batch(ilqg_dev_t *d, int index, const double *values, int on_device) {
+    ahead_stale(d);
     HIP_TRY(hipSetDevice(d->device));
     if(WAVE_MAP) {
         g_err = "set_param_steps_batch: this library maps one wavefront to a trajectory (wave mapping); its kernels do not carry "
@@ -819,6 +826,7 @@
         g_err = "ilqg_dev_set_opts: n_alpha must be in 1..16";
         return 1;
     }
+    if(memcmp(&d->O, o, sizeof(*o)) != 0) ahead_stale(d);
     d->O = *o;
     return 0;
 }
@@ -839,6 +847,7 @@
 }
 
 int ilqg_dev_write(ilqg_dev_t *d, int field, const double *host) {
+    ahead_stale(d);
     return ilqg_dev_write_steps(d, field, host, field_steps(d, field));
 }
 
@@ -914,6 +923,7 @@
 static int all_home(ilqg_dev_t *d);
 
 int ilqg_dev_write_steps(ilqg_dev_t *d, int field, const double *host, int steps) {
+    ahead_stale(d);
     HIP_TRY(hipSetDevice(d->device));
     if(has_tiled_copy(field) && all_home(d)) return 1;
     const FieldInfo fi = field_info(field);
@@ -988,6 +998,7 @@
 }
 
 int ilqg_dev_write_int(ilqg_dev_t *d, int field, const int *host) {
+    ahead_stale(d);
     HIP_TRY(hipSetDevice(d->device));
     const int w = int_field_width(field);
     const size_t bytes = (size_t)w * d->Bp * sizeof(int);
@@ -1057,6 +1068,7 @@
 }
 
 int ilqg_dev_reset(ilqg_dev_t *d) {
+    ahead_stale(d);
     HIP_TRY(hipSetDevice(d->device));
     hipLaunchKernelGGL(k_reset, grid1(d->Bp, 256), dim3(256), 0, d->stream, d->P, d->O);
     if(HAS_MUL) {
@@ -1108,6 +1120,7 @@
 }
 
 int ilqg_dev_rollout_init(ilqg_dev_t *d) {
+    ahead_stale(d);
     NEED_PARAMS(d);
     HIP_TRY(hipSetDevice(d->device));
     if(all_home(d)) return 1;
@@ -1119,6 +1132,7 @@
 }
 
 int ilqg_dev_shift(ilqg_dev_t *d, int steps, int use_plan_x0) {
+    ahead_stale(d);
     HIP_TRY(hipSetDevice(d->device));
     if(steps < 0 || steps >= d->N) {
         g_err = "ilqg_dev_shift: steps must be in 0 .. n_hor - 1";
@@ -1141,6 +1155,7 @@
 }
 
 int ilqg_dev_write_u_tail(ilqg_dev_t *d, const double *host, int steps) {
+    ahead_stale(d);
     HIP_TRY(hipSetDevice(d->device));
     if(steps < 1 || steps > d->N) {
         g_err = "ilqg_dev_write_u_tail: bad step count";
@@ -1218,6 +1233,7 @@
 
 int ilqg_dev_shift_winners(ilqg_dev_t *d, int K, int first, const int *winner, int steps, const double *x0_new, const double *u_tail, const double *du,
                            int on_device) {
+    ahead_stale(d);
     HIP_TRY(hipSetDevice(d->device));
     if(!segments_ok(d, K, first)) return 1;
     if(steps < 0 || steps >= d->N) {
@@ -1437,6 +1453,7 @@
 }
 
 int ilqg_dev_put_x0_device(ilqg_dev_t *d, const double *x0) {
+    ahead_stale(d);
     HIP_TRY(hipSetDevice(d->device));
     if(all_home(d)) return 1;
     const size_t n = (size_t)d->B * NX;
@@ -1450,6 +1467,7 @@
 }
 
 int ilqg_dev_put_u_tail_device(ilqg_dev_t *d, const double *tail, int steps) {
+    ahead_stale(d);
     HIP_TRY(hipSetDevice(d->device));
     if(steps < 1 || steps > d->N) {
         g_err = "ilqg_dev_put_u_tail_device: bad step count";
@@ -1491,6 +1509,7 @@
 }
 
 int ilqg_dev_shift_param(ilqg_dev_t *d, int index, int steps, const double *tail) {
+    ahead_stale(d);
     HIP_TRY(hipSetDevice(d->device));
     NEED_PARAMS(d);
     constexpr int want[ILQG_NP > 0 ? ILQG_NP : 1] = ILQG_PSIZES;
@@ -1520,6 +1539,7 @@
 }
 
 int ilqg_dev_shift_param_batch(ilqg_dev_t *d, int index, int steps, const double *tail, int on_device) {
+    ahead_stale(d);
     HIP_TRY(hipSetDevice(d->device));
     const int s = step_slot(index);
     if(s < 0 || !d->sr_on[s]) {
@@ -1600,6 +1620,7 @@
 }
 extern "C" {
 int ilqg_dev_loop_begin(ilqg_dev_t *d, const ilqg_dev_loop_t *loop) {
+    ahead_stale(d);
     HIP_TRY(hipSetDevice(d->device));
     const ilqg_dev_loop_t &L = *loop;
     const bool windows = L.windows && N_STEP_PARAMS > 0, named = L.plant && L.n_named > 0;
@@ -1656,6 +1677,7 @@
 }
 
 int ilqg_dev_loop_apply(ilqg_dev_t *d, int round, int feedback) {
+    ahead_stale(d);
     HIP_TRY(hipSetDevice(d->device));
     if(!loop_round_ok(d, round, "ilqg_dev_loop_apply")) return 1;
     const int steps = d->loop.steps, rounds = d->loop.rounds;
@@ -1686,6 +1708,7 @@
 }
 
 int ilqg_dev_loop_shift(ilqg_dev_t *d, int round) {
+    ahead_stale(d);
     HIP_TRY(hipSetDevice(d->device));
     if(!loop_round_ok(d, round, "ilqg_dev_loop_shift")) return 1;
     if(d->loop.windows && windows_move<N_STEP_PARAMS>(d, round)) return 1;
@@ -1875,6 +1898,7 @@
 #endif
 
 int ilqg_dev_derivs(ilqg_dev_t *d) {
+    ahead_stale(d);
     NEED_PARAMS(d);
     HIP_TRY(hipSetDevice(d->device));
 #if ILQG_WAVE_MAP
@@ -1891,6 +1915,7 @@
 }
 
 int ilqg_dev_backward(ilqg_dev_t *d, int mode) {
+    if(!d->defer_commit) ahead_stale(d);
     HIP_TRY(hipSetDevice(d->device));
     if(mode < 0 || mode > 2) {
         g_err = "ilqg_dev_backward: mode must be 0, 1 or 2";
@@ -1925,6 +1950,12 @@
 #endif
 }
 
+static bool ahead_eligible(const ilqg_dev_t *d);
+static int ahead_prepare(ilqg_dev_t *d);
+static void launch_backward_ahead(ilqg_dev_t *d);
+static void launch_search2_ahead(ilqg_dev_t *d, hipStream_t rs, int a0, int n, int set);
+static void launch_adopt_home_ahead(ilqg_dev_t *d, hipStream_t rs, int s1);
+
 static void launch_select(ilqg_dev_t *d, hipStream_t rs, int a0, int a1, int second) {
     Timed t(d, ILQG_K_SELECT, rs);
     hipLaunchKernelGGL(k_select, grid1(d->Bp, 256), dim3(256), 0, rs, d->P, d->O, a0, a1, second);
@@ -1970,7 +2001,11 @@
     if(!d->pending_zero) HIP_TRY(hipMemsetAsync(d->P.n_pending, 0, sizeof(int), rs));
     d->pending_zero = false;
     launch_search_stage<0>(d, rs, 0, s1, set);
-    if(n2 > 0) {
+    if(n2 > 0 && d->ahead_run) {
+        launch_search2_ahead(d, rs, s1, n2, set);
+        launch_adopt_home_ahead(d, rs, s1);
+        d->ahead_run = false;
+    } else if(n2 > 0) {
         launch_search_stage<1>(d, rs, s1, n2, set);
         Timed t(d, ILQG_K_ADOPT, rs);
         hipLaunchKernelGGL(k_adopt_home, dim3(8 * d->cus), dim3(256), 0, rs, d->P, s1);
@@ -2039,6 +2074,7 @@
 }
 
 int ilqg_dev_search(ilqg_dev_t *d) {
+    if(!d->defer_commit) ahead_stale(d);
     NEED_PARAMS(d);
     HIP_TRY(hipSetDevice(d->device));
     const int A = d->O.n_alpha;
@@ -2068,6 +2104,7 @@
 static void launch_harvest(ilqg_dev_t *d, const HarvestPlan &plan, const int *from);
 
 int ilqg_dev_winner(ilqg_dev_t *d) {
+    if(!d->defer_commit) ahead_stale(d);
     NEED_PARAMS(d);
     HIP_TRY(hipSetDevice(d->device));
     if(d->winner_done) {
@@ -2081,6 +2118,7 @@
 }
 
 int ilqg_dev_update(ilqg_dev_t *d) {
+    if(!d->defer_commit) ahead_stale(d);
     NEED_PARAMS(d);
     HIP_TRY(hipSetDevice(d->device));
     hipStream_t rs = roll_stream(d);
@@ -2109,16 +2147,26 @@
     struct Defer {
         ilqg_dev_t *d;
         explicit Defer(ilqg_dev_t *d_) : d(d_) { d->defer_commit = true; }
-        ~Defer() { d->defer_commit = false; }
+        ~Defer() { d->defer_commit = d->ahead_run = false; }
     } defer(d);
     for(int it = 0; it < n; it++) {
-        if(d->O.fuse_derivs || WAVE_MAP) {
+        d->ahead_run = ahead_eligible(d);
+        if(d->ahead_run && ahead_prepare(d)) return 1;
+        if(d->ahead_run) {
+            launch_backward_ahead(d);
+            HIP_TRY(hipGetLastError());
+        } else if(d->O.fuse_derivs || WAVE_MAP) {
             if(ilqg_dev_backward(d, 2)) return 1;
         } else {
             if(ilqg_dev_derivs(d)) return 1;
             if(ilqg_dev_backward(d, 0)) return 1;
         }
+        const bool ahead = d->ahead_run;
         if(ilqg_dev_search(d)) return 1;
+        if(ahead && d->ahead_run) {
+            d->ahead_run = d->ahead_valid = false;
+            d->ahead_off = true;
+        }
         if(ilqg_dev_winner(d)) return 1;
         if(ilqg_dev_update(d)) return 1;
     }
@@ -2132,6 +2180,8 @@
         return 1;
     }
     HIP_TRY(hipSetDevice(dst->device));
+    ahead_stale(dst);
+    ahead_stale(src);
     for(int j = 0; j < count; j++)
         if(to[j] < 0 || to[j] >= dst->B || from[j] < 0 || from[j] >= src->B) {
             g_err = "ilqg_dev_move: trajectory index out of range";
@@ -2492,6 +2542,62 @@
     hipLaunchKernelGGL(k_harvest<>, dim3((unsigned)((plan.count + HARVEST_WAVES - 1) / HARVEST_WAVES), (unsigned)((plan.W + WAVE - 1) / WAVE)),
                        dim3(WAVE * HARVEST_WAVES), 0, d->stream, d->P, d->hist, plan, from, d->harvest.get());
 }
+
+static bool ahead_eligible(const ilqg_dev_t *d) {
+#if ILQG_HAVE_AHEAD
+    const int A = d->O.n_alpha, s1 = (d->O.ls_split > 0 && d->O.ls_split < A) ? d->O.ls_split : A;
+    return d->O.derivs_ahead && d->O.fuse_derivs && !d->O.bw_split && !HAS_MUL && !d->rows_on && !d->ahead_off && d->O.ls_keep >= 2 && s1 < A &&
+           s1 <= PLANE_A && WAVE / (A - s1) >= 1;
+#else
+    return false;
+#endif
+}
+#if ILQG_HAVE_AHEAD
+static int ahead_prepare(ilqg_dev_t *d) {
+    NEED_PARAMS(d);
+    HIP_TRY(hipSetDevice(d->device));
+    const int rc = d->ahead_rec.try_reserve((size_t)d->N * d->Bp * AHEAD_W * sizeof(double), d->stream);
+    if(rc == 1) return 1;
+    if(rc == 2) {
+        d->ahead_run = d->ahead_valid = false;
+        d->ahead_off = true;
+        return 0;
+    }
+    if(d->ahead_valid) return 0;
+    if constexpr(!HAS_MUL) {
+        Timed t(d, ILQG_K_DERIVS);
+        hipLaunchKernelGGL(k_derivs_compact<>, grid1((size_t)d->Bp * d->N, 256), dim3(256), 0, d->stream, d->P, d->O, d->pv, d->ahead_rec.get());
+    }
+    HIP_TRY(hipGetLastError());
+    d->ahead_valid = true;
+    return 0;
+}
+static void launch_backward_ahead(ilqg_dev_t *d) {
+    Timed t(d, ILQG_K_BACKWARD_FUSED);
+    if constexpr(!HAS_MUL) hipLaunchKernelGGL(k_backward_ahead<>, dim3(d->Bp / WAVE), dim3(WAVE), 0, d->stream, d->P, d->O, d->pv, (const double *)d->ahead_rec.get());
+}
+static void launch_search2_ahead(ilqg_dev_t *d, hipStream_t rs, int a0, int n, int set) {
+    Timed t(d, ILQG_K_SEARCH2, rs);
+    const int T = WAVE / n;
+    const dim3 grid((d->B + T - 1) / T + 1), block(WAVE);
+    if constexpr(!HAS_MUL) {
+        if(T * (RN / 2) <= WAVE * DMA_LOADS && !d->env.no_dma)
+            hipLaunchKernelGGL(k_search_ahead<true>, grid, block, 2 * T * RN * sizeof(double), rs, d->P, d->O, d->pv, a0, n, set, d->ahead_rec.get());
+        else
+            hipLaunchKernelGGL(k_search_ahead<false>, grid, block, 0, rs, d->P, d->O, d->pv, a0, n, set, d->ahead_rec.get());
+    }
+}
+static void launch_adopt_home_ahead(ilqg_dev_t *d, hipStream_t rs, int s1) {
+    Timed t(d, ILQG_K_ADOPT, rs);
+    hipLaunchKernelGGL(k_adopt_home, dim3(8 * d->cus), dim3(256), 0, rs, d->P, s1);
+    if constexpr(!HAS_MUL) hipLaunchKernelGGL(k_adopted_records<>, dim3(8 * d->cus), dim3(256), 0, rs, d->P, d->O, d->pv, s1, d->ahead_rec.get());
+}
+#else
+static int ahead_prepare(ilqg_dev_t *) { return 0; }
+static void launch_backward_ahead(ilqg_dev_t *) {}
+static void launch_search2_ahead(ilqg_dev_t *, hipStream_t, int, int, int) {}
+static void launch_adopt_home_ahead(ilqg_dev_t *, hipStream_t, int) {}
+#endif
 
 static int boxqp_batch(int rows, int device, int n, int count, const double *H, const double *g, const double *lower,
                        const double *upper, double *x, int *clamp, int *n_free, double *invH, int *rc, const int *active = nullptr) {
diff --git a/ddp-generator_amd/csrc/k_lane_backward.inc b/ddp-generator_amd/csrc/k_lane_backward.inc
--- a/ddp-generator_amd/csrc/k_lane_backward.inc
+++ b/ddp-generator_amd/csrc/k_lane_backward.inc
@@ -196,8 +196,53 @@
     return failed;
 }
 
+#if defined(ILQG_TIME_VARYING) && !ILQG_STATE_DEPENDENT_LIMITS && !FULL_DDP
+#define ILQG_HAVE_AHEAD 1
+#define ILQG_COUNT_ENTRY(member, index) +1
+constexpr int AHEAD_VARY = 0 ILQG_TIME_VARYING(ILQG_COUNT_ENTRY) ILQG_TIME_VARYING_FULL(ILQG_COUNT_ENTRY);
+#else
+#define ILQG_HAVE_AHEAD 0
+constexpr int AHEAD_VARY = 0;
+#endif
+constexpr int AHEAD_W = AHEAD_VARY + 1;
+
+#if ILQG_HAVE_AHEAD
+__device__ __forceinline__ void derivs_compact_step(const DevPtrs &P, double *compact, trajEl_t &t, Callbacks &C, ilqg_hooks &H, int k, int b) {
+    H.nonfinite = 0.0;
+    const int ok = derivs_step(t, nullptr, C, H, k, P.N, [] {});
+    double *out = compact + ix(P, AHEAD_W, P.N, k, 0, b);
+    int j = 0;
+#define ILQG_PUT_ENTRY(member, index) out[(j++) * SI] = t.member[index];
+    ILQG_TIME_VARYING(ILQG_PUT_ENTRY) ILQG_TIME_VARYING_FULL(ILQG_PUT_ENTRY)
+#undef ILQG_PUT_ENTRY
+    out[AHEAD_VARY * SI] = (!ok || H.nonfinite != 0.0) ? 1.0 : 0.0;
+}
+
+__device__ __forceinline__ void derivs_compact_lane(DevPtrs P, ilqg_dev_opts_t O, ParamValues A, double *compact) {
+    const size_t tid = (size_t)blockIdx.x * blockDim.x + threadIdx.x;
+    const int b = (int)(tid % P.Bp);
+    const int k = (int)(tid / P.Bp);
+    if(k >= P.N || b >= P.B) return;
+    if(P.i[ILQG_I_STATUS][b] != ILQG_ST_ACTIVE) return;
+    ILQG_CALLBACKS(C, H);
+    trajEl_t t;
+    init_running(&t, &C.o1);
+    const double *xs = cur_x(P, k, b), *us = cur_u(P, k, b);
+#pragma unroll
+    for(int i = 0; i < NX; i++) t.x[i] = xs[i * XSI];
+#pragma unroll
+    for(int i = 0; i < NU; i++) t.u[i] = us[i * XSI];
+    derivs_compact_step(P, compact, t, C, H, k, b);
+}
+template <class Compact = double>
+__global__ __launch_bounds__(256) void k_derivs_compact(DevPtrs P, ilqg_dev_opts_t O, ParamValues A, Compact *compact) {
+    derivs_compact_lane(P, O, A, compact);
+}
+#endif
+
+template <bool AHEAD = false>
 __device__ __forceinline__ int backward_sweep_fused(const DevPtrs &P, Callbacks &C, ilqg_hooks &H, int b, double lambda, int regType,
-                                                    double &dV0, double &dV1, double &g_norm) {
+                                                    double &dV0, double &dV1, double &g_norm, const double *compact = nullptr) {
     const int N = P.N;
     H.nonfinite = 0.0;
     const double *xp = cur_x(P, N, b);
@@ -248,12 +293,43 @@
         REC_COPY(GETF, t)
         return ok;
     };
+    double cn[AHEAD_W];
+    const double *cp = AHEAD ? compact + ix(P, AHEAD_W, N, N - 1, 0, b) : nullptr;
+    const size_t cs = step_stride(P, AHEAD_W);
+    auto load_compact = [&](const double *src, double *cv) {
+#pragma unroll
+        for(int i = 0; i < AHEAD_W; i++) cv[i] = src[i * SI];
+    };
+#if ILQG_HAVE_AHEAD
+    auto record_from = [&](const double *cv, const double *xv, const double *uv, int k, double *rec) {
+#pragma unroll
+        for(int i = 0; i < NX; i++) t.x[i] = xv[i];
+#pragma unroll
+        for(int i = 0; i < NU; i++) t.u[i] = uv[i];
+        int j = 0;
+#define ILQG_GET_ENTRY(member, index) t.member[index] = cv[j++];
+        ILQG_TIME_VARYING(ILQG_GET_ENTRY) ILQG_TIME_VARYING_FULL(ILQG_GET_ENTRY)
+#undef ILQG_GET_ENTRY
+        limitsU(&t, k, C.o.p, N);
+        REC_COPY(GETF, t)
+        return cv[AHEAD_VARY] == 0.0 ? 1 : 0;
+    };
+#else
+    auto record_from = [&](const double *, const double *, const double *, int, double *) { return 0; };
+#endif
     {
 #pragma unroll
         for(int i = 0; i < NX; i++) xk[i] = xp[i * XSI];
 #pragma unroll
         for(int i = 0; i < NU; i++) uk[i] = up[i * XSI];
-        const int ok = record_of(xk, uk, N - 1, cur, [] {});
+        int ok;
+        if(AHEAD) {
+            load_compact(cp, cn);
+            ok = record_from(cn, xk, uk, N - 1, cur);
+            load_compact(cp - cs, cn);
+        } else {
+            ok = record_of(xk, uk, N - 1, cur, [] {});
+        }
         if(!ok || H.nonfinite != 0.0) return 2;
     }
     double xn[NX], un[NU];
@@ -278,10 +354,12 @@
         for(int i = 0; i < NX; i++) xnn[i] = (xp - back * xs)[i * XSI];
 #pragma unroll
         for(int i = 0; i < NU; i++) unn[i] = (up - back * us)[i * XSI];
+        double cnn[AHEAD_W];
+        if(AHEAD) load_compact(cp - back * cs, cnn);
         if(pf) pf->probe(0);
         const int rc = back_step<NX, NU, FULL, HX, RecZeros>(cur, uk, Vx, Vxx, l, K, lambda, regType, dV0, dV1, gsum, pf);
         double nxt[REC];
-        const int ok = record_of(xn, un, (k > 0) ? k - 1 : 0, nxt, [&] {
+        const int ok = AHEAD ? record_from(cn, xn, un, (k > 0) ? k - 1 : 0, nxt) : record_of(xn, un, (k > 0) ? k - 1 : 0, nxt, [&] {
 #pragma unroll
             for(int i = 0; i < NX; i++) pin(Vx[i]);
 #pragma unroll
@@ -319,6 +397,11 @@
         for(int i = 0; i < NX; i++) xn[i] = xnn[i];
 #pragma unroll
         for(int i = 0; i < NU; i++) un[i] = unn[i];
+        if(AHEAD) {
+            cp -= cs;
+#pragma unroll
+            for(int i = 0; i < AHEAD_W; i++) cn[i] = cnn[i];
+        }
     }
 #undef GETF
     if(!result) g_norm = gsum / ((double)(N - 1));
@@ -332,36 +415,16 @@
 template <int mode, class... Rows>
 __global__ __launch_bounds__(WAVE, 1)
 void k_backward(DevPtrs P, ilqg_dev_opts_t O, ParamValues A, Rows... rows) {
-    constexpr bool PER_TRAJECTORY = RowPack<OWN_NONE, Rows...>::has_trajectory_rows;
-    const Place place(1);
-    const int b = blockIdx.x * WAVE + threadIdx.x;
-    if(b >= P.B) return;
-    if(P.i[ILQG_I_STATUS][b] != ILQG_ST_ACTIVE) return;
-    const int single_sweep = (mode == 1);
-    P.i[ILQG_I_NEED_DERIVS][b] = 0;
-    if(P.derivs_failed[b]) {
-        P.i[ILQG_I_STATUS][b] = ILQG_ST_DERIVS_FAILED;
-        return;
-    }
-    ILQG_CALLBACKS_IN(C, H, VECTOR_PARAMS && !PER_TRAJECTORY && mode == 2);
-    apply_rows<OWN_NONE>(C_values, C_table, P, b, 0, 0, rows...);
-    load_penalty_weights_der(C, P, b);
-    double lambda = P.f[ILQG_F_LAMBDA][b], dlambda = P.f[ILQG_F_DLAMBDA][b];
-    double dV0 = 0.0, dV1 = 0.0, g_norm = P.f[ILQG_F_GNORM][b];
-    int calls = 0, rc;
-    for(;;) {
-        if(mode == 2)
-            rc = backward_sweep_fused(P, C, H, b, lambda, O.regType, dV0, dV1, g_norm);
-        else
-            rc = backward_sweep(P, b, lambda, O.regType, dV0, dV1, g_norm);
-        calls++;
-        if(single_sweep || rc != 1) break;
-        lambda_up(O.lambdaFactor, O.lambdaMin, &lambda, &dlambda);
-        if(lambda > O.lambdaMax) break;
-    }
-    const int status = back_status(rc, g_norm, lambda, dlambda, single_sweep, O);
-    store_result(P, b, {status, lambda, dlambda, dV0, dV1, g_norm, calls, rc});
-}
+    constexpr const double *compact = nullptr;
+#include "k_lane_backward_lane.inc"
+}
+#if ILQG_HAVE_AHEAD
+template <class... Rows>
+__global__ __launch_bounds__(WAVE, 1) void k_backward_ahead(DevPtrs P, ilqg_dev_opts_t O, ParamValues A, const double *compact, Rows... rows) {
+    constexpr int mode = 3;
+#include "k_lane_backward_lane.inc"
+}
+#endif
 
 #if defined(ILQG_TIME_VARYING) && !ILQG_STATE_DEPENDENT_LIMITS && ILQG_EXPERIMENTS
 #define ILQG_HAVE_SPLIT 1
diff --git a/ddp-generator_amd/csrc/k_lane_backward_lane.inc b/ddp-generator_amd/csrc/k_lane_backward_lane.inc
--- /dev/null
+++ b/ddp-generator_amd/csrc/k_lane_backward_lane.inc
@@ -0,0 +1,31 @@
+    constexpr bool PER_TRAJECTORY = RowPack<OWN_NONE, Rows...>::has_trajectory_rows;
+    const Place place(1);
+    const int b = blockIdx.x * WAVE + threadIdx.x;
+    if(b >= P.B) return;
+    if(P.i[ILQG_I_STATUS][b] != ILQG_ST_ACTIVE) return;
+    const int single_sweep = (mode == 1);
+    P.i[ILQG_I_NEED_DERIVS][b] = 0;
+    if(P.derivs_failed[b]) {
+        P.i[ILQG_I_STATUS][b] = ILQG_ST_DERIVS_FAILED;
+        return;
+    }
+    ILQG_CALLBACKS_IN(C, H, VECTOR_PARAMS && !PER_TRAJECTORY && mode >= 2);
+    apply_rows<OWN_NONE>(C_values, C_table, P, b, 0, 0, rows...);
+    load_penalty_weights_der(C, P, b);
+    double lambda = P.f[ILQG_F_LAMBDA][b], dlambda = P.f[ILQG_F_DLAMBDA][b];
+    double dV0 = 0.0, dV1 = 0.0, g_norm = P.f[ILQG_F_GNORM][b];
+    int calls = 0, rc;
+    for(;;) {
+        if constexpr(mode == 3)
+            rc = backward_sweep_fused<true>(P, C, H, b, lambda, O.regType, dV0, dV1, g_norm, compact);
+        else if(mode == 2)
+            rc = backward_sweep_fused(P, C, H, b, lambda, O.regType, dV0, dV1, g_norm);
+        else
+            rc = backward_sweep(P, b, lambda, O.regType, dV0, dV1, g_norm);
+        calls++;
+        if(single_sweep || rc != 1) break;
+        lambda_up(O.lambdaFactor, O.lambdaMin, &lambda, &dlambda);
+        if(lambda > O.lambdaMax) break;
+    }
+    const int status = back_status(rc, g_norm, lambda, dlambda, single_sweep, O);
+    store_result(P, b, {status, lambda, dlambda, dV0, dV1, g_norm, calls, rc});
diff --git a/ddp-generator_amd/csrc/k_lane_search.inc b/ddp-generator_amd/csrc/k_lane_search.inc
--- a/ddp-generator_amd/csrc/k_lane_search.inc
+++ b/ddp-generator_amd/csrc/k_lane_search.inc
@@ -2,220 +2,54 @@
 template <int stage, bool DMA, class... Rows>
 __global__ __launch_bounds__(WAVE, 1)
 void k_search(DevPtrs P, ilqg_dev_opts_t O, ParamValues A, int a0, int n, int set, Rows... rows) {
-    constexpr bool PER_TRAJECTORY = RowPack<OWN_NONE, Rows...>::has_trajectory_rows;
-    extern __shared__ __attribute__((aligned(16))) double s_rec[];
-    const Place place(2 + stage);
-    const int lane = threadIdx.x;
-    const int T = WAVE / n;
-    int a = lane / T;
-    const int t = lane - a * T;
-    const bool used = a < n;
-    if(!used) a = n - 1;
-    const int count = stage ? *P.n_pending : P.B;
-    if((int)blockIdx.x * T >= count) return;
-    const int e = blockIdx.x * T + t;
-    const int ee = e < count ? e : count - 1;
-    const int b = stage ? P.pending[ee] : ee;
-    const bool live = used && e < count && P.i[ILQG_I_STATUS][b] == ILQG_ST_ACTIVE;
-    if(__builtin_amdgcn_ballot_w64(live) == 0ull) return;
-    const int N = P.N;
-    const int ai = a0 + a;
-    const double alpha = O.alpha[ai];
-    const bool feedback = (alpha != 0.0);
+#include "k_lane_search_wave.inc"
+}
 
-    ILQG_CALLBACKS_IN(C, H, VECTOR_PARAMS && !PER_TRAJECTORY && DMA);
-    apply_rows<OWN_NONE>(C_values, C_table, P, b, 0, 0, rows...);
-    load_penalty_weights(C, P, b);
-    trajEl_t ct;
-    multipliersEl_t mk;
-    multipliersEl_t *const mp = HAS_MUL ? &mk : nullptr;
-    init_running(&ct, &C.o1);
-
-    NomPtrs q;
-    q.x = nomp(P, 0, b) + NOM_X;
-    q.u = nomp(P, 0, b) + NOM_U;
-    q.l = nomp(P, 0, b) + NOM_L;
-    q.K = nomp(P, 0, b) + NOM_K;
-    constexpr int PIECES = RN / 2;
-    const double *dsrc[DMA_LOADS];
-    bool dact[DMA_LOADS];
-    if(DMA) {
+#if ILQG_HAVE_AHEAD
+template <bool DMA, class... Rows>
+__global__ __launch_bounds__(WAVE, 1) void k_search_ahead(DevPtrs P, ilqg_dev_opts_t O, ParamValues A, int a0, int n, int set, double *compact, Rows... rows) {
+    const int searching = (*P.n_pending + WAVE / n - 1) / (WAVE / n);
+    if((int)blockIdx.x < searching) {
+        constexpr int stage = 1;
+#include "k_lane_search_wave.inc"
+        return;
+    }
+    const size_t first = blockIdx.x - searching, stride = gridDim.x - searching;
+    const int lane = threadIdx.x, N = P.N;
+    const size_t total = (size_t)(P.Bp / WAVE) * N;
+    ILQG_CALLBACKS(C, H);
+    trajEl_t t;
+    init_running(&t, &C.o1);
+    int tile = -1, b = 0;
+    bool mine = false;
+    const double *xs = nullptr, *us = nullptr;
+    for(size_t w = first; w < total; w += stride) {
+        const int wt = (int)(w / N), k = (int)(w - (size_t)wt * N);
+        if(wt != tile) {
+            tile = wt;
+            b = tile * WAVE + lane;
+            const int a = b < P.B ? P.i[ILQG_I_ALPHA_IDX][b] - 1 : a0;
+            mine = b < P.B && P.i[ILQG_I_STATUS][b] == ILQG_ST_ACTIVE && a >= 0 && a < a0;
+            const int plane = set * P.plane_n + (mine ? a : 0);
+            xs = P.xpl + (size_t)plane * P.xplane + ix(P, NX, N + 1, 0, 0, b);
+            us = P.upl + (size_t)plane * P.uplane + ix(P, NU, N, 0, 0, b);
+        }
+        if(__builtin_amdgcn_ballot_w64(mine) == 0ull) {
+            const size_t next = (size_t)(tile + 1) * N;
+            w += (next - w - 1) / stride * stride;
+            continue;
+        }
+        if(mine) {
+            const double *xk = xs + (size_t)k * cur_xstride(P), *uk = us + (size_t)k * cur_ustride(P);
 #pragma unroll
-        for(int m = 0; m < DMA_LOADS; m++) {
-            const int qq = m * WAVE + lane;
-            const int j = qq / T, r = qq - j * T;
-            dact[m] = qq < T * PIECES;
-            const int br = __shfl(b, r < T ? r : 0);
-            dsrc[m] = nomp(P, 0, br) + 2 * (j < PIECES ? j : 0);
+            for(int i = 0; i < NX; i++) t.x[i] = xk[i * XSI];
+#pragma unroll
+            for(int i = 0; i < NU; i++) t.u[i] = uk[i * XSI];
+            derivs_compact_step(P, compact, t, C, H, k, b);
         }
     }
-    auto dma_issue = [&](int buf) {
-#pragma unroll
-        for(int m = 0; m < DMA_LOADS; m++) {
-            if(dact[m])
-                __builtin_amdgcn_global_load_lds((const __attribute__((address_space(1))) void *)dsrc[m],
-                                                 (__attribute__((address_space(3))) void *)(s_rec + (size_t)buf * T * RN + m * WAVE * 2),
-                                                 16, 0, 0);
-            dsrc[m] += RN;
-        }
-    };
-    auto dma_read = [&](NomStep &c, int buf) {
-        double rec[RN];
-        const double *base = s_rec + (size_t)buf * T * RN + 2 * t;
-#pragma unroll
-        for(int j = 0; j < PIECES; j++) {
-            rec[2 * j] = base[(size_t)j * T * 2];
-            rec[2 * j + 1] = base[(size_t)j * T * 2 + 1];
-        }
-#pragma unroll
-        for(int i = 0; i < NX; i++) c.x[i] = rec[NOM_X + i];
-#pragma unroll
-        for(int i = 0; i < NU; i++) c.u[i] = rec[NOM_U + i];
-#pragma unroll
-        for(int i = 0; i < NU; i++) c.l[i] = rec[NOM_L + i];
-#pragma unroll
-        for(int i = 0; i < NXU; i++) c.K[i] = rec[NOM_K + i];
-    };
-    double *kx, *ku;
-    const size_t kxs = stage ? (size_t)CAND_W * P.Bp : cur_xstride(P), kus = stage ? kxs : cur_ustride(P);
-    const size_t kcs = stage ? (size_t)P.Bp : (size_t)XSI;
-    if(stage) {
-        kx = P.cand + (size_t)a * (N + 1) * CAND_W * P.Bp + ee;
-        ku = kx + (size_t)NX * P.Bp;
-    } else {
-        const int plane = set * P.plane_n + a;
-        kx = P.xpl + (size_t)plane * P.xplane + ix(P, NX, N + 1, 0, 0, b);
-        ku = P.upl + (size_t)plane * P.uplane + ix(P, NU, N, 0, 0, b);
-    }
-
-    double xc[NX];
-#pragma unroll
-    for(int i = 0; i < NX; i++) xc[i] = q.x[i];
-    double csum = 0.0;
-    int okc = 1;
-    NomStep cur;
-    if(DMA) {
-        dma_issue(0);
-        asm volatile("s_waitcnt vmcnt(0)" ::: "memory");
-        dma_issue(1);
-    } else {
-        load_nominal<true, 1>(cur, q);
-    }
-    drain_memory_ops();
-    for(int k = 0; k < N; k++) {
-        NomPtrs qn;
-        qn.x = q.x + RN;
-        qn.u = q.u + RN;
-        qn.l = q.l + RN;
-        qn.K = q.K + RN;
-        if(DMA) dma_read(cur, k & 1);
-        double xin[NX], uin[NU];
-#pragma unroll
-        for(int i = 0; i < NX; i++) xin[i] = xc[i];
-        {
-            double uf[NU];
-#pragma unroll
-            for(int j = 0; j < NU; j++) uf[j] = cur.u[j] + cur.l[j] * alpha;
-#pragma unroll
-            for(int i = 0; i < NX; i++) {
-                const double dx = xin[i] - cur.x[i];
-#pragma unroll
-                for(int j = 0; j < NU; j++) uf[j] += cur.K[j + i * NU] * dx;
-            }
-#pragma unroll
-            for(int j = 0; j < NU; j++) uin[j] = feedback ? uf[j] : cur.u[j];
-        }
-        if(!DMA) load_nominal<true, 1>(cur, qn);
-        if(HAS_MUL) load_mul(P, k, b, mk);
-        double xnext[NX];
-        auto step = ILQG_FORWARD_STEP(false, ct, mp, k, N, C, xin, uin, xnext);
-        const int r = run_step(H, okc, step);
-        okc &= r;
-        csum += ct.c;
-        if(DMA) {
-            asm volatile("s_waitcnt vmcnt(0)" ::: "memory");
-        }
-        if(live) {
-#pragma unroll
-            for(int i = 0; i < NX; i++) kx[i * kcs] = ct.x[i];
-#pragma unroll
-            for(int i = 0; i < NU; i++) ku[i * kcs] = ct.u[i];
-        }
-        if(DMA && k + 2 <= N) dma_issue(k & 1);
-        kx += kxs;
-        ku += kus;
-#pragma unroll
-        for(int i = 0; i < NX; i++) xc[i] = xnext[i];
-        q = qn;
-    }
-    {
-        trajFin_t cf;
-        multipliersFin_t mf;
-        if(HAS_MUL) load_mul_fin(P, b, mf);
-        init_final(&cf, &C.o);
-        auto fin = [&]() {
-#pragma unroll
-            for(int i = 0; i < NX; i++) cf.x[i] = xc[i];
-            int r = calcFVariableAux(&cf, HAS_MUL ? &mf : nullptr, &C.o);
-            r &= ddpF(&cf, &C.o);
-            return r;
-        };
-        const int r = run_step(H, okc, fin);
-        okc &= r;
-        csum += cf.c;
-        if(live) {
-#pragma unroll
-            for(int i = 0; i < NX; i++) kx[i * kcs] = cf.x[i];
-        }
-    }
-    const int ok = (okc && H.nonfinite == 0.0) ? 1 : 0;
-    if(live) {
-        P.f[ILQG_F_ALPHA_COST][tile_ix(ILQG_MAX_ALPHA, ai, b)] = csum;
-        P.i[ILQG_I_ALPHA_OK][(size_t)ai * P.Bp + b] = ok;
-    }
-
-    const double cost = P.f[ILQG_F_COST][b], dV0 = P.f[ILQG_F_DV0][b], dV1 = P.f[ILQG_F_DV1][b];
-    const double my_dcost = cost - csum;
-    const double my_expected = expected_reduction(alpha, dV0, dV1);
-    const double my_z = reduction_ratio(my_dcost, my_expected);
-    const int my_pass = (ok && my_z > O.zMin) ? 1 : 0;
-    double cnew = (a0 > 0) ? P.f[ILQG_F_NEW_COST][b] : 0.0;
-    double dcost = P.f[ILQG_F_DCOST][b], expected = P.f[ILQG_F_EXPECTED][b];
-    int win = -1;
-    for(int i = 0; i < n; i++) {
-        const int src = i * T + t;
-        const int ok_i = __shfl(ok, src);
-        const int pass_i = __shfl(my_pass, src);
-        const double cnew_i = __shfl(csum, src);
-        const double dcost_i = __shfl(my_dcost, src);
-        const double expected_i = __shfl(my_expected, src);
-        if(win < 0) {
-            cnew = cnew_i;
-            if(ok_i) {
-                dcost = dcost_i;
-                expected = expected_i;
-                if(pass_i) win = i;
-            }
-        }
-    }
-    const bool leader = live && lane < T;
-    if(leader) {
-        P.i[ILQG_I_ALPHA_IDX][b] = (win >= 0 ? a0 + win : a0 + n) + 1;
-        P.i[ILQG_I_ACCEPTED][b] = win >= 0 ? 1 : 0;
-        P.f[ILQG_F_NEW_COST][b] = cnew;
-        P.f[ILQG_F_DCOST][b] = dcost;
-        P.f[ILQG_F_EXPECTED][b] = expected;
-    }
-    const bool more = leader && win < 0 && stage == 0 && a0 + n < O.n_alpha;
-    const unsigned long long m = __builtin_amdgcn_ballot_w64(more);
-    if(m != 0ull) {
-        int base = 0;
-        const int first = __builtin_ctzll(m);
-        if(lane == first) base = atomicAdd(P.n_pending_next, __builtin_popcountll(m));
-        base = __shfl(base, first);
-        if(more) P.pending[base + __builtin_popcountll(m & ((1ull << lane) - 1ull))] = b;
-    }
 }
+#endif
 
 __global__ void k_adopt_home(DevPtrs P, int s1) {
     const size_t stride = (size_t)gridDim.x * blockDim.x;
@@ -249,6 +83,31 @@
         }
     }
 }
+
+#if ILQG_HAVE_AHEAD
+template <class Compact = double>
+__global__ void k_adopted_records(DevPtrs P, ilqg_dev_opts_t O, ParamValues A, int s1, Compact *compact) {
+    const size_t stride = (size_t)gridDim.x * blockDim.x;
+    const int np = *P.n_pending, N1 = P.N + 1;
+    const size_t total = (size_t)P.N * np;
+    if((size_t)blockIdx.x * blockDim.x >= total) return;
+    ILQG_CALLBACKS(C, H);
+    trajEl_t t;
+    init_running(&t, &C.o1);
+    for(size_t w = (size_t)blockIdx.x * blockDim.x + threadIdx.x; w < total; w += stride) {
+        const int e = (int)(w % np), k = (int)(w / np);
+        const int b = P.pending[e];
+        if(P.i[ILQG_I_STATUS][b] != ILQG_ST_ACTIVE || !P.i[ILQG_I_ACCEPTED][b]) continue;
+        const int a = P.i[ILQG_I_ALPHA_IDX][b] - 1 - s1;
+        const double *src = P.cand + ((size_t)a * N1 + k) * CAND_W * P.Bp + e;
+#pragma unroll
+        for(int i = 0; i < NX; i++) t.x[i] = src[(size_t)i * P.Bp];
+#pragma unroll
+        for(int i = 0; i < NU; i++) t.u[i] = src[(size_t)(NX + i) * P.Bp];
+        derivs_compact_step(P, compact, t, C, H, k, b);
+    }
+}
+#endif
 
 __global__ void k_rejected_home(DevPtrs P) {
     const size_t total = (size_t)(P.N + 1) * P.Bp, stride = (size_t)gridDim.x * blockDim.x;
diff --git a/ddp-generator_amd/csrc/k_lane_search_wave.inc b/ddp-generator_amd/csrc/k_lane_search_wave.inc
--- /dev/null
+++ b/ddp-generator_amd/csrc/k_lane_search_wave.inc
@@ -0,0 +1,213 @@
+    constexpr bool PER_TRAJECTORY = RowPack<OWN_NONE, Rows...>::has_trajectory_rows;
+    extern __shared__ __attribute__((aligned(16))) double s_rec[];
+    const Place place(2 + stage);
+    const int lane = threadIdx.x;
+    const int T = WAVE / n;
+    int a = lane / T;
+    const int t = lane - a * T;
+    const bool used = a < n;
+    if(!used) a = n - 1;
+    const int count = stage ? *P.n_pending : P.B;
+    if((int)blockIdx.x * T >= count) return;
+    const int e = blockIdx.x * T + t;
+    const int ee = e < count ? e : count - 1;
+    const int b = stage ? P.pending[ee] : ee;
+    const bool live = used && e < count && P.i[ILQG_I_STATUS][b] == ILQG_ST_ACTIVE;
+    if(__builtin_amdgcn_ballot_w64(live) == 0ull) return;
+    const int N = P.N;
+    const int ai = a0 + a;
+    const double alpha = O.alpha[ai];
+    const bool feedback = (alpha != 0.0);
+
+    ILQG_CALLBACKS_IN(C, H, VECTOR_PARAMS && !PER_TRAJECTORY && DMA);
+    apply_rows<OWN_NONE>(C_values, C_table, P, b, 0, 0, rows...);
+    load_penalty_weights(C, P, b);
+    trajEl_t ct;
+    multipliersEl_t mk;
+    multipliersEl_t *const mp = HAS_MUL ? &mk : nullptr;
+    init_running(&ct, &C.o1);
+
+    NomPtrs q;
+    q.x = nomp(P, 0, b) + NOM_X;
+    q.u = nomp(P, 0, b) + NOM_U;
+    q.l = nomp(P, 0, b) + NOM_L;
+    q.K = nomp(P, 0, b) + NOM_K;
+    constexpr int PIECES = RN / 2;
+    const double *dsrc[DMA_LOADS];
+    bool dact[DMA_LOADS];
+    if(DMA) {
+#pragma unroll
+        for(int m = 0; m < DMA_LOADS; m++) {
+            const int qq = m * WAVE + lane;
+            const int j = qq / T, r = qq - j * T;
+            dact[m] = qq < T * PIECES;
+            const int br = __shfl(b, r < T ? r : 0);
+            dsrc[m] = nomp(P, 0, br) + 2 * (j < PIECES ? j : 0);
+        }
+    }
+    auto dma_issue = [&](int buf) {
+#pragma unroll
+        for(int m = 0; m < DMA_LOADS; m++) {
+            if(dact[m])
+                __builtin_amdgcn_global_load_lds((const __attribute__((address_space(1))) void *)dsrc[m],
+                                                 (__attribute__((address_space(3))) void *)(s_rec + (size_t)buf * T * RN + m * WAVE * 2),
+                                                 16, 0, 0);
+            dsrc[m] += RN;
+        }
+    };
+    auto dma_read = [&](NomStep &c, int buf) {
+        double rec[RN];
+        const double *base = s_rec + (size_t)buf * T * RN + 2 * t;
+#pragma unroll
+        for(int j = 0; j < PIECES; j++) {
+            rec[2 * j] = base[(size_t)j * T * 2];
+            rec[2 * j + 1] = base[(size_t)j * T * 2 + 1];
+        }
+#pragma unroll
+        for(int i = 0; i < NX; i++) c.x[i] = rec[NOM_X + i];
+#pragma unroll
+        for(int i = 0; i < NU; i++) c.u[i] = rec[NOM_U + i];
+#pragma unroll
+        for(int i = 0; i < NU; i++) c.l[i] = rec[NOM_L + i];
+#pragma unroll
+        for(int i = 0; i < NXU; i++) c.K[i] = rec[NOM_K + i];
+    };
+    double *kx, *ku;
+    const size_t kxs = stage ? (size_t)CAND_W * P.Bp : cur_xstride(P), kus = stage ? kxs : cur_ustride(P);
+    const size_t kcs = stage ? (size_t)P.Bp : (size_t)XSI;
+    if(stage) {
+        kx = P.cand + (size_t)a * (N + 1) * CAND_W * P.Bp + ee;
+        ku = kx + (size_t)NX * P.Bp;
+    } else {
+        const int plane = set * P.plane_n + a;
+        kx = P.xpl + (size_t)plane * P.xplane + ix(P, NX, N + 1, 0, 0, b);
+        ku = P.upl + (size_t)plane * P.uplane + ix(P, NU, N, 0, 0, b);
+    }
+
+    double xc[NX];
+#pragma unroll
+    for(int i = 0; i < NX; i++) xc[i] = q.x[i];
+    double csum = 0.0;
+    int okc = 1;
+    NomStep cur;
+    if(DMA) {
+        dma_issue(0);
+        asm volatile("s_waitcnt vmcnt(0)" ::: "memory");
+        dma_issue(1);
+    } else {
+        load_nominal<true, 1>(cur, q);
+    }
+    drain_memory_ops();
+    for(int k = 0; k < N; k++) {
+        NomPtrs qn;
+        qn.x = q.x + RN;
+        qn.u = q.u + RN;
+        qn.l = q.l + RN;
+        qn.K = q.K + RN;
+        if(DMA) dma_read(cur, k & 1);
+        double xin[NX], uin[NU];
+#pragma unroll
+        for(int i = 0; i < NX; i++) xin[i] = xc[i];
+        {
+            double uf[NU];
+#pragma unroll
+            for(int j = 0; j < NU; j++) uf[j] = cur.u[j] + cur.l[j] * alpha;
+#pragma unroll
+            for(int i = 0; i < NX; i++) {
+                const double dx = xin[i] - cur.x[i];
+#pragma unroll
+                for(int j = 0; j < NU; j++) uf[j] += cur.K[j + i * NU] * dx;
+            }
+#pragma unroll
+            for(int j = 0; j < NU; j++) uin[j] = feedback ? uf[j] : cur.u[j];
+        }
+        if(!DMA) load_nominal<true, 1>(cur, qn);
+        if(HAS_MUL) load_mul(P, k, b, mk);
+        double xnext[NX];
+        auto step = ILQG_FORWARD_STEP(false, ct, mp, k, N, C, xin, uin, xnext);
+        const int r = run_step(H, okc, step);
+        okc &= r;
+        csum += ct.c;
+        if(DMA) {
+            asm volatile("s_waitcnt vmcnt(0)" ::: "memory");
+        }
+        if(live) {
+#pragma unroll
+            for(int i = 0; i < NX; i++) kx[i * kcs] = ct.x[i];
+#pragma unroll
+            for(int i = 0; i < NU; i++) ku[i * kcs] = ct.u[i];
+        }
+        if(DMA && k + 2 <= N) dma_issue(k & 1);
+        kx += kxs;
+        ku += kus;
+#pragma unroll
+        for(int i = 0; i < NX; i++) xc[i] = xnext[i];
+        q = qn;
+    }
+    {
+        trajFin_t cf;
+        multipliersFin_t mf;
+        if(HAS_MUL) load_mul_fin(P, b, mf);
+        init_final(&cf, &C.o);
+        auto fin = [&]() {
+#pragma unroll
+            for(int i = 0; i < NX; i++) cf.x[i] = xc[i];
+            int r = calcFVariableAux(&cf, HAS_MUL ? &mf : nullptr, &C.o);
+            r &= ddpF(&cf, &C.o);
+            return r;
+        };
+        const int r = run_step(H, okc, fin);
+        okc &= r;
+        csum += cf.c;
+        if(live) {
+#pragma unroll
+            for(int i = 0; i < NX; i++) kx[i * kcs] = cf.x[i];
+        }
+    }
+    const int ok = (okc && H.nonfinite == 0.0) ? 1 : 0;
+    if(live) {
+        P.f[ILQG_F_ALPHA_COST][tile_ix(ILQG_MAX_ALPHA, ai, b)] = csum;
+        P.i[ILQG_I_ALPHA_OK][(size_t)ai * P.Bp + b] = ok;
+    }
+
+    const double cost = P.f[ILQG_F_COST][b], dV0 = P.f[ILQG_F_DV0][b], dV1 = P.f[ILQG_F_DV1][b];
+    const double my_dcost = cost - csum;
+    const double my_expected = expected_reduction(alpha, dV0, dV1);
+    const double my_z = reduction_ratio(my_dcost, my_expected);
+    const int my_pass = (ok && my_z > O.zMin) ? 1 : 0;
+    double cnew = (a0 > 0) ? P.f[ILQG_F_NEW_COST][b] : 0.0;
+    double dcost = P.f[ILQG_F_DCOST][b], expected = P.f[ILQG_F_EXPECTED][b];
+    int win = -1;
+    for(int i = 0; i < n; i++) {
+        const int src = i * T + t;
+        const int ok_i = __shfl(ok, src);
+        const int pass_i = __shfl(my_pass, src);
+        const double cnew_i = __shfl(csum, src);
+        const double dcost_i = __shfl(my_dcost, src);
+        const double expected_i = __shfl(my_expected, src);
+        if(win < 0) {
+            cnew = cnew_i;
+            if(ok_i) {
+                dcost = dcost_i;
+                expected = expected_i;
+                if(pass_i) win = i;
+            }
+        }
+    }
+    const bool leader = live && lane < T;
+    if(leader) {
+        P.i[ILQG_I_ALPHA_IDX][b] = (win >= 0 ? a0 + win : a0 + n) + 1;
+        P.i[ILQG_I_ACCEPTED][b] = win >= 0 ? 1 : 0;
+        P.f[ILQG_F_NEW_COST][b] = cnew;
+        P.f[ILQG_F_DCOST][b] = dcost;
+        P.f[ILQG_F_EXPECTED][b] = expected;
+    }
+    const bool more = leader && win < 0 && stage == 0 && a0 + n < O.n_alpha;
+    const unsigned long long m = __builtin_amdgcn_ballot_w64(more);
+    if(m != 0ull) {
+        int base = 0;
+        const int first = __builtin_ctzll(m);
+        if(lane == first) base = atomicAdd(P.n_pending_next, __builtin_popcountll(m));
+        base = __shfl(base, first);
+        if(more) P.pending[base + __builtin_popcountll(m & ((1ull << lane) - 1ull))] = b;
+    }
```

Result: slower. 124.3 (-35.7%).
